# Quantco/tabmat

Measured on AMD Instinct MI355X. Metric: SplitMatrix.sandwich GFLOP/s + effective HBM GB/s, 10M×1k mixed, higher is better.
Workload: dtype f64; 1 GPU; SplitMatrix.sandwich: dense128 + csr512@5% + cats(256,96,32), 10000000 rows/GPU, p=1024, float64 (BASELINE configs[3]); rows_per_gpu=10000000, p=1024, launch=eager, collective=none

## Files before the change

### include/tabmat_hip.h

```cpp
#ifndef TABMAT_HIP_H
#define TABMAT_HIP_H

#include <stddef.h>
#include <stdint.h>

#ifdef __cplusplus
extern "C" {
#endif

#define TM_OK 0
#define TM_EINVAL (-1)
#define TM_ENOMEM (-2)
#define TM_EUNSUPPORTED (-3)

int tm_version(void);
const char *tm_last_error(void);
int tm_device_count(int *count);
int tm_set_device(int device);
int tm_device_info(char *name, int name_len, int *compute_units, int64_t *hbm_bytes);
int tm_malloc(void **ptr, size_t bytes);
int tm_free(void *ptr);
int tm_memcpy_h2d(void *dst, const void *h_src, size_t bytes, void *stream);
int tm_memcpy_d2h(void *h_dst, const void *src, size_t bytes, void *stream);
int tm_memset(void *dst, int value, size_t bytes, void *stream);
// ... 433 lines not shown
                                          int64_t n_sel, int64_t m, const double *d_sel, double *out,
                                          void *stream);
int tm_multi_cat_sparse_sandwich_rows_u8_f32(const void *const *h_codes, const int64_t *h_ncols,
                                             const int32_t *h_drop_first, int n_cats,
                                             const float *cm_data, const uint8_t *cm_col8,
                                             const int32_t *row_ranges, const int32_t *rows,
                                             int64_t n_sel, int64_t m, const float *d_sel, float *out,
                                             void *stream);
int tm_multi_cat_sparse_sandwich_rows_u8_f64(const void *const *h_codes, const int64_t *h_ncols,
                                             const int32_t *h_drop_first, int n_cats,
                                             const double *cm_data, const uint8_t *cm_col8,
                                             const int32_t *row_ranges, const int32_t *rows,
                                             int64_t n_sel, int64_t m, const double *d_sel, double *out,
                                             void *stream);
int tm_multi_cat_sparse_sandwich_ent_f32(const void *const *h_codes, const int64_t *h_ncols,
                                         const int32_t *h_drop_first, int n_cats, int64_t n, const float *d,
                                         const float *vals, const uint16_t *meta, const uint32_t *bstart,
                                         int64_t n_slots, int64_t mk, float *out, void *stream);
int tm_multi_cat_sparse_sandwich_ent_f64(const void *const *h_codes, const int64_t *h_ncols,
                                         const int32_t *h_drop_first, int n_cats, int64_t n, const double *d,
                                         const double *vals, const uint16_t *meta, const uint32_t *bstart,
                                         int64_t n_slots, int64_t mk, double *out, void *stream);
int tm_multi_cat_pack_codes(const void *const *h_codes, const int64_t *h_ncols, const int32_t *h_drop_first, int n_cats,
                            int64_t n, uint32_t *packed, void *stream);
int tm_multi_cat_sparse_sandwich_entp_f32(const void *const *h_codes, const int64_t *h_ncols,
                                          const int32_t *h_drop_first, int n_cats, int64_t n, const float *d,
                                          const float *vals, const uint16_t *meta, const uint32_t *bstart,
                                          int64_t n_slots, int64_t mk, const uint32_t *packed, float *out, void *stream);
int tm_multi_cat_sparse_sandwich_entp_f64(const void *const *h_codes, const int64_t *h_ncols,
                                          const int32_t *h_drop_first, int n_cats, int64_t n, const double *d,
                                          const double *vals, const uint16_t *meta, const uint32_t *bstart,
                                          int64_t n_slots, int64_t mk, const uint32_t *packed, double *out, void *stream);

int tm_multi_cat_sparse_sandwich_slab_f32(const void *const *h_codes, const int64_t *h_ncols,
                                          const int32_t *h_drop_first, int n_cats, int64_t n,
                                          const float *d, const float *vals, const uint32_t *koff,
                                          const uint8_t *ecol, const int64_t *gptr, int64_t m,
                                          float *out, void *stream);
int tm_multi_cat_sparse_sandwich_slab_f64(const void *const *h_codes, const int64_t *h_ncols,
                                          const int32_t *h_drop_first, int n_cats, int64_t n,
                                          const double *d, const double *vals, const uint32_t *koff,
                                          const uint8_t *ecol, const int64_t *gptr, int64_t m,
                                          double *out, void *stream);

int tm_multi_cat_pairs_max_bins(void);
int tm_multi_cat_pairs_max_slots(void);
int tm_multi_cat_pairs_row_words(void);
int tm_multi_cat_pairs_f32(const int64_t *cat_tab, int64_t n, const float *d, const int32_t *rows,
                           int64_t n_rows, const int32_t *bundles, int n_bundles,
                           const int32_t *wg_map, int n_wg, int slots, int64_t bins,
                           const int64_t *desc, int64_t n_pairs, const int64_t *pos, double *tables,
                           double *out, int64_t p, void *stream);
int tm_multi_cat_pairs_f64(const int64_t *cat_tab, int64_t n, const double *d, const int32_t *rows,
                           int64_t n_rows, const int32_t *bundles, int n_bundles,
                           const int32_t *wg_map, int n_wg, int slots, int64_t bins,
                           const int64_t *desc, int64_t n_pairs, const int64_t *pos, double *tables,
                           double *out, int64_t p, void *stream);

int tm_multi_cat_matvec_f32(const int64_t *cat_tab, int n_cats, const int64_t *pos, const float *v,
                            int64_t n, float *out, void *stream);
int tm_multi_cat_matvec_f64(const int64_t *cat_tab, int n_cats, const int64_t *pos, const double *v,
                            int64_t n, double *out, void *stream);

int tm_csr_densify_cols_f32(const float *data, const int32_t *indices, const int64_t *indptr, int64_t n,
                            const int32_t *colmap, float *T, int64_t ld, void *stream);
int tm_csr_densify_cols_f64(const double *data, const int32_t *indices, const int64_t *indptr, int64_t n,
                            const int32_t *colmap, double *T, int64_t ld, void *stream);
int tm_csc_densify_cols_f32(const int32_t *rows, const float *vals, const int64_t *seg, const int32_t *tcol,
                            int64_t n_sel, int64_t max_len, float *T, int64_t ld, void *stream);
int tm_csc_densify_cols_f64(const int32_t *rows, const double *vals, const int64_t *seg, const int32_t *tcol,
                            int64_t n_sel, int64_t max_len, double *T, int64_t ld, void *stream);
int tm_dense_gather_cols_f32(const float *X, int64_t n, int64_t m, int order_f, const int32_t *cols,
                             int64_t n_sel, float *T, int64_t ld, int64_t t0, void *stream);
int tm_dense_gather_cols_f64(const double *X, int64_t n, int64_t m, int order_f, const int32_t *cols,
                             int64_t n_sel, double *T, int64_t ld, int64_t t0, void *stream);

int tm_scatter_block_f32(const float *src, int64_t nr, int64_t nc, const int64_t *ri,
                         const int64_t *ci, double *out, int64_t p, int mirror, int diag,
                         void *stream);
int tm_scatter_block_f64(const double *src, int64_t nr, int64_t nc, const int64_t *ri,
                         const int64_t *ci, double *out, int64_t p, int mirror, int diag,
                         void *stream);

int tm_sparse_sandwich_chunked_rows_f32(const float *cm_data, const int32_t *cm_indices,
                                        const int32_t *row_ranges, int64_t n_sel, int64_t m,
                                        int64_t nnz, const float *d_sel, float *out, void *stream);
int tm_sparse_sandwich_chunked_rows_f64(const double *cm_data, const int32_t *cm_indices,
                                        const int32_t *row_ranges, int64_t n_sel, int64_t m,
                                        int64_t nnz, const double *d_sel, double *out, void *stream);

int tm_sparse_sandwich_chunked_u8_f32(const float *cm_data, const uint8_t *cm_col8, const int32_t *cptr, int64_t n,
                                      int64_t m, int64_t nnz, const float *d, float *out, void *stream);
int tm_sparse_sandwich_chunked_u8_f64(const double *cm_data, const uint8_t *cm_col8, const int32_t *cptr, int64_t n,
                                      int64_t m, int64_t nnz, const double *d, double *out, void *stream);
int tm_sparse_sandwich_chunked_rows_u8_f32(const float *cm_data, const uint8_t *cm_col8, const int32_t *row_ranges,
                                           int64_t n_sel, int64_t m, int64_t nnz, const float *d_sel, float *out,
                                           void *stream);
int tm_sparse_sandwich_chunked_rows_u8_f64(const double *cm_data, const uint8_t *cm_col8, const int32_t *row_ranges,
                                           int64_t n_sel, int64_t m, int64_t nnz, const double *d_sel, double *out,
                                           void *stream);
int tm_sparse_sandwich_direct_f32(const float *csr_data, const int32_t *csr_indices,
                                  const int64_t *csr_indptr, int64_t n, int64_t m, const float *d,
                                  float *out, void *stream);
int tm_sparse_sandwich_direct_f64(const double *csr_data, const int32_t *csr_indices,
                                  const int64_t *csr_indptr, int64_t n, int64_t m, const double *d,
                                  double *out, void *stream);
int tm_csr_dense_sandwich_rows_f32(const float *cm_data, const int32_t *cm_indices,
                                   const int32_t *row_ranges, int64_t n_sel, const int32_t *rows,
                                   const float *d_sel, int64_t n, int64_t m, const float *B, int64_t r,
                                   int order_f, float *out, void *stream);
int tm_csr_dense_sandwich_rows_f64(const double *cm_data, const int32_t *cm_indices,
                                   const int32_t *row_ranges, int64_t n_sel, const int32_t *rows,
                                   const double *d_sel, int64_t n, int64_t m, const double *B, int64_t r,
                                   int order_f, double *out, void *stream);
int tm_csr_dense_sandwich_rows_u8_f32(const float *cm_data, const uint8_t *cm_col8,
                                      const int32_t *row_ranges, int64_t n_sel, const int32_t *rows,
                                      const float *d_sel, int64_t n, int64_t m, const float *B, int64_t r,
                                      int order_f, float *out, void *stream);
int tm_csr_dense_sandwich_rows_u8_f64(const double *cm_data, const uint8_t *cm_col8,
                                      const int32_t *row_ranges, int64_t n_sel, const int32_t *rows,
                                      const double *d_sel, int64_t n, int64_t m, const double *B, int64_t r,
                                      int order_f, double *out, void *stream);

int tm_cat_det_block_rows(void);
int tm_cat_transpose_matvec_det_f32(const int32_t *perm, const int64_t *bstart, int64_t n_blocks,
                                    const int64_t *cat_bptr, int64_t n_cols, const float *v,
                                    float *out, int accumulate, void *stream);
int tm_cat_transpose_matvec_det_f64(const int32_t *perm, const int64_t *bstart, int64_t n_blocks,
                                    const int64_t *cat_bptr, int64_t n_cols, const double *v,
                                    double *out, int accumulate, void *stream);

int tm_cat_dense_sandwich_sorted_f32(const int32_t *perm, const int64_t *bstart, int64_t n_blocks,
                                     const int64_t *cat_bptr, int64_t n_cols, const float *d,
                                     const float *Y, int64_t m, float *out, void *stream);
int tm_cat_dense_sandwich_sorted_f64(const int32_t *perm, const int64_t *bstart, int64_t n_blocks,
                                     const int64_t *cat_bptr, int64_t n_cols, const double *d,
                                     const double *Y, int64_t m, double *out, void *stream);
int tm_csc_dense_sandwich_sorted_f32(const int32_t *rows, const float *vals, const int64_t *bstart,
                                     int64_t n_blocks, const int64_t *col_bptr, int64_t n_cols,
                                     const float *d, const float *Y, int64_t m, float *out,
                                     void *stream);
int tm_csc_dense_sandwich_sorted_f64(const int32_t *rows, const double *vals, const int64_t *bstart,
                                     int64_t n_blocks, const int64_t *col_bptr, int64_t n_cols,
                                     const double *d, const double *Y, int64_t m, double *out,
                                     void *stream);
int tm_cat_sparse_sandwich_sorted_f32(const int32_t *perm, const int64_t *bstart, int64_t n_blocks,
                                      const int64_t *cat_bptr, int64_t n_cols, const float *d,
                                      const float *csr_data, const int32_t *csr_indices,
                                      const int64_t *csr_indptr, int64_t m, float *out, void *stream);
int tm_cat_sparse_sandwich_sorted_f64(const int32_t *perm, const int64_t *bstart, int64_t n_blocks,
                                      const int64_t *cat_bptr, int64_t n_cols, const double *d,
                                      const double *csr_data, const int32_t *csr_indices,
                                      const int64_t *csr_indptr, int64_t m, double *out, void *stream);

int tm_csr_matvec_multi_f32(const float *csr_data, const int32_t *csr_indices,
                            const int64_t *csr_indptr, int64_t n, int64_t m, const float *V,
                            int64_t K, const int32_t *rows, int64_t n_rows, const int32_t *cols,
                            int64_t n_cols, float *out, void *stream);
int tm_csr_rmatvec_multi_f32(const float *csr_data, const int32_t *csr_indices,
                             const int64_t *csr_indptr, int64_t n, int64_t m, const float *V,
                             int64_t K, const int32_t *rows, int64_t n_rows, const int32_t *cols,
                             int64_t n_cols, float *out, void *stream);
int tm_dense_matvec_multi_f32(const float *X, int64_t n, int64_t m, int order_f, const float *V,
                              int64_t K, const int32_t *rows, int64_t n_rows, const int32_t *cols,
                              int64_t n_cols, float *out, void *stream);
int tm_dense_rmatvec_multi_f32(const float *X, int64_t n, int64_t m, int order_f, const float *V,
// ... 31 lines not shown
```

### tabmat_amd/csrc/cat.hip

```cpp
#include <algorithm>

#include "common.hpp"
#include "reduce.hpp"

namespace tmh {

__global__ void fill_i32_kernel(int32_t *p, int64_t n, int32_t v) {
    int64_t i = (int64_t)blockIdx.x * blockDim.x + threadIdx.x;
    if (i < n) p[i] = v;
}

__global__ void scatter_iota_i32_kernel(int32_t *map, const int32_t *cols, int64_t n_cols) {
    int64_t i = (int64_t)blockIdx.x * blockDim.x + threadIdx.x;
    if (i < n_cols) map[cols[i]] = (int32_t)i;
}

int build_col_map(int32_t *map, int64_t m, const int32_t *cols, int64_t n_cols, hipStream_t st) {
    if (m > 0) {
        hipLaunchKernelGGL(fill_i32_kernel, dim3((unsigned)ceil_div(m, 256)), dim3(256), 0, st, map,
                           m, -1);
        TM_LAUNCH_CHECK();
    }
    if (n_cols > 0) {
        hipLaunchKernelGGL(scatter_iota_i32_kernel, dim3((unsigned)ceil_div(n_cols, 256)),
// ... 1199 lines not shown
        }
    }
    __syncthreads();
    F *dst = ws + ((int64_t)blockIdx.y * gridDim.x + blockIdx.x) * stride;
    for (int b = threadIdx.x; b < cs.total * GC; b += blockDim.x)
        dst[b] = (F)tile[(b / GC) * TSTR + (b % GC)];
}

template <typename F, typename IX>
__global__ __launch_bounds__(1024) void multi_cat_sparse_rows_kernel(
    CatSet cs, const F *__restrict__ cm_data, const IX *__restrict__ cm_ind,
    const int32_t *__restrict__ ranges, const int32_t *__restrict__ rows, const F *__restrict__ d_sel,
    int64_t n_sel, int64_t rows_per_block, F *__restrict__ ws, int64_t stride) {
    constexpr int GC = 32;
    extern __shared__ __attribute__((aligned(16))) unsigned char smem_raw[];
    lds_acc_t *tile = reinterpret_cast<lds_acc_t *>(smem_raw);
    constexpr int tstr = GC + 1;
    const int nel = cs.total * tstr;
    for (int b = threadIdx.x; b < nel; b += blockDim.x) tile[b] = 0.0;
    __syncthreads();
    static_assert(SPARSE_CHUNK_COLS == 4 * GC, "the chunk of the chunk-major twin must hold four 32-column groups");
    const int g = blockIdx.y;
    const int ch = g >> 2;
    const int lane = threadIdx.x & 63, wave = threadIdx.x >> 6, nwave = blockDim.x >> 6;
    const int lr = lane >> 3, lt = lane & 7;
    const int64_t t0 = (int64_t)blockIdx.x * rows_per_block;
    const int64_t t1 = min(t0 + rows_per_block, n_sel);
    const int32_t *rg = ranges + (int64_t)ch * n_sel * 2;
    for (int64_t k0 = t0 + wave * 8; k0 < t1; k0 += (int64_t)nwave * 8) {
        const int64_t k = k0 + lr;
        if (k >= t1) continue;
        const F dk = d_sel[k];
        if (dk == F(0)) continue;
        const int e0 = rg[2 * k], e1 = rg[2 * k + 1];
        if (e0 >= e1) continue;
        const int64_t row = rows[k];
        int off[MAX_CATS];
#pragma unroll
        for (int c = 0; c < MAX_CATS; ++c) {
            off[c] = -1;
            if (c < cs.n_cats) {
                const int col = cs.codes[c][row] - cs.drop[c];
                off[c] = col >= 0 ? (cs.off[c] + col) * tstr : -1;
            }
        }
        for (int e = e0 + lt; e < e1; e += 8) {
            const int col = (int)cm_ind[e] - (sizeof(IX) == 1 ? (g & 3) : g) * GC;
            if (col < 0 || col >= GC) continue;
            const lds_acc_t x = (lds_acc_t)(dk * cm_data[e]);
#pragma unroll
            for (int c = 0; c < MAX_CATS; ++c)
                if (off[c] >= 0) atomic_add(&tile[off[c] + col], x);
        }
    }
    __syncthreads();
    F *dst = ws + ((int64_t)blockIdx.y * gridDim.x + blockIdx.x) * stride;
    for (int b = threadIdx.x; b < cs.total * GC; b += blockDim.x)
        dst[b] = (F)tile[(b / GC) * tstr + (b % GC)];
}

static int make_catset(const void *const *h_codes, const int64_t *h_ncols, const int32_t *h_drop,
                       int n_cats, CatSet *cs) {
    if (n_cats < 1 || n_cats > MAX_CATS) {
        set_error("multi-cat call supports 1..%d categoricals, got %d", MAX_CATS, n_cats);
        return TM_EINVAL;
    }
    int off = 0;
    for (int c = 0; c < MAX_CATS; ++c) {
        cs->codes[c] = c < n_cats ? reinterpret_cast<const int32_t *>(h_codes[c]) : nullptr;
        cs->ncol[c] = c < n_cats ? (int)h_ncols[c] : 0;
        cs->drop[c] = c < n_cats ? h_drop[c] : 0;
        cs->off[c] = off;
        off += cs->ncol[c];
    }
    cs->n_cats = n_cats;
    cs->total = off;
    return TM_OK;
}

template <typename F>
static int run_multi_cat_dense(const void *const *h_codes, const int64_t *h_ncols,
                               const int32_t *h_drop, int n_cats, int64_t n, const F *d, const F *M,
                               int64_t m, int order_f, F *out, hipStream_t st,
                               const int32_t *rows = nullptr, int64_t n_rows = 0) {
    CatSet cs;
    int rc = make_catset(h_codes, h_ncols, h_drop, n_cats, &cs);
    if (rc) return rc;
    const int64_t total = (int64_t)cs.total * m;
    if (total == 0) return TM_OK;
    if (rows != nullptr) n = n_rows;
    if (n == 0) {
        TM_HIP(hipMemsetAsync(out, 0, sizeof(F) * (size_t)total, st));
        return TM_OK;
    }
    {
        constexpr int VEC = MCW_VEC;
        constexpr int TJW = 16 * VEC;
        const size_t tile_b = ((sizeof(lds_acc_t) * (size_t)cs.total * TJW + 15) / 16) * 16;
        const size_t lds_w = tile_b + (size_t)16 * MCW_RS * (sizeof(F) + (size_t)n_cats * sizeof(int));
        if (!order_f && n_cats <= 8 && m >= VEC && m % VEC == 0 &&
            (reinterpret_cast<uintptr_t>(M) & 15) == 0 && lds_w <= 150 * 1024 &&
            (int64_t)cs.total * TJW * (int64_t)sizeof(lds_acc_t) < (1ll << 30)) {
            const int64_t n_parts = ceil_div(m, TJW);
            const int64_t stride = (int64_t)cs.total * TJW;
            int64_t nblk = std::max<int64_t>(1, tune("catdense_rounds", 1) * NUM_CU / n_parts);
            nblk = std::min<int64_t>(nblk, std::max<int64_t>(1, ceil_div(n, 4096)));
            const int64_t rpb = ceil_div(ceil_div(n, nblk), MCW_RS) * MCW_RS;
            nblk = ceil_div(n, rpb);
            const size_t tmp_bytes = ((sizeof(F) * (size_t)(n_parts * stride) + 255) / 256) * 256;
            void *wsv = nullptr;
            rc = get_workspace(tmp_bytes + sizeof(F) * (size_t)(n_parts * nblk * stride) + 256, &wsv, st);
            if (rc) return rc;
            F *tmp = reinterpret_cast<F *>(wsv);
            F *ws = reinterpret_cast<F *>(reinterpret_cast<char *>(wsv) + tmp_bytes);
            auto gow = [&](auto kern) -> int {
                TM_HIP(hipFuncSetAttribute(reinterpret_cast<const void *>(kern),
                                           hipFuncAttributeMaxDynamicSharedMemorySize, (int)lds_w));
                prof_begin(st);
                const int nw_dflt = (sizeof(F) == 8 && tile_b > 64 * 1024) ? 8 : 16;
                const int nw = (int)std::min<int64_t>(16, std::max<int64_t>(4, tune("catdense_waves", nw_dflt)));
                hipLaunchKernelGGL(kern, dim3((unsigned)nblk, (unsigned)n_parts), dim3(nw * 64), lds_w, st,
                                   cs, d, M, n, m, rpb, ws, stride, rows, wg_log_ptr());
                prof_end(st);
                TM_LAUNCH_CHECK();
                return TM_OK;
            };
            if (n_cats == 1) rc = gow(&multi_cat_dense_wide_kernel<F, 1>);
            else if (n_cats == 2) rc = gow(&multi_cat_dense_wide_kernel<F, 2>);
            else if (n_cats == 3) rc = gow(&multi_cat_dense_wide_kernel<F, 3>);
            else if (n_cats == 4) rc = gow(&multi_cat_dense_wide_kernel<F, 4>);
            else if (n_cats == 5) rc = gow(&multi_cat_dense_wide_kernel<F, 5>);
            else if (n_cats == 6) rc = gow(&multi_cat_dense_wide_kernel<F, 6>);
            else if (n_cats == 7) rc = gow(&multi_cat_dense_wide_kernel<F, 7>);
            else rc = gow(&multi_cat_dense_wide_kernel<F, 8>);
            if (rc) return rc;
            rc = launch_reduce_partials<F>(ws, stride, (int)nblk, (int)n_parts, tmp, n_parts * stride,
                                           false, st);
            if (rc) return rc;
            hipLaunchKernelGGL((multi_cat_untile_kernel<F>), dim3((unsigned)ceil_div(total, 256)),
                               dim3(256), 0, st, tmp, (int64_t)cs.total, m, TJW, out);
            TM_LAUNCH_CHECK();
            return TM_OK;
        }
    }
    if (rows != nullptr) {
        set_error("multi_cat_dense: the row-list form needs the wide-load path");
        return TM_EUNSUPPORTED;
    }
    int TJ = 64;
    while (TJ > 1 && sizeof(lds_acc_t) * (size_t)cs.total * TJ > HIST_LDS_MAX) TJ >>= 1;
    while (TJ > 1 && TJ / 2 >= m) TJ >>= 1;
    if (sizeof(lds_acc_t) * (size_t)cs.total * TJ > HIST_LDS_MAX) {
        set_error("multi_cat_dense: %d stacked categories exceed the LDS tile", cs.total);
        return TM_EUNSUPPORTED;
    }
    const int64_t n_parts = ceil_div(m, TJ);
    const int64_t stride = (int64_t)cs.total * TJ;
    const size_t lds = sizeof(lds_acc_t) * (size_t)stride;
    int64_t nblk = std::max<int64_t>(1, NUM_CU / n_parts);
    nblk = std::min<int64_t>(nblk, std::max<int64_t>(1, ceil_div(n, 4096)));
    const int64_t rpb = ceil_div(n, nblk);
    nblk = ceil_div(n, rpb);
    const size_t tmp_bytes = ((sizeof(F) * (size_t)(n_parts * stride) + 255) / 256) * 256;
    void *wsv = nullptr;
    rc = get_workspace(tmp_bytes + sizeof(F) * (size_t)(n_parts * nblk * stride) + 256, &wsv, st);
    if (rc) return rc;
    F *tmp = reinterpret_cast<F *>(wsv);
    F *ws = reinterpret_cast<F *>(reinterpret_cast<char *>(wsv) + tmp_bytes);
    auto go = [&](auto kern) -> int {
        if (lds > 48 * 1024)
            TM_HIP(hipFuncSetAttribute(reinterpret_cast<const void *>(kern),
                                       hipFuncAttributeMaxDynamicSharedMemorySize, (int)lds));
        prof_begin(st);
        hipLaunchKernelGGL(kern, dim3((unsigned)nblk, (unsigned)n_parts), dim3(1024), lds, st, cs, d,
                           M, n, m, rpb, ws, stride);
        prof_end(st);
        TM_LAUNCH_CHECK();
        return TM_OK;
    };
#define TM_MCD_CASE(V)                                                                       \
    case V:                                                                                  \
        if (order_f) rc = go(&multi_cat_dense_f_kernel<F, V>);                               \
        else if (n_cats == 1) rc = go(&multi_cat_dense_c_kernel<F, V, 1>);                   \
        else if (n_cats == 2) rc = go(&multi_cat_dense_c_kernel<F, V, 2>);                   \
        else if (n_cats == 3) rc = go(&multi_cat_dense_c_kernel<F, V, 3>);                   \
        else if (n_cats == 4) rc = go(&multi_cat_dense_c_kernel<F, V, 4>);                   \
        else rc = go(&multi_cat_dense_c_kernel<F, V, 0>);                                    \
        break;
    switch (TJ) {
        TM_MCD_CASE(64)
        TM_MCD_CASE(32)
        TM_MCD_CASE(16)
        TM_MCD_CASE(8)
        TM_MCD_CASE(4)
        TM_MCD_CASE(2)
        TM_MCD_CASE(1)
        default:
            rc = TM_EINVAL;
    }
#undef TM_MCD_CASE
    if (rc) return rc;
    rc = launch_reduce_partials<F>(ws, stride, (int)nblk, (int)n_parts, tmp, n_parts * stride, false,
                                   st);
    if (rc) return rc;
    hipLaunchKernelGGL((multi_cat_untile_kernel<F>), dim3((unsigned)ceil_div(total, 256)),
                       dim3(256), 0, st, tmp, (int64_t)cs.total, m, TJ, out);
    TM_LAUNCH_CHECK();
    return TM_OK;
}

template <typename F, typename IX>
static int run_multi_cat_sparse_rows(const void *const *h_codes, const int64_t *h_ncols,
                                     const int32_t *h_drop, int n_cats, const F *cm_data,
                                     const IX *cm_ind, const int32_t *ranges, const int32_t *rows,
                                     int64_t n_sel, int64_t m, const F *d_sel, F *out, hipStream_t st);

template <typename F>
static int run_multi_cat_sparse(const void *const *h_codes, const int64_t *h_ncols,
                                const int32_t *h_drop, int n_cats, int64_t n, const F *d,
                                const F *vals, const unsigned *koff, const unsigned char *ecol,
                                const int64_t *gptr, int64_t m, int slab_rows, int group_cols,
                                F *out, hipStream_t st) {
    CatSet cs;
    int rc = make_catset(h_codes, h_ncols, h_drop, n_cats, &cs);
    if (rc) return rc;
    const int64_t total = (int64_t)cs.total * m;
    if (total == 0) return TM_OK;
    if (n == 0) {
        TM_HIP(hipMemsetAsync(out, 0, sizeof(F) * (size_t)total, st));
        return TM_OK;
    }
    const int64_t stride = (int64_t)cs.total * group_cols;
    const size_t tile_bytes = ((sizeof(lds_acc_t) * (size_t)cs.total * (group_cols + 1) + 15) / 16) * 16;
    if (tile_bytes > HIST_LDS_MAX) {
        set_error("multi_cat_sparse: %d stacked categories exceed the LDS tile", cs.total);
        return TM_EUNSUPPORTED;
    }
    const int nw = (int)std::min<int64_t>(16, std::max<int64_t>(4, tune("catsparse_waves", 16)));
    const size_t stage_bytes = (size_t)nw * slab_rows * (sizeof(F) + sizeof(int32_t) * (size_t)n_cats);
    const bool stage = tile_bytes + stage_bytes <= 150 * 1024;
    const size_t lds = tile_bytes + (stage ? stage_bytes : 0);
    const int n_groups = (int)ceil_div(m, group_cols);
    const int64_t n_slabs = ceil_div(n, slab_rows);
    int64_t nblk = std::max<int64_t>(1, tune("catsparse_rounds", 1) * NUM_CU / n_groups);
    nblk = std::min<int64_t>(nblk, n_slabs);
    const int64_t spb = ceil_div(n_slabs, nblk);
    nblk = ceil_div(n_slabs, spb);
    const size_t tmp_bytes = ((sizeof(F) * (size_t)(n_groups * stride) + 255) / 256) * 256;
    void *wsv = nullptr;
    rc = get_workspace(tmp_bytes + sizeof(F) * (size_t)((int64_t)n_groups * nblk * stride) + 256,
                       &wsv, st);
    if (rc) return rc;
    F *tmp = reinterpret_cast<F *>(wsv);
    F *ws = reinterpret_cast<F *>(reinterpret_cast<char *>(wsv) + tmp_bytes);
    if (stage && n_cats <= 8 && slab_rows == 128) {
        auto kpf = n_cats == 1   ? &multi_cat_sparse_pf_kernel<F, 1>
                   : n_cats == 2 ? &multi_cat_sparse_pf_kernel<F, 2>
                   : n_cats == 3 ? &multi_cat_sparse_pf_kernel<F, 3>
                   : n_cats == 4 ? &multi_cat_sparse_pf_kernel<F, 4>
                   : n_cats == 5 ? &multi_cat_sparse_pf_kernel<F, 5>
                   : n_cats == 6 ? &multi_cat_sparse_pf_kernel<F, 6>
                   : n_cats == 7 ? &multi_cat_sparse_pf_kernel<F, 7>
                                 : &multi_cat_sparse_pf_kernel<F, 8>;
        if (lds > 48 * 1024)
            TM_HIP(hipFuncSetAttribute(reinterpret_cast<const void *>(kpf),
                                       hipFuncAttributeMaxDynamicSharedMemorySize, (int)lds));
        prof_begin(st);
        hipLaunchKernelGGL(kpf, dim3((unsigned)nblk, (unsigned)n_groups), dim3(nw * 64), lds, st, cs, d,
                           vals, koff, ecol, gptr, n_groups, n_slabs, spb, group_cols, n, ws, stride,
                           wg_log_ptr());
        prof_end(st);
        TM_LAUNCH_CHECK();
    } else {
        auto kern = stage ? &multi_cat_sparse_kernel<F, true> : &multi_cat_sparse_kernel<F, false>;
        if (lds > 48 * 1024)
            TM_HIP(hipFuncSetAttribute(reinterpret_cast<const void *>(kern),
                                       hipFuncAttributeMaxDynamicSharedMemorySize, (int)lds));
        prof_begin(st);
        hipLaunchKernelGGL(kern, dim3((unsigned)nblk, (unsigned)n_groups), dim3(nw * 64), lds, st, cs,
                           d, vals, koff, ecol, gptr, n_groups, n_slabs, spb, slab_rows, group_cols,
                           n, ws, stride);
        prof_end(st);
        TM_LAUNCH_CHECK();
    }
    rc = launch_reduce_partials<F>(ws, stride, (int)nblk, n_groups, tmp,
                                   (int64_t)n_groups * stride, false, st);
    if (rc) return rc;
    hipLaunchKernelGGL((multi_cat_untile_kernel<F>), dim3((unsigned)ceil_div(total, 256)),
                       dim3(256), 0, st, tmp, (int64_t)cs.total, m, group_cols, out);
    TM_LAUNCH_CHECK();
    return TM_OK;
}

__global__ __launch_bounds__(256) void multi_cat_pack_codes_kernel(CatSet cs, int64_t n, unsigned *__restrict__ out) {
    for (int64_t r = (int64_t)blockIdx.x * blockDim.x + threadIdx.x; r < n; r += (int64_t)gridDim.x * blockDim.x) {
        unsigned pk = 0u;
#pragma unroll
        for (int c = 0; c < 3; ++c) {
            unsigned f = 1023u;
            if (c < cs.n_cats) {
                const int col = cs.codes[c][r] - cs.drop[c];
                if (col >= 0 && col < cs.ncol[c]) f = (unsigned)(cs.off[c] + col);
            }
            pk |= f << (10 * c);
        }
        out[r] = pk;
    }
}

template <typename F>
static int run_multi_cat_sparse_ent(const void *const *h_codes, const int64_t *h_ncols, const int32_t *h_drop,
                                    int n_cats, int64_t n, const F *d, const F *vals, const unsigned short *meta,
                                    const unsigned *bstart, int64_t mk, F *out, hipStream_t st,
                                    const unsigned *packed = nullptr, int64_t n_slots = 0) {
    CatSet cs;
    int rc = make_catset(h_codes, h_ncols, h_drop, n_cats, &cs);
    if (rc) return rc;
    const int64_t total = (int64_t)cs.total * mk;
    if (total == 0) return TM_OK;
    if (n == 0) {
        TM_HIP(hipMemsetAsync(out, 0, sizeof(F) * (size_t)total, st));
        return TM_OK;
    }
    TM_REQUIRE(mk % 16 == 0 && n_cats >= 1 && n_cats <= 8, "kernel columns in groups of 16, 1 .. 8 categoricals");
    TM_REQUIRE(n < (1ll << 28), "at most 2^28 - 1 rows per block");
    constexpr int GC = 32;
    const int64_t stride = (int64_t)cs.total * GC;
    const size_t lds = ((sizeof(lds_acc_t) * (size_t)cs.total * (GC + 1) + 15) / 16) * 16;
    if (lds > HIST_LDS_MAX) {
        set_error("multi_cat_sparse_ent: %d stacked categories exceed the LDS tile", cs.total);
        return TM_EUNSUPPORTED;
    }
    const int nw = (int)std::min<int64_t>(16, std::max<int64_t>(4, tune("catsparse_waves", 16)));
    const int n_groups = (int)(mk / 16);
    const int n_pairs = (n_groups + 1) / 2;
    const int64_t n_slabs = ceil_div(n, 64);
    int64_t nblk = std::max<int64_t>(1, tune("catsparse_rounds", 1) * NUM_CU / n_pairs);
    nblk = std::min<int64_t>(nblk, n_slabs);
    const int64_t spb = ceil_div(n_slabs, nblk);
    nblk = ceil_div(n_slabs, spb);
    const size_t tmp_bytes = ((sizeof(F) * (size_t)(n_pairs * stride) + 255) / 256) * 256;
    void *wsv = nullptr;
    rc = get_workspace(tmp_bytes + sizeof(F) * (size_t)((int64_t)n_pairs * nblk * stride) + 256, &wsv, st);
    if (rc) return rc;
    F *tmp = reinterpret_cast<F *>(wsv);
    F *ws = reinterpret_cast<F *>(reinterpret_cast<char *>(wsv) + tmp_bytes);
    auto kern = n_cats == 1   ? &multi_cat_sparse_ent_kernel<F, 1>
                : n_cats == 2 ? &multi_cat_sparse_ent_kernel<F, 2>
                : n_cats == 3 ? &multi_cat_sparse_ent_kernel<F, 3>
                : n_cats == 4 ? &multi_cat_sparse_ent_kernel<F, 4>
                : n_cats == 5 ? &multi_cat_sparse_ent_kernel<F, 5>
                : n_cats == 6 ? &multi_cat_sparse_ent_kernel<F, 6>
                : n_cats == 7 ? &multi_cat_sparse_ent_kernel<F, 7>
                              : &multi_cat_sparse_ent_kernel<F, 8>;
    TM_REQUIRE(packed == nullptr || (n_cats <= 3 && cs.total < 1023), "packed codes: at most 3 categoricals, 1022 levels");
    const int ncw = packed != nullptr ? 1 : n_cats;
    const size_t lds_staged = lds + (size_t)nw * 64 * (sizeof(F) + 4 * (size_t)ncw);
    const double fill = (double)n_slots / ((double)std::max(n_groups, 1) * (double)n_slabs);
    if (tune("catsparse_staged", 1) != 0 && lds_staged <= 156 * 1024 &&
        fill >= (double)tune("catsparse_staged_fill", 44)) {
        using KS = void (*)(CatSet, const F *, const F *, const unsigned short *, const unsigned *, int, int64_t, int64_t,
                            int64_t, F *, int64_t, const unsigned *, int);
        KS ks = nullptr;
        if (packed != nullptr) {
            ks = n_cats == 1 ? &multi_cat_sparse_ent_staged_kernel<F, 1, true>
                 : n_cats == 2 ? &multi_cat_sparse_ent_staged_kernel<F, 2, true>
                               : &multi_cat_sparse_ent_staged_kernel<F, 3, true>;
        } else {
            ks = n_cats == 1   ? &multi_cat_sparse_ent_staged_kernel<F, 1, false>
                 : n_cats == 2 ? &multi_cat_sparse_ent_staged_kernel<F, 2, false>
                 : n_cats == 3 ? &multi_cat_sparse_ent_staged_kernel<F, 3, false>
                 : n_cats == 4 ? &multi_cat_sparse_ent_staged_kernel<F, 4, false>
                 : n_cats == 5 ? &multi_cat_sparse_ent_staged_kernel<F, 5, false>
                 : n_cats == 6 ? &multi_cat_sparse_ent_staged_kernel<F, 6, false>
                 : n_cats == 7 ? &multi_cat_sparse_ent_staged_kernel<F, 7, false>
                               : &multi_cat_sparse_ent_staged_kernel<F, 8, false>;
        }
        if (lds_staged > 48 * 1024)
            TM_HIP(hipFuncSetAttribute(reinterpret_cast<const void *>(ks),
                                       hipFuncAttributeMaxDynamicSharedMemorySize, (int)lds_staged));
        prof_begin(st);
        hipLaunchKernelGGL(ks, dim3((unsigned)nblk, (unsigned)n_pairs), dim3(nw * 64), lds_staged, st, cs, d, vals,
                           meta, bstart, n_groups, n, n_slabs, spb, ws, stride, packed, (int)lds);
        prof_end(st);
        TM_LAUNCH_CHECK();
    } else {
        if (lds > 48 * 1024)
            TM_HIP(hipFuncSetAttribute(reinterpret_cast<const void *>(kern),
                                       hipFuncAttributeMaxDynamicSharedMemorySize, (int)lds));
        prof_begin(st);
        hipLaunchKernelGGL(kern, dim3((unsigned)nblk, (unsigned)n_pairs), dim3(nw * 64), lds, st, cs, d, vals, meta,
                           bstart, n_groups, n, n_slabs, spb, ws, stride, packed);
        prof_end(st);
        TM_LAUNCH_CHECK();
    }
    rc = launch_reduce_partials<F>(ws, stride, (int)nblk, n_pairs, tmp, (int64_t)n_pairs * stride, false, st);
    if (rc) return rc;
    hipLaunchKernelGGL((multi_cat_untile_kernel<F>), dim3((unsigned)ceil_div(total, 256)), dim3(256), 0, st, tmp,
                       (int64_t)cs.total, mk, GC, out);
    TM_LAUNCH_CHECK();
    return TM_OK;
}

}

using namespace tmh;

#define TM_CHECK_COMMON(nn) \
    TM_REQUIRE((nn) >= 0, "negative size")

extern "C" {

int tm_cat_transpose_matvec_f32(const int32_t *codes, int64_t n, int64_t n_cols, int drop_first,
                                const float *v, const int32_t *rows, int64_t n_rows,
                                const int32_t *cols, int64_t n_cols_sel, float *out, void *stream) {
    TM_CHECK_COMMON(n);
    return run_cat_tmv<float>(codes, n, n_cols, drop_first, v, rows, n_rows, cols, n_cols_sel, out,
                              as_stream(stream));
}
int tm_cat_transpose_matvec_f64(const int32_t *codes, int64_t n, int64_t n_cols, int drop_first,
                                const double *v, const int32_t *rows, int64_t n_rows,
                                const int32_t *cols, int64_t n_cols_sel, double *out,
                                void *stream) {
    TM_CHECK_COMMON(n);
    return run_cat_tmv<double>(codes, n, n_cols, drop_first, v, rows, n_rows, cols, n_cols_sel,
                               out, as_stream(stream));
}

int tm_cat_matvec_f32(const int32_t *codes, int64_t n, int64_t n_cols, int drop_first,
                      const float *v, const int32_t *cols, int64_t n_cols_sel, float *out,
                      void *stream) {
    TM_CHECK_COMMON(n);
    return run_cat_matvec<float>(codes, n, n_cols, drop_first, v, cols, n_cols_sel, out,
                                 as_stream(stream));
}
int tm_cat_matvec_f64(const int32_t *codes, int64_t n, int64_t n_cols, int drop_first,
                      const double *v, const int32_t *cols, int64_t n_cols_sel, double *out,
                      void *stream) {
    TM_CHECK_COMMON(n);
    return run_cat_matvec<double>(codes, n, n_cols, drop_first, v, cols, n_cols_sel, out,
                                  as_stream(stream));
}

int tm_cat_matvec_assign_f32(const int32_t *codes, int64_t n, int64_t n_cols, int drop_first,
                             const float *v, const int32_t *cols, int64_t n_cols_sel, float *out,
                             void *stream) {
    TM_CHECK_COMMON(n);
    return run_cat_matvec<float>(codes, n, n_cols, drop_first, v, cols, n_cols_sel, out,
                                 as_stream(stream), true);
}
int tm_cat_matvec_assign_f64(const int32_t *codes, int64_t n, int64_t n_cols, int drop_first,
                             const double *v, const int32_t *cols, int64_t n_cols_sel, double *out,
                             void *stream) {
    TM_CHECK_COMMON(n);
    return run_cat_matvec<double>(codes, n, n_cols, drop_first, v, cols, n_cols_sel, out,
                                  as_stream(stream), true);
}

int tm_cat_cat_sandwich_f32(const int32_t *i_codes, const int32_t *j_codes, int64_t n,
                            const float *d, const int32_t *rows, int64_t n_rows, int64_t i_ncol,
                            int64_t j_ncol, int i_drop_first, int j_drop_first, float *out,
                            void *stream) {
    TM_CHECK_COMMON(n);
    return run_hist<float, true>(i_codes, j_codes, d, rows, rows ? n_rows : n, i_drop_first,
                                 j_drop_first, i_ncol, j_ncol, nullptr, out, false,
                                 as_stream(stream));
}
int tm_cat_cat_sandwich_f64(const int32_t *i_codes, const int32_t *j_codes, int64_t n,
                            const double *d, const int32_t *rows, int64_t n_rows, int64_t i_ncol,
                            int64_t j_ncol, int i_drop_first, int j_drop_first, double *out,
                            void *stream) {
    TM_CHECK_COMMON(n);
    return run_hist<double, true>(i_codes, j_codes, d, rows, rows ? n_rows : n, i_drop_first,
                                  j_drop_first, i_ncol, j_ncol, nullptr, out, false,
                                  as_stream(stream));
}

int tm_cat_cat_sandwich_atomic_f32(const int32_t *i_codes, const int32_t *j_codes, int64_t n,
                                   const float *d, const int32_t *rows, int64_t n_rows, int64_t i_ncol,
                                   int64_t j_ncol, int i_drop_first, int j_drop_first, float *out,
                                   void *stream) {
    TM_CHECK_COMMON(n);
    return run_hist<float, true>(i_codes, j_codes, d, rows, rows ? n_rows : n, i_drop_first,
                                 j_drop_first, i_ncol, j_ncol, nullptr, out, false,
                                 as_stream(stream), 12);
}
int tm_cat_cat_sandwich_atomic_f64(const int32_t *i_codes, const int32_t *j_codes, int64_t n,
                                   const double *d, const int32_t *rows, int64_t n_rows, int64_t i_ncol,
                                   int64_t j_ncol, int i_drop_first, int j_drop_first, double *out,
                                   void *stream) {
    TM_CHECK_COMMON(n);
    return run_hist<double, true>(i_codes, j_codes, d, rows, rows ? n_rows : n, i_drop_first,
                                  j_drop_first, i_ncol, j_ncol, nullptr, out, false,
                                  as_stream(stream), 12);
}

int tm_cat_cat_sandwich_sorted_f32(const int32_t *ci_sorted, const int32_t *cj_sorted, const int32_t *perm,
                                   const int64_t *lptr, int64_t n_sorted, const float *d, int64_t i_ncol,
                                   int64_t j_ncol, float *out, void *stream) {
    TM_CHECK_COMMON(n_sorted);
    return run_hist_sorted<float>(ci_sorted, cj_sorted, perm, lptr, n_sorted, d, i_ncol, j_ncol, out,
                                  as_stream(stream));
}
int tm_cat_cat_sandwich_sorted_f64(const int32_t *ci_sorted, const int32_t *cj_sorted, const int32_t *perm,
                                   const int64_t *lptr, int64_t n_sorted, const double *d, int64_t i_ncol,
                                   int64_t j_ncol, double *out, void *stream) {
    TM_CHECK_COMMON(n_sorted);
    return run_hist_sorted<double>(ci_sorted, cj_sorted, perm, lptr, n_sorted, d, i_ncol, j_ncol, out,
                                   as_stream(stream));
}

int tm_cat_dense_sandwich_f32(const int32_t *codes, int64_t n, int64_t i_ncol, int drop_first,
                              const float *d, const int32_t *rows, int64_t n_rows, const float *M,
                              int64_t M_ncol, int order_f, const int32_t *j_cols, int64_t n_j,
                              float *out, void *stream) {
    TM_CHECK_COMMON(n);
    return run_cat_dense<float>(codes, n, i_ncol, drop_first, d, rows, n_rows, M, M_ncol, order_f,
                                j_cols, j_cols ? n_j : M_ncol, out, as_stream(stream));
}
int tm_cat_dense_sandwich_f64(const int32_t *codes, int64_t n, int64_t i_ncol, int drop_first,
                              const double *d, const int32_t *rows, int64_t n_rows,
                              const double *M, int64_t M_ncol, int order_f, const int32_t *j_cols,
                              int64_t n_j, double *out, void *stream) {
    TM_CHECK_COMMON(n);
    return run_cat_dense<double>(codes, n, i_ncol, drop_first, d, rows, n_rows, M, M_ncol, order_f,
                                 j_cols, j_cols ? n_j : M_ncol, out, as_stream(stream));
}

int tm_cat_sparse_sandwich_f32(const int32_t *codes, int64_t n, int64_t i_ncol, int drop_first,
                               const float *csr_data, const int32_t *csr_indices,
                               const int64_t *csr_indptr, int64_t s_ncol, const float *d,
                               const int32_t *rows, int64_t n_rows, const int32_t *cols,
                               int64_t n_cols, float *out, void *stream) {
    TM_CHECK_COMMON(n);
    return run_cat_sparse<float>(codes, n, i_ncol, drop_first, csr_data, csr_indices, csr_indptr,
                                 s_ncol, d, rows, n_rows, cols, n_cols, out, as_stream(stream));
}
int tm_cat_sparse_sandwich_f64(const int32_t *codes, int64_t n, int64_t i_ncol, int drop_first,
                               const double *csr_data, const int32_t *csr_indices,
                               const int64_t *csr_indptr, int64_t s_ncol, const double *d,
                               const int32_t *rows, int64_t n_rows, const int32_t *cols,
                               int64_t n_cols, double *out, void *stream) {
    TM_CHECK_COMMON(n);
    return run_cat_sparse<double>(codes, n, i_ncol, drop_first, csr_data, csr_indices, csr_indptr,
                                  s_ncol, d, rows, n_rows, cols, n_cols, out, as_stream(stream));
}

int tm_multi_cat_dense_sandwich_f32(const void *const *h_codes, const int64_t *h_ncols,
                                    const int32_t *h_drop_first, int n_cats, int64_t n,
                                    const float *d, const float *M, int64_t M_ncol, int order_f,
                                    float *out, void *stream) {
    return run_multi_cat_dense<float>(h_codes, h_ncols, h_drop_first, n_cats, n, d, M, M_ncol,
                                      order_f, out, as_stream(stream));
}
int tm_multi_cat_dense_sandwich_f64(const void *const *h_codes, const int64_t *h_ncols,
                                    const int32_t *h_drop_first, int n_cats, int64_t n,
                                    const double *d, const double *M, int64_t M_ncol, int order_f,
                                    double *out, void *stream) {
    return run_multi_cat_dense<double>(h_codes, h_ncols, h_drop_first, n_cats, n, d, M, M_ncol,
                                       order_f, out, as_stream(stream));
}
int tm_multi_cat_dense_sandwich_rows_f32(const void *const *h_codes, const int64_t *h_ncols,
                                         const int32_t *h_drop_first, int n_cats, int64_t n,
                                         const float *d, const float *M, int64_t M_ncol,
                                         const int32_t *rows, int64_t n_rows, float *out,
                                         void *stream) {
    return run_multi_cat_dense<float>(h_codes, h_ncols, h_drop_first, n_cats, n, d, M, M_ncol, 0, out,
                                      as_stream(stream), rows, n_rows);
}
int tm_multi_cat_dense_sandwich_rows_f64(const void *const *h_codes, const int64_t *h_ncols,
                                         const int32_t *h_drop_first, int n_cats, int64_t n,
                                         const double *d, const double *M, int64_t M_ncol,
                                         const int32_t *rows, int64_t n_rows, double *out,
                                         void *stream) {
    return run_multi_cat_dense<double>(h_codes, h_ncols, h_drop_first, n_cats, n, d, M, M_ncol, 0, out,
                                       as_stream(stream), rows, n_rows);
}
int tm_multi_cat_sparse_sandwich_ent_f32(const void *const *h_codes, const int64_t *h_ncols,
                                         const int32_t *h_drop_first, int n_cats, int64_t n, const float *d,
                                         const float *vals, const uint16_t *meta, const uint32_t *bstart,
                                         int64_t n_slots, int64_t mk, float *out, void *stream) {
    return run_multi_cat_sparse_ent<float>(h_codes, h_ncols, h_drop_first, n_cats, n, d, vals, meta, bstart, mk,
                                           out, as_stream(stream), nullptr, n_slots);
}
int tm_multi_cat_sparse_sandwich_ent_f64(const void *const *h_codes, const int64_t *h_ncols,
                                         const int32_t *h_drop_first, int n_cats, int64_t n, const double *d,
                                         const double *vals, const uint16_t *meta, const uint32_t *bstart,
                                         int64_t n_slots, int64_t mk, double *out, void *stream) {
    return run_multi_cat_sparse_ent<double>(h_codes, h_ncols, h_drop_first, n_cats, n, d, vals, meta, bstart, mk,
                                            out, as_stream(stream), nullptr, n_slots);
}
int tm_multi_cat_pack_codes(const void *const *h_codes, const int64_t *h_ncols, const int32_t *h_drop_first, int n_cats,
                            int64_t n, uint32_t *packed, void *stream) {
    CatSet cs;
    int rc = make_catset(h_codes, h_ncols, h_drop_first, n_cats, &cs);
    if (rc) return rc;
    TM_REQUIRE(n_cats <= 3 && cs.total < 1023, "packed codes: at most 3 categoricals, 1022 stacked levels");
    if (n == 0) return TM_OK;
    hipLaunchKernelGGL(multi_cat_pack_codes_kernel, dim3((unsigned)std::min<int64_t>(4 * NUM_CU, ceil_div(n, 256))),
                       dim3(256), 0, as_stream(stream), cs, n, packed);
    TM_LAUNCH_CHECK();
    return TM_OK;
}
int tm_multi_cat_sparse_sandwich_entp_f32(const void *const *h_codes, const int64_t *h_ncols,
                                          const int32_t *h_drop_first, int n_cats, int64_t n, const float *d,
                                          const float *vals, const uint16_t *meta, const uint32_t *bstart,
                                          int64_t n_slots, int64_t mk, const uint32_t *packed, float *out, void *stream) {
    return run_multi_cat_sparse_ent<float>(h_codes, h_ncols, h_drop_first, n_cats, n, d, vals, meta, bstart, mk, out,
                                           as_stream(stream), packed, n_slots);
}
int tm_multi_cat_sparse_sandwich_entp_f64(const void *const *h_codes, const int64_t *h_ncols,
                                          const int32_t *h_drop_first, int n_cats, int64_t n, const double *d,
                                          const double *vals, const uint16_t *meta, const uint32_t *bstart,
                                          int64_t n_slots, int64_t mk, const uint32_t *packed, double *out, void *stream) {
    return run_multi_cat_sparse_ent<double>(h_codes, h_ncols, h_drop_first, n_cats, n, d, vals, meta, bstart, mk,
                                            out, as_stream(stream), packed, n_slots);
}
int tm_multi_cat_sparse_sandwich_slab_f32(const void *const *h_codes, const int64_t *h_ncols,
                                          const int32_t *h_drop_first, int n_cats, int64_t n,
                                          const float *d, const float *vals, const uint32_t *koff,
                                          const uint8_t *ecol, const int64_t *gptr, int64_t m,
                                          float *out, void *stream) {
    return run_multi_cat_sparse<float>(h_codes, h_ncols, h_drop_first, n_cats, n, d, vals, koff,
                                       ecol, gptr, m, tm_slab_rows(), tm_slab_group_cols(), out,
                                       as_stream(stream));
}
int tm_multi_cat_sparse_sandwich_slab_f64(const void *const *h_codes, const int64_t *h_ncols,
                                          const int32_t *h_drop_first, int n_cats, int64_t n,
                                          const double *d, const double *vals, const uint32_t *koff,
                                          const uint8_t *ecol, const int64_t *gptr, int64_t m,
                                          double *out, void *stream) {
    return run_multi_cat_sparse<double>(h_codes, h_ncols, h_drop_first, n_cats, n, d, vals, koff,
                                        ecol, gptr, m, tm_slab_rows(), tm_slab_group_cols(), out,
                                        as_stream(stream));
}

}

namespace tmh {
template <typename F, typename IX>
static int run_multi_cat_sparse_rows(const void *const *h_codes, const int64_t *h_ncols,
                                     const int32_t *h_drop, int n_cats, const F *cm_data,
                                     const IX *cm_ind, const int32_t *ranges, const int32_t *rows,
                                     int64_t n_sel, int64_t m, const F *d_sel, F *out, hipStream_t st) {
    CatSet cs;
    int rc = make_catset(h_codes, h_ncols, h_drop, n_cats, &cs);
    if (rc) return rc;
    const int64_t total = (int64_t)cs.total * m;
    if (total == 0) return TM_OK;
    if (n_sel == 0) {
        TM_HIP(hipMemsetAsync(out, 0, sizeof(F) * (size_t)total, st));
        return TM_OK;
    }
    constexpr int GC = 32;
    const size_t lds = ((sizeof(lds_acc_t) * (size_t)cs.total * (GC + 1) + 15) / 16) * 16;
    if (lds > HIST_LDS_MAX) {
        set_error("multi_cat_sparse_rows: %d stacked categories exceed the LDS tile", cs.total);
        return TM_EUNSUPPORTED;
    }
    const int n_groups = (int)ceil_div(m, GC);
    const int64_t stride = (int64_t)cs.total * GC;
    int64_t nblk = std::max<int64_t>(1, tune("catsparse_rounds", 1) * NUM_CU / n_groups);
    nblk = std::min<int64_t>(nblk, std::max<int64_t>(1, ceil_div(n_sel, 2048)));
    const int64_t rpb = ceil_div(n_sel, nblk);
    nblk = ceil_div(n_sel, rpb);
    const size_t tmp_bytes = ((sizeof(F) * (size_t)(n_groups * stride) + 255) / 256) * 256;
    void *wsv = nullptr;
    rc = get_workspace(tmp_bytes + sizeof(F) * (size_t)((int64_t)n_groups * nblk * stride) + 256, &wsv, st);
    if (rc) return rc;
    F *tmp = reinterpret_cast<F *>(wsv);
    F *ws = reinterpret_cast<F *>(reinterpret_cast<char *>(wsv) + tmp_bytes);
    auto kern = &multi_cat_sparse_rows_kernel<F, IX>;
    if (lds > 48 * 1024)
        TM_HIP(hipFuncSetAttribute(reinterpret_cast<const void *>(kern),
                                   hipFuncAttributeMaxDynamicSharedMemorySize, (int)lds));
    prof_begin(st);
    hipLaunchKernelGGL(kern, dim3((unsigned)nblk, (unsigned)n_groups), dim3(1024), lds, st, cs, cm_data,
                       cm_ind, ranges, rows, d_sel, n_sel, rpb, ws, stride);
    prof_end(st);
    TM_LAUNCH_CHECK();
    rc = launch_reduce_partials<F>(ws, stride, (int)nblk, n_groups, tmp, (int64_t)n_groups * stride, false, st);
    if (rc) return rc;
    hipLaunchKernelGGL((multi_cat_untile_kernel<F>), dim3((unsigned)ceil_div(total, 256)), dim3(256), 0,
                       st, tmp, (int64_t)cs.total, m, GC, out);
    TM_LAUNCH_CHECK();
    return TM_OK;
}
}

extern "C" {
int tm_multi_cat_sparse_sandwich_rows_f32(const void *const *h_codes, const int64_t *h_ncols,
                                          const int32_t *h_drop_first, int n_cats,
                                          const float *cm_data, const int32_t *cm_indices,
                                          const int32_t *row_ranges, const int32_t *rows,
                                          int64_t n_sel, int64_t m, const float *d_sel, float *out,
                                          void *stream) {
    return tmh::run_multi_cat_sparse_rows<float, int32_t>(h_codes, h_ncols, h_drop_first, n_cats, cm_data,
                                                 cm_indices, row_ranges, rows, n_sel, m, d_sel, out,
                                                 tmh::as_stream(stream));
// ... 33 lines not shown
```

### tabmat_amd/csrc/reduce.hpp

```cpp
#pragma once
#include "common.hpp"

namespace tmh {

template <typename F, bool ACCUMULATE, int NW>
__global__ __launch_bounds__(NW * 64) void reduce_partials_kernel(const F *__restrict__ ws,
                                                                  int64_t stride, int nb,
                                                                  F *__restrict__ out,
                                                                  int64_t out_elems) {
    __shared__ double red[NW][64];
    const int lane = threadIdx.x & 63;
    const int wave = threadIdx.x >> 6;
    const int64_t e = (int64_t)blockIdx.x * 64 + lane;
    const int part = blockIdx.y;
    double acc = 0.0;
    if (e < stride) {
        const F *p = ws + ((int64_t)part * nb) * stride + e;
        for (int b = wave; b < nb; b += NW) acc += (double)p[(int64_t)b * stride];
    }
    red[wave][lane] = acc;
    __syncthreads();
    if (wave == 0 && e < stride) {
        const int64_t o = (int64_t)part * stride + e;
        if (o < out_elems) {
            double s = 0.0;
#pragma unroll
            for (int w = 0; w < NW; w += 4)
                s += (red[w][lane] + red[w + 1][lane]) + (red[w + 2][lane] + red[w + 3][lane]);
            if (ACCUMULATE)
                out[o] += (F)s;
            else
                out[o] = (F)s;
        }
    }
}

template <typename F>
inline int launch_reduce_partials(const F *ws, int64_t stride, int nb, int n_parts, F *out,
                                  int64_t out_elems, bool accumulate, hipStream_t st) {
    dim3 grid((unsigned)ceil_div(stride, 64), (unsigned)n_parts);
    const bool small = (int64_t)grid.x * grid.y < 1024 && nb > 16;
    if (small) {
        if (accumulate)
            hipLaunchKernelGGL((reduce_partials_kernel<F, true, 16>), grid, dim3(1024), 0, st, ws,
                               stride, nb, out, out_elems);
        else
            hipLaunchKernelGGL((reduce_partials_kernel<F, false, 16>), grid, dim3(1024), 0, st, ws,
                               stride, nb, out, out_elems);
    } else if (accumulate) {
        hipLaunchKernelGGL((reduce_partials_kernel<F, true, 4>), grid, dim3(256), 0, st, ws, stride,
                           nb, out, out_elems);
    } else {
        hipLaunchKernelGGL((reduce_partials_kernel<F, false, 4>), grid, dim3(256), 0, st, ws, stride,
                           nb, out, out_elems);
    }
    TM_LAUNCH_CHECK();
    return TM_OK;
}

__global__ void fill_i32_kernel(int32_t *p, int64_t n, int32_t v);
__global__ void scatter_iota_i32_kernel(int32_t *map, const int32_t *cols, int64_t n_cols);

int build_col_map(int32_t *map, int64_t m, const int32_t *cols, int64_t n_cols, hipStream_t st);

}
```

### tabmat_amd/csrc/sparse_blocks.hip

```cpp
#include <algorithm>

#include "common.hpp"
#include "reduce.hpp"

namespace tmh {

constexpr int KB_WAVES = 16;
constexpr int KB_TS = 128;

template <typename F>
__global__ void blocks_assemble_kernel(const F *__restrict__ tiles, int n_out, F *__restrict__ out) {
    const int j = blockIdx.x * blockDim.x + threadIdx.x;
    const int i = blockIdx.y;
    if (i >= n_out || j >= n_out) return;
    const int hi = max(i, j), lo = min(i, j);
    const int I = hi / KB_TS, J = lo / KB_TS;
    const int part = I * (I + 1) / 2 + J;
    out[(int64_t)i * n_out + j] = tiles[(int64_t)part * KB_TS * KB_TS + (hi % KB_TS) * KB_TS + (lo % KB_TS)];
}

constexpr int KB_FLAG_REP_A = 1 << 16;
constexpr int KB_FLAG_REP_B = 1 << 17;

template <typename F, bool U8, bool D12 = false>
// ... 96 lines not shown
                const unsigned iA = min((unsigned)(sd.q.x - baseA) + min((unsigned)e.ta, (unsigned)max(e.nA - 1, 0)), spanA1);
                const unsigned iB = min((unsigned)(sd.q.y - baseB) + min((unsigned)e.tb, (unsigned)max(e.nB - 1, 0)), spanB1);
#ifdef KB_ABL_WRAP
                const unsigned iAw = iA & (unsigned)(KB_ABL_WRAP), iBw = iB & (unsigned)(KB_ABL_WRAP);
                e.ca = ldi(indA, min(iAw, spanA1));
                e.va = ldf(dataA, min(iAw, spanA1));
                e.cb = ldi(indB, min(iBw, spanB1));
                e.vb = ldf(dataB, min(iBw, spanB1));
                return e;
#endif
                e.ca = U8 ? (int)ind8A[iA] : ldi(indA, iA);
                e.va = ldf(dataA, iA);
                e.cb = U8 ? (int)ind8B[iB] : ldi(indB, iB);
                e.vb = ldf(dataB, iB);
                return e;
            };
            auto process = [&](const Grp &cur) {
                __builtin_amdgcn_s_setprio(1);
                const int colA = cur.ta < cur.nA ? cur.ca - i0c : -1;
                const int colB = cur.tb < cur.nB ? cur.cb - j0c : -1;
                const int la = (colA < 0 ? -8 : colA << SH) | offmask;
                const int ba = (int)(((unsigned)colA << (7 + SH)) | ((colA & 15) << (3 + SH)));
                const int kb = colB < 0 ? BIGKEY : colB << SH;
                const F av = cur.va * cur.d, vb = cur.vb;
                add_pair(kb, la, ba, av * vb);
                add_pair(dpp_xor_i32<1>(kb), la, ba, av * dpp_xor<1>(vb));
                add_pair(dpp_xor_i32<2>(kb), la, ba, av * dpp_xor<2>(vb));
                add_pair(dpp_xor_i32<3>(kb), la, ba, av * dpp_xor<3>(vb));
#ifndef KB_ABL_HALFSTEPS
                if constexpr (FULL) {
                    const int kb4 = dpp_xor_i32<4>(kb);
                    const F vb4 = dpp_xor<4>(vb);
                    add_pair(kb4, la, ba, av * vb4);
                    add_pair(dpp_xor_i32<1>(kb4), la, ba, av * dpp_xor<1>(vb4));
                    add_pair(dpp_xor_i32<2>(kb4), la, ba, av * dpp_xor<2>(vb4));
                    add_pair(dpp_xor_i32<3>(kb4), la, ba, av * dpp_xor<3>(vb4));
                }
#endif
                __builtin_amdgcn_s_setprio(0);
            };
            const int gstep = nw * 8;
            const int gw = (wave - w0) * 8;
            Grp ea[2], eb[2];
            Dsc ps[2];
            ea[0] = load_entries(load_desc(gw));
            ea[1] = load_entries(load_desc(gw + gstep));
            ps[0] = load_desc(gw + 2 * gstep);
            ps[1] = load_desc(gw + 3 * gstep);
            for (int g = gw; g < nseg; g += 4 * gstep) {
                eb[0] = load_entries(ps[0]);
                eb[1] = load_entries(ps[1]);
                ps[0] = load_desc(g + 4 * gstep);
                ps[1] = load_desc(g + 5 * gstep);
                process(ea[0]);
                if (g + gstep < nseg) process(ea[1]);
                if (g + 2 * gstep >= nseg) break;
                ea[0] = load_entries(ps[0]);
                ea[1] = load_entries(ps[1]);
                ps[0] = load_desc(g + 6 * gstep);
                ps[1] = load_desc(g + 7 * gstep);
                process(eb[0]);
                if (g + 3 * gstep < nseg) process(eb[1]);
            }
        };
        auto run_tile = [&](auto diag_c) {
            if (wave < wfull) run_list(diag_c, std::true_type{}, b0, bfull, 0, wfull);
            else run_list(diag_c, std::false_type{}, bfull, b1, wfull, (int)(blockDim.x >> 6) - wfull);
        };
        if (I == J) run_tile(std::true_type{});
        else run_tile(std::false_type{});
    }
    __syncthreads();
    if (threadIdx.x == 0) wg_log_end(wglog, t_begin, WG_K2);
    F *dst = ws + ((int64_t)part * max_nb + slot) * (TS * TS);
    for (int b = threadIdx.x; b < TS * TS; b += blockDim.x) {
        const int r = b / TS, c = b % TS;
        dst[b] = (F)tile[r * TS + (c ^ ((r & 15) << 3))];
    }
}

template <typename F, bool U8 = false, bool D12 = false>
static int run_sparse_sandwich_blocks(const F *data, const int32_t *ind, const int32_t *cptr, int64_t n,
                                      int64_t m, int64_t nnz, const int32_t *blocks, const int32_t *wg_tab,
                                      int n_wg, int max_nb, const F *d, F *out, hipStream_t st) {
    if (m == 0) return TM_OK;
    if (n == 0 || nnz == 0 || n_wg == 0) {
        TM_HIP(hipMemsetAsync(out, 0, sizeof(F) * (size_t)(m * m), st));
        return TM_OK;
    }
    constexpr int TS = KB_TS;
    const int nchunk = (int)ceil_div(m, TS);
    const int n_parts = nchunk * (nchunk + 1) / 2;
    TM_REQUIRE(nnz < (1ll << 31) && n < (1ll << 29), "sparse block too large for the block-list sandwich");
    TM_REQUIRE(!D12 || n < (1ll << 24), "12-byte block descriptors hold 24 bits of row");
    TM_REQUIRE(max_nb >= 1 && n_wg >= 1, "empty workgroup table");
    const size_t lds = sizeof(lds_acc_t) * (size_t)(TS * TS);
    const size_t tmp_bytes = (sizeof(F) * (size_t)n_parts * TS * TS + 255) / 256 * 256;
    const size_t ws_bytes = sizeof(F) * (size_t)n_parts * (size_t)max_nb * TS * TS;
    void *wsv = nullptr;
    int rc = get_workspace(tmp_bytes + ws_bytes + 256, &wsv, st);
    if (rc) return rc;
    F *tmp = reinterpret_cast<F *>(wsv);
    F *ws = reinterpret_cast<F *>(reinterpret_cast<char *>(wsv) + tmp_bytes);
    TM_HIP(hipMemsetAsync(ws, 0, ws_bytes, st));
    auto kern = &sparse_sandwich_blocks_kernel<F, U8, D12>;
    TM_HIP(hipFuncSetAttribute(reinterpret_cast<const void *>(kern),
                               hipFuncAttributeMaxDynamicSharedMemorySize, (int)lds));
    prof_begin(st);
    const int kb_waves = (int)std::min<int64_t>(KB_WAVES, std::max<int64_t>(2, tune("k2b_waves", KB_WAVES)));
    hipLaunchKernelGGL(kern, dim3((unsigned)n_wg), dim3(kb_waves * 64), lds, st, data, ind, cptr, n, nnz - 1,
                       blocks, reinterpret_cast<const int4 *>(wg_tab), d,
                       max_nb, ws, wg_log_ptr());
    prof_end(st);
    TM_LAUNCH_CHECK();
    rc = launch_reduce_partials<F>(ws, (int64_t)TS * TS, max_nb, n_parts, tmp, (int64_t)n_parts * TS * TS,
                                   false, st);
    if (rc) return rc;
    hipLaunchKernelGGL((blocks_assemble_kernel<F>), dim3((unsigned)ceil_div(m, 64), (unsigned)m), dim3(64),
                       0, st, tmp, (int)m, out);
    TM_LAUNCH_CHECK();
    return TM_OK;
}

}

extern "C" {

int tm_sparse_sandwich_blocks_f32(const float *cm_data, const int32_t *cm_indices, const int32_t *cptr,
                                  int64_t n, int64_t m, int64_t nnz, const int32_t *blocks,
                                  const int32_t *wg_tab, int n_wg, int max_nb, const float *d, float *out,
                                  void *stream) {
    return tmh::run_sparse_sandwich_blocks<float>(cm_data, cm_indices, cptr, n, m, nnz, blocks, wg_tab, n_wg,
                                                  max_nb, d, out, tmh::as_stream(stream));
}
int tm_sparse_sandwich_blocks_f64(const double *cm_data, const int32_t *cm_indices, const int32_t *cptr,
                                  int64_t n, int64_t m, int64_t nnz, const int32_t *blocks,
                                  const int32_t *wg_tab, int n_wg, int max_nb, const double *d, double *out,
                                  void *stream) {
    return tmh::run_sparse_sandwich_blocks<double>(cm_data, cm_indices, cptr, n, m, nnz, blocks, wg_tab, n_wg,
                                                   max_nb, d, out, tmh::as_stream(stream));
}

int tm_sparse_sandwich_blocks_u8_f32(const float *cm_data, const uint8_t *cm_col8, const int32_t *cptr,
                                     int64_t n, int64_t m, int64_t nnz, const int32_t *blocks,
                                     const int32_t *wg_tab, int n_wg, int max_nb, const float *d, float *out,
                                     void *stream) {
    return tmh::run_sparse_sandwich_blocks<float, true>(cm_data, reinterpret_cast<const int32_t *>(cm_col8), cptr, n, m,
                                                        nnz, blocks, wg_tab, n_wg, max_nb, d, out,
                                                        tmh::as_stream(stream));
}
int tm_sparse_sandwich_blocks_u8_f64(const double *cm_data, const uint8_t *cm_col8, const int32_t *cptr,
                                     int64_t n, int64_t m, int64_t nnz, const int32_t *blocks,
                                     const int32_t *wg_tab, int n_wg, int max_nb, const double *d, double *out,
                                     void *stream) {
    return tmh::run_sparse_sandwich_blocks<double, true>(cm_data, reinterpret_cast<const int32_t *>(cm_col8), cptr, n, m,
                                                         nnz, blocks, wg_tab, n_wg, max_nb, d, out,
                                                         tmh::as_stream(stream));
}

int tm_sparse_sandwich_blocks_p12_f32(const float *cm_data, const uint8_t *cm_col8, const int32_t *cptr,
                                      int64_t n, int64_t m, int64_t nnz, const int32_t *blocks12,
                                      const int32_t *wg_tab, int n_wg, int max_nb, const float *d, float *out,
                                      void *stream) {
    return tmh::run_sparse_sandwich_blocks<float, true, true>(cm_data, reinterpret_cast<const int32_t *>(cm_col8), cptr,
                                                              n, m, nnz, blocks12, wg_tab, n_wg, max_nb, d, out,
                                                              tmh::as_stream(stream));
}
int tm_sparse_sandwich_blocks_p12_f64(const double *cm_data, const uint8_t *cm_col8, const int32_t *cptr,
                                      int64_t n, int64_t m, int64_t nnz, const int32_t *blocks12,
                                      const int32_t *wg_tab, int n_wg, int max_nb, const double *d, double *out,
                                      void *stream) {
    return tmh::run_sparse_sandwich_blocks<double, true, true>(cm_data, reinterpret_cast<const int32_t *>(cm_col8), cptr,
                                                               n, m, nnz, blocks12, wg_tab, n_wg, max_nb, d, out,
                                                               tmh::as_stream(stream));
}

}
```

### tabmat_amd/csrc/sparse_ent.hip

```cpp
#include "common.hpp"
#include "reduce.hpp"

namespace tmh {

constexpr int EN_R = 64;
constexpr int EN_C = 16;
constexpr int EN_NW = 16;
constexpr int EN_THREADS = EN_NW * 64;
constexpr int EN_W = 128;
constexpr int EN_B = 16;
constexpr int EN_SB = 64;

template <typename F>
struct EnLds {
    static constexpr int ROWB = EN_W * (int)sizeof(F);
    static constexpr int SLABB = EN_R * ROWB;
    static constexpr int SCR_OFF = ROWB + 2 * SLABB;
    static constexpr int CS_OFF = SCR_OFF + EN_NW * EN_SB * 16;
    static constexpr int TOTAL = CS_OFF + EN_NW * EN_C * (int)sizeof(double);
};

constexpr int EN_CVGPR = 24;
#define EN_LD "40"

// ... 254 lines not shown
        if (q != 3) enext = scratch[(q + 1) * EN_B + l16];
        EN_TICK(pt_a)
        const int slab = __builtin_amdgcn_readlane((int)e[3], 1);
        while (w < slab) end_slab();
        if (ncopied == 0 && w + 1 < ns) {
            issue_pieces((w & 1) ^ 1, 0, NV);

            ncopied = NV;
            psince += NV;
            lsince = 0;
        }
        EN_TICK(pt_p)
        F a;
        if constexpr (sizeof(F) == 8) a = __hiloint2double((int)e[1], (int)e[0]);
        else a = __uint_as_float(e[0]);
#if defined(EN_ABL_NOBATCH)
        asm volatile("" ::"v"(a), "v"(e[2]), "v"(e[3]));
#else
        const unsigned live = (unsigned)__builtin_amdgcn_ballot_w64(a != F(0)) & 0xffffu;
        const int nq = live ? ((31 - __builtin_clz(live)) >> 2) + 1 : 0;
        unsigned p0 = (unsigned)__builtin_amdgcn_readlane((int)e[3], 0);
        unsigned p1 = (unsigned)__builtin_amdgcn_readlane((int)e[3], 4);
        unsigned p2 = (unsigned)__builtin_amdgcn_readlane((int)e[3], 8);
        unsigned p3 = (unsigned)__builtin_amdgcn_readlane((int)e[3], 12);
        if (nq == 4) en_batch_asm<16, F>(p0, p1, p2, p3, a, e[2], lane_off);
        else if (nq == 3) en_batch_asm<12, F>(p0, p1, p2, p3, a, e[2], lane_off);
        else if (nq == 2) en_batch_asm<8, F>(p0, p1, p2, p3, a, e[2], lane_off);
        else if (nq == 1) en_batch_asm<4, F>(p0, p1, p2, p3, a, e[2], lane_off);
#endif
        EN_TICK(pt_x)
#if defined(EN_PROF)
        ++pt_n;
#endif
    }
    while (w < ns) end_slab();
    wait_loads(std::integral_constant<int, 0>{});
#if defined(EN_PROF)
    if (prof != nullptr && lane == 0) {
        long long *o = prof + (((int64_t)blockIdx.z * gridDim.y + blockIdx.y) * gridDim.x + blockIdx.x) * (EN_NW * 8) + wave * 8;
        o[0] = pt_a; o[1] = pt_p; o[2] = pt_x; o[3] = pt_b; o[4] = pt_bar; o[5] = pt_n; o[6] = clock64() - pt_start; o[7] = ns;
    }
#endif

    if (active) {
        F *dst = ws + (((int64_t)blockIdx.y * gridDim.x + blockIdx.x) * n_groups + group) * (EN_C * EN_W);
        static_for<EN_C>([&](auto jc) {
            constexpr int j = decltype(jc)::value;
            if constexpr (sizeof(F) == 8) {
                const u4 o = u4{en_read_acc<4 * j>(), en_read_acc<4 * j + 1>(), en_read_acc<4 * j + 2>(),
                                en_read_acc<4 * j + 3>()};
                *reinterpret_cast<u4 *>(dst + j * EN_W + 2 * lane) = o;
            } else {
                typedef unsigned u2 __attribute__((ext_vector_type(2)));
                const u2 o = u2{en_read_acc<2 * j>(), en_read_acc<2 * j + 1>()};
                *reinterpret_cast<u2 *>(dst + j * EN_W + 2 * lane) = o;
            }
        });
        if constexpr (CSUM) {
            if (blockIdx.y == 0 && lane < EN_C)
                ws_csum[(int64_t)blockIdx.x * (n_groups * EN_C) + group * EN_C + lane] = (F)cs_lds[lane];
        }
    }
}

template <typename F>
__global__ void en_untile_kernel(const F *__restrict__ tmp, int64_t m, int64_t nB, F *__restrict__ out) {
    const int64_t e = (int64_t)blockIdx.x * blockDim.x + threadIdx.x;
    if (e >= m * nB) return;
    const int64_t i = e / nB, j = e % nB;
    out[e] = tmp[((j / EN_W) * m + i) * EN_W + (j % EN_W)];
}

template <typename F>
__global__ void en_csum_kernel(const F *__restrict__ part, int nblk, int64_t m, F *__restrict__ csum) {
    const int64_t c = (int64_t)blockIdx.x * blockDim.x + threadIdx.x;
    if (c >= m) return;
    double a = 0.0;
    for (int b = 0; b < nblk; ++b) a += (double)part[(int64_t)b * m + c];
    csum[c] = (F)a;
}

template <typename F>
static int run_csr_dense_ent(const F *vals, const uint16_t *meta, const uint32_t *bstart, int64_t n, int64_t m,
                             const F *B, int64_t r, const F *d, F *out, F *colsum, hipStream_t st) {
    const int64_t nB = r;
    const int64_t total = m * nB;
    if (total == 0) return TM_OK;
    constexpr int VEC = 16 / (int)sizeof(F);
    if ((reinterpret_cast<uintptr_t>(B) & 15) != 0 || r % VEC != 0 || nB < VEC) {
        set_error("tm_csr_dense_sandwich_ent: B must be C-ordered with 16-byte aligned rows");
        return TM_EUNSUPPORTED;
    }
    if (m % EN_C != 0) {
        set_error("tm_csr_dense_sandwich_ent: m must be a multiple of tm_ent_group_cols()");
        return TM_EINVAL;
    }
    if (n >= (1ll << 28)) {
        set_error("tm_csr_dense_sandwich_ent: at most 2^28 - 1 rows per block (work in row parts)");
        return TM_EUNSUPPORTED;
    }
    const int64_t n_slabs = ceil_div(n, EN_R);
    const int n_groups = (int)(m / EN_C);
    const int n_parts = (int)ceil_div(nB, EN_W);
    const int nz = (int)ceil_div(n_groups, EN_NW);
    const bool want_csum = colsum != nullptr;
    if (n_slabs == 0) {
        TM_HIP(hipMemsetAsync(out, 0, sizeof(F) * (size_t)total, st));
        if (want_csum) TM_HIP(hipMemsetAsync(colsum, 0, sizeof(F) * (size_t)m, st));
        return TM_OK;
    }
    int64_t nblk = std::max<int64_t>(1, tune("ent_rounds", 1) * NUM_CU / ((int64_t)n_parts * nz));
    nblk = std::min<int64_t>(nblk, n_slabs);
    const int64_t spb = ceil_div(n_slabs, nblk);
    nblk = ceil_div(n_slabs, spb);
    const int64_t stride = m * EN_W;
    const size_t tmp_bytes = (sizeof(F) * (size_t)(n_parts * stride) + 255) / 256 * 256;
    const size_t part_bytes = (sizeof(F) * (size_t)((int64_t)n_parts * nblk * stride) + 255) / 256 * 256;
    const size_t csum_bytes = ((want_csum ? sizeof(F) * (size_t)(nblk * m) : 0) + 255) / 256 * 256 + 256;
    void *wsv = nullptr;
    int rc = get_workspace(tmp_bytes + part_bytes + csum_bytes + 256, &wsv, st);
    if (rc) return rc;
    F *tmp = reinterpret_cast<F *>(wsv);
    F *ws = reinterpret_cast<F *>(reinterpret_cast<char *>(wsv) + tmp_bytes);
    F *ws_csum = reinterpret_cast<F *>(reinterpret_cast<char *>(wsv) + tmp_bytes + part_bytes);
    const size_t lds = (size_t)EnLds<F>::TOTAL;
    auto kern = want_csum ? &csr_dense_ent_kernel<F, true> : &csr_dense_ent_kernel<F, false>;
    TM_HIP(hipFuncSetAttribute(reinterpret_cast<const void *>(kern),
                               hipFuncAttributeMaxDynamicSharedMemorySize, (int)lds));
    prof_begin(st);
    hipLaunchKernelGGL(kern, dim3((unsigned)nblk, (unsigned)n_parts, (unsigned)nz), dim3(EN_THREADS), lds, st,
                       vals, meta, bstart, n_groups, n_slabs, spb, B, n, r, (int)nB, d, ws, ws_csum,
                       reinterpret_cast<long long *>((uintptr_t)tune("ent_prof", 0)));
    prof_end(st);
    TM_LAUNCH_CHECK();
    rc = launch_reduce_partials<F>(ws, stride, (int)nblk, n_parts, tmp, n_parts * stride, false, st);
    if (rc) return rc;
    hipLaunchKernelGGL((en_untile_kernel<F>), dim3((unsigned)ceil_div(total, 256)), dim3(256), 0, st, tmp, m,
                       nB, out);
    TM_LAUNCH_CHECK();
    if (want_csum) {
        hipLaunchKernelGGL((en_csum_kernel<F>), dim3((unsigned)ceil_div(m, 256)), dim3(256), 0, st, ws_csum,
                           (int)nblk, m, colsum);
        TM_LAUNCH_CHECK();
    }
    return TM_OK;
}

}

extern "C" {
int tm_ent_rows(void) { return tmh::EN_R; }
int tm_ent_group_cols(void) { return tmh::EN_C; }
int tm_ent_batch_slots(void) { return tmh::EN_B; }

int tm_csr_dense_sandwich_ent_f32(const float *vals, const uint16_t *meta, const uint32_t *bstart, int64_t n,
                                  int64_t m, const float *B, int64_t r, const float *d, float *out,
                                  float *colsum, void *stream) {
    return tmh::run_csr_dense_ent<float>(vals, meta, bstart, n, m, B, r, d, out, colsum, tmh::as_stream(stream));
}
int tm_csr_dense_sandwich_ent_f64(const double *vals, const uint16_t *meta, const uint32_t *bstart, int64_t n,
                                  int64_t m, const double *B, int64_t r, const double *d, double *out,
                                  double *colsum, void *stream) {
    return tmh::run_csr_dense_ent<double>(vals, meta, bstart, n, m, B, r, d, out, colsum, tmh::as_stream(stream));
}
}
```

### tabmat_amd/csrc/syrk_i8.hip

```cpp
#include <algorithm>
#include <cmath>

#include "common.hpp"

#if defined(I8_NO_SB)
#define I8_SB
#else
#define I8_SB __builtin_amdgcn_sched_barrier(0)
#endif
#if defined(I8_TRACE)
#define I8_STAMP(k)                                                                                     \
    do {                                                                                                \
        if (blockIdx.x == 0 && lane == 0 && trace_it >= 8 && trace_it < 12)                             \
            trace_buf[((trace_it - 8) * 4 + wave) * 8 + (k)] = __builtin_readcyclecounter();            \
    } while (0)
#else
#define I8_STAMP(k)
#endif
namespace tmh {

constexpr int I8_W = 128;
constexpr int I8_T = 36;
constexpr int I8_ND = 5;
constexpr int I8_WLO = 2;
// ... 647 lines not shown
        if (xtv) TM_HIP(hipMemsetAsync(xtv, 0, sizeof(double) * (size_t)m, st));
        return TM_OK;
    }
    if (colsum) TM_HIP(hipMemsetAsync(colsum, 0, sizeof(double) * (size_t)m, st));
    if (xtv) TM_HIP(hipMemsetAsync(xtv, 0, sizeof(double) * (size_t)m, st));
    const int64_t n_items64 = ceil_div(n, I8_ITEM_ROWS);
    TM_REQUIRE(n_items64 < (1ll << 31), "too many rows");
    const int n_items = (int)n_items64;
    const int grid = (int)std::max<int64_t>(1, std::min<int64_t>(n_items, tune("i8_grid", NUM_CU)));
    const size_t part_bytes = sizeof(double) * (size_t)grid * I8_T * 256;
    const size_t own_bytes = (4096 + part_bytes + 255) / 256 * 256;
    void *wsv = nullptr;
    int rc = get_workspace(own_bytes + syrk_co_ws_bytes(), &wsv, st);
    if (rc) return rc;
    char *wb = reinterpret_cast<char *>(wsv);
    I8Info *info = reinterpret_cast<I8Info *>(wb);
    unsigned *counter = reinterpret_cast<unsigned *>(wb + 256);
    double *sigma = reinterpret_cast<double *>(wb + 512);
    double *rscale = reinterpret_cast<double *>(wb + 512 + 1024);
    double *part = reinterpret_cast<double *>(wb + 4096);
    TM_HIP(hipMemsetAsync(wb, 0, 4096 + part_bytes, st));
    const int sgrid = (int)std::min<int64_t>(4 * NUM_CU, ceil_div(n, 1024));
    hipLaunchKernelGGL(i8_screen_kernel, dim3((unsigned)sgrid), dim3(256), 0, st, d, n, info);
    hipLaunchKernelGGL(i8_scale_kernel, dim3(1), dim3(I8_W), 0, st, colmax, (int)m, n, info, sigma, rscale, history);
    TM_LAUNCH_CHECK();
    prof_begin(st);
    auto go = [&](auto kern) {
        hipLaunchKernelGGL(kern, dim3((unsigned)grid), dim3(I8_THREADS), 0, st, X, ldx, n, m, d, sigma, info, n_items,
                           counter, part, colsum, center, v, xtv);
    };
    if (v) {
        if (center) go(syrk_i8_kernel<false, true, true>);
        else go(syrk_i8_kernel<false, false, true>);
    } else if (center) {
        if (colsum) go(syrk_i8_kernel<true, true>);
        else go(syrk_i8_kernel<false, true>);
    } else {
        if (colsum) go(syrk_i8_kernel<true, false>);
        else go(syrk_i8_kernel<false, false>);
    }
    prof_end(st);
    TM_LAUNCH_CHECK();
    hipLaunchKernelGGL(syrk_i8_finish_kernel, dim3(I8_T, 4), dim3(64, 16), 0, st, part, grid, (int)m, rscale, info,
                       out, ldo);
    hipLaunchKernelGGL(i8_envelope_kernel, dim3(1), dim3(I8_W), 0, st, out, ldo, colmax, (int)m, n, info, history);
    TM_LAUNCH_CHECK();
    prof_hold(true);
    rc = run_syrk_co_flagged(X, ldx, n, m, d, out, ldo, colsum, &info->flag, wb + own_bytes, st, center, v, xtv);
    prof_hold(false);
    if (rc == TM_OK && history != nullptr) {
        hipLaunchKernelGGL(i8_record_diag_kernel, dim3(1), dim3(I8_W), 0, st, out, ldo, (int)m, history);
        TM_LAUNCH_CHECK();
    }
    return rc;
}

int run_syrk_i8(const double *X, int64_t n, int64_t m, const double *d, const double *colmax, double *out,
                double *colsum, int *history, hipStream_t st, const double *center = nullptr,
                const double *v = nullptr, double *xtv = nullptr) {
    return run_syrk_i8_panel(X, m, n, m, d, colmax, out, m, colsum, history, st, center, v, xtv);
}

}

extern "C" {

int tm_dense_sandwich_i8_history_words(void) { return 4 + 2 * tmh::I8_W; }

int tm_dense_sandwich_i8_f64(const double *X, int64_t n, int64_t m, const double *d, const double *colmax,
                             double *out, void *stream) {
    return tmh::run_syrk_i8(X, n, m, d, colmax, out, nullptr, nullptr, tmh::as_stream(stream));
}

int tm_dense_sandwich_i8_xtd_f64(const double *X, int64_t n, int64_t m, const double *d, const double *colmax,
                                 double *out, double *colsum, void *stream) {
    return tmh::run_syrk_i8(X, n, m, d, colmax, out, colsum, nullptr, tmh::as_stream(stream));
}

int tm_dense_sandwich_i8_hist_f64(const double *X, int64_t n, int64_t m, const double *d, const double *colmax,
                                  double *out, double *colsum, int32_t *history, void *stream) {
    return tmh::run_syrk_i8(X, n, m, d, colmax, out, colsum, history, tmh::as_stream(stream));
}

int tm_dense_sandwich_i8_centered_f64(const double *X, int64_t n, int64_t m, const double *d, const double *colmax,
                                      const double *center, double *out, double *colsum, int32_t *history,
                                      void *stream) {
    return tmh::run_syrk_i8(X, n, m, d, colmax, out, colsum, history, tmh::as_stream(stream), center);
}

int tm_dense_sandwich_i8_xtv_f64(const double *X, int64_t n, int64_t m, const double *d, const double *v,
                                 const double *colmax, double *out, double *xtv, int32_t *history, void *stream) {
    TM_REQUIRE(v != nullptr && xtv != nullptr, "v and xtv are required");
    return tmh::run_syrk_i8(X, n, m, d, colmax, out, nullptr, history, tmh::as_stream(stream), nullptr, v, xtv);
}

int tm_dense_sandwich_i8_centered_xtv_f64(const double *X, int64_t n, int64_t m, const double *d, const double *v,
                                          const double *colmax, const double *center, double *out, double *xtv,
                                          int32_t *history, void *stream) {
    TM_REQUIRE(v != nullptr && xtv != nullptr, "v and xtv are required");
    return tmh::run_syrk_i8(X, n, m, d, colmax, out, nullptr, history, tmh::as_stream(stream), center, v, xtv);
}

}
```

### tabmat_amd/dense_matrix.py

```python
from __future__ import annotations

import os
import warnings

import numpy as np
import torch

from . import _device as D
from .ext import dense as xd
from .ext._types import DenseDev
from .matrix_base import MatrixBase
from .util import (
    check_indexer,
    check_matvec_dimensions,
    check_matvec_out_shape,
    check_sandwich_compatible,
    check_transpose_matvec_out_shape,
    normalize_index,
    np_dtype_of,
    device_row_index,
    selects_all_columns,
)


# ... 131 lines not shown
    def astype(self, dtype, order="K", casting="unsafe", copy=True):
        return type(self)(self.toarray().astype(dtype, order, casting, copy),
                          column_names=self._colnames, term_names=self._terms)

    def getcol(self, i):
        return type(self)(self.toarray()[:, [i]], column_names=[self._colnames[i]],
                          term_names=[self._terms[i]])

    def __getitem__(self, key):
        row, col = check_indexer(key)
        if self._devblk is not None and selects_all_columns(col, self.shape[1]):
            kind, *arg = device_row_index(row, self.shape[0])
            t = self._devblk.as_2d()
            sub = t[arg[0]:arg[1]] if kind == "slice" else t[D.idx_dev(arg[0], torch.int64)]
            return type(self)(sub, column_names=self._colnames, term_names=self._terms)
        names = np.array(self._colnames, dtype=object)[col].ravel().tolist()
        terms = np.array(self._terms, dtype=object)[col].ravel().tolist()
        return type(self)(self.toarray()[row, col], column_names=names, term_names=terms)

    def __matmul__(self, other):
        return self.matvec(other)

    def __str__(self):
        return "{}x{} DenseMatrix:\n\n".format(*self.shape) + np.array_str(self.toarray())

    def __repr__(self):
        return f"DenseMatrix({np.array2string(self.toarray(), separator=', ')})"

    def multiply(self, other):
        other = np.asanyarray(other)
        arr = self.toarray() * (other[:, None] if other.ndim == 1 else other)
        return type(self)(arr, column_names=self._colnames, term_names=self._terms)

    def _i8_colmax(self, center=None):
        hit = getattr(self, "_i8_ok", None)
        if hit is None:
            hit = False
            blk = self._dev_c()
            if (not blk.order_f and blk.buf.dtype == torch.float64 and 64 < blk.m <= I8_MAX_COLS
                    and (blk.m % 2 == 0 or blk.m <= 128) and blk.n >= I8_MIN_ROWS
                    and blk.buf.data_ptr() % 16 == 0):
                x = blk.as_2d()
                hi, lo = x.amax(dim=0), x.amin(dim=0)
                if bool((torch.isfinite(hi) & torch.isfinite(lo)).all().item()):
                    hit = (hi, lo, torch.maximum(hi, -lo).contiguous())
            self._i8_ok = hit
        if hit is False:
            return None
        if center is None:
            return hit[2]
        return torch.maximum(hit[0] - center, center - hit[1]).contiguous()

    def _i8_history(self, key=None):
        hs = self.__dict__.setdefault("_i8_hist", {})
        h = hs.get(key)
        if h is None:
            from ._lib import lib

            h = hs[key] = torch.zeros(int(lib().tm_dense_sandwich_i8_history_words()), dtype=torch.int32,
                                      device=self._dev_c().buf.device)
        return h

    def _center_dev(self, center):
        if center is None:
            return None
        tdt = D.torch_dtype(self.dtype)
        c = D.to_dev(center, tdt) if not isinstance(center, torch.Tensor) else center.to(tdt)
        return c.contiguous()

    def _sandwich_dev(self, d, rows, cols, center=None):
        if (SYRK_I8 and cols is None and d.dtype == torch.float64
                and (rows is None or D.nlen(rows) >= I8_MASKED_ROWS_SHARE * self.shape[0])):
            cmax = self._i8_colmax(center)
            if cmax is not None:
                key = None if center is None else "centered"
                if rows is not None:
                    d = D.masked_d(d, rows)
                    key = "masked" if center is None else "masked-centered"
                if self.shape[1] > 128:
                    return xd.dense_sandwich_i8_wide(self._dev_c(), d, cmax, center=center)
                return xd.dense_sandwich_i8(self._dev_c(), d, cmax, history=self._i8_history(key), center=center)
        return xd.dense_sandwich(self._dev_c(), d, rows, cols, center=center)

    def _sandwich_xtd_dev(self, d, center=None):
        blk = self._dev_c()
        if SYRK_I8 and d.dtype == torch.float64 and blk.m <= 128:
            cmax = self._i8_colmax(center)
            if cmax is not None:
                return xd.dense_sandwich_i8(blk, d, cmax, want_colsum=True,
                                            history=self._i8_history(None if center is None else "centered"),
                                            center=center)
        if xd.co_supported(blk, d):
            return xd.dense_sandwich_co(blk, d, want_colsum=True, center=center)
        return None

    def _sandwich_xtv_dev(self, d, v, rows=None, center=None):
        from . import categorical_matrix as _cm

        if _cm.DETERMINISTIC or d.dtype != torch.float64 or v.dtype != torch.float64 or v.ndim != 1:
            return None
        n = self.shape[0]
        if rows is not None and not (SYRK_I8 and D.nlen(rows) >= I8_MASKED_ROWS_SHARE * n):
            return None
        blk = self._dev_c()
        res = None
        if SYRK_I8:
            cmax = self._i8_colmax(center)
            if cmax is not None:
                key = None if center is None else "centered"
                if rows is not None:
                    d, v = D.masked_d(d, rows), D.masked_d(v, rows)
                    key = "masked" if center is None else "masked-centered"
                if self.shape[1] > 128:
                    out, _, xtv = xd.dense_sandwich_xtv(blk, d, v.contiguous(), "i8_wide", cmax, center=center)
                else:
                    out, _, xtv = xd.dense_sandwich_xtv(blk, d, v.contiguous(), "i8", cmax,
                                                        history=self._i8_history(key), center=center)
                res = (out, xtv)
        if res is None and rows is None and xd.co_supported(blk, d):
            out, _, xtv = xd.dense_sandwich_xtv(blk, d, v.contiguous(), "co", center=center)
            res = (out, xtv)
        if res is not None and center is not None:
            res = (res[0], res[1] + center.to(torch.float64) * v.sum(dtype=torch.float64))
        return res

    def sandwich_and_transpose_matvec(self, d, v, rows=None, cols=None):
        from .matrix_base import _check_1d

        _check_1d(v)
        d_dev_side, v_dev_side = D.is_dev(d), D.is_dev(v)
        if not d_dev_side:
            d = np.asarray(d)
        if not v_dev_side:
            v = np.asarray(v)
        check_sandwich_compatible(self, d)
        check_matvec_dimensions(self, v, transpose=True)
        n, m = self.shape
        rows_n = normalize_index(rows, n)
        cols_n = normalize_index(cols, m)
        both = None
        if (cols_n is None or (len(cols_n) == m and np.array_equal(cols_n, np.arange(m)))) \
                and (rows_n is None or len(rows_n) < n) and self.dtype == np.float64:
            d_dev = D.to_dev(d)
            if d_dev.dtype == torch.float64:
                both = self._sandwich_xtv_dev(d_dev, D.to_dev(v, torch.float64), D.idx_dev(rows_n))
        if both is None:
            return self.sandwich(d, rows, cols), self.transpose_matvec(v, rows, cols)
        H, g = both
        if not v_dev_side:
            g = D.to_host(g)
            if np.issubdtype(v.dtype, np.floating) and v.dtype != self.dtype:
                g = g.astype(np.result_type(v.dtype, self.dtype))
        return (H if d_dev_side else D.to_host(H)), g

    def _smv_block(self):
        blk = self._dev_c()
        return blk if xd.sandwich_matvec_supported(blk) else None

    def _smv_dev(self, dm, u_full, shift=None, centers=None):
        blk = self._smv_block()
        if blk is None:
            return None
        c, shift = _centre_and_shift(centers, 0, u_full, shift)
        g, w = xd.dense_sandwich_matvec(blk, u_full.contiguous(), dm, center=c, shift=shift, want_w=True)
        return g, w, (None if c is None else (None, c))

# ... 141 lines not shown
```

### tabmat_amd/ext/dense.py

```python
from __future__ import annotations

from .. import _device as D
from .._lib import call
from ._types import DenseDev


def dense_sandwich(X: DenseDev, d, rows, cols, center=None):
    out_m = X.m if cols is None else D.nlen(cols)
    in_n = X.n if rows is None else D.nlen(rows)
    if in_n == 0 or out_m == 0:
        return D.zeros((out_m, out_m), X.dtype)
    out = D.out_buf((out_m, out_m), X.dtype)
    D.same_float("dense_sandwich", X.buf, d)
    if center is not None:
        D.same_float("dense_sandwich", X.buf, center)
        assert center.numel() == X.m and center.is_contiguous()
        call(f"tm_dense_sandwich_centered_{D.fsuf(X.buf)}", D.p(X.buf), X.n, X.m, X.order_f, D.p(d), D.p(rows),
             D.nlen(rows), D.p(cols), D.nlen(cols), D.p(center), D.p(out), D.stream_ptr())
        return out
    call(f"tm_dense_sandwich_{D.fsuf(X.buf)}", D.p(X.buf), X.n, X.m, X.order_f, D.p(d), D.p(rows),
         D.nlen(rows), D.p(cols), D.nlen(cols), D.p(out), D.stream_ptr())
    return out


# ... 33 lines not shown
    D.same_float("dense_matvec_multi", X.buf, V)
    Vc = V.contiguous()
    fn = "tm_dense_rmatvec_multi_" if transpose else "tm_dense_matvec_multi_"
    call(fn + D.fsuf(X.buf), D.p(X.buf), X.n, X.m, X.order_f, D.p(Vc), K, D.p(rows), D.nlen(rows),
         D.p(cols), D.nlen(cols), D.p(out), D.stream_ptr())
    return out


def transpose_square_dot_weights(X: DenseDev, weights, shift):
    out = D.zeros((X.m,), X.dtype)
    if X.n == 0 or X.m == 0:
        return out
    D.same_float("transpose_square_dot_weights", X.buf, weights, shift)
    call(f"tm_dense_col_sq_dev_{D.fsuf(X.buf)}", D.p(X.buf), X.n, X.m, X.order_f, D.p(weights),
         D.p(shift), D.p(out), D.stream_ptr())
    return out


def dense_gather_cols(X: DenseDev, cols, T, t0: int):
    D.same_float("dense_gather_cols", X.buf, T)
    call(f"tm_dense_gather_cols_{D.fsuf(T)}", D.p(X.buf), X.n, X.m, int(X.order_f), D.p(cols),
         D.nlen(cols), D.p(T), T.shape[1], int(t0), D.stream_ptr())


def dense_sandwich_co(X: DenseDev, d, want_colsum=False, center=None):
    import torch

    out = D.out_buf((X.m, X.m), torch.float64)
    cs = D.out_buf((X.m,), torch.float64) if want_colsum else None
    D.same_float("dense_sandwich_co", X.buf, d, out)
    if center is not None:
        D.same_float("dense_sandwich_co", X.buf, center)
        assert center.numel() == X.m and center.is_contiguous()
        call("tm_dense_sandwich_co_centered_f64", D.p(X.buf), X.n, X.m, D.p(d), D.p(center), D.p(out), D.p(cs),
             D.stream_ptr())
        return (out, cs) if want_colsum else out
    call("tm_dense_sandwich_co_f64", D.p(X.buf), X.n, X.m, D.p(d), D.p(out), D.p(cs), D.stream_ptr())
    return (out, cs) if want_colsum else out


def co_supported(X: DenseDev, d, any_width=False) -> bool:
    import torch

    return (not X.order_f and X.buf.dtype == torch.float64 and d.dtype == torch.float64
            and X.m <= 128 and X.m > 0 and X.n > 0 and X.buf.data_ptr() % 16 == 0
            and (any_width or X.m > 64))


def dense_sandwich_bf16x3(X: DenseDev, d):
    import torch

    assert not X.order_f and X.buf.dtype == torch.float32 and X.m % 4 == 0 and X.m <= 256
    out = D.out_buf((X.m, X.m), torch.float32)
    D.same_float("dense_sandwich_bf16x3", X.buf, d)
    call("tm_dense_sandwich_bf16x3_f32", D.p(X.buf), X.n, X.m, D.p(d), D.p(out), D.stream_ptr())
    return out


def dense_sandwich_i8(X: DenseDev, d, colmax, want_colsum=False, history=None, center=None):
    import torch
    from .._lib import lib

    out = D.out_buf((X.m, X.m), torch.float64)
    D.same_float("dense_sandwich_i8", X.buf, d, colmax)
    cs = D.out_buf((X.m,), torch.float64) if want_colsum else None
    if history is not None and history.numel() < int(lib().tm_dense_sandwich_i8_history_words()):
        raise ValueError("history needs tm_dense_sandwich_i8_history_words() int32 words")
    if center is not None:
        D.same_float("dense_sandwich_i8", X.buf, center)
        assert center.numel() == X.m and center.is_contiguous()
        call("tm_dense_sandwich_i8_centered_f64", D.p(X.buf), X.n, X.m, D.p(d), D.p(colmax), D.p(center),
             D.p(out), D.p(cs), D.p(history), D.stream_ptr())
        return (out, cs) if want_colsum else out
    if history is not None:
        call("tm_dense_sandwich_i8_hist_f64", D.p(X.buf), X.n, X.m, D.p(d), D.p(colmax), D.p(out), D.p(cs),
             D.p(history), D.stream_ptr())
        return (out, cs) if want_colsum else out
    if want_colsum:
        call("tm_dense_sandwich_i8_xtd_f64", D.p(X.buf), X.n, X.m, D.p(d), D.p(colmax), D.p(out), D.p(cs),
             D.stream_ptr())
        return out, cs
    call("tm_dense_sandwich_i8_f64", D.p(X.buf), X.n, X.m, D.p(d), D.p(colmax), D.p(out), D.stream_ptr())
    return out


def dense_sandwich_i8_wide(X: DenseDev, d, colmax, center=None):
    import torch

    out = D.out_buf((X.m, X.m), torch.float64)
    D.same_float("dense_sandwich_i8_wide", X.buf, d, colmax)
    if center is not None:
        D.same_float("dense_sandwich_i8_wide", X.buf, center)
        assert center.numel() == X.m and center.is_contiguous()
        call("tm_dense_sandwich_i8_wide_centered_f64", D.p(X.buf), X.n, X.m, D.p(d), D.p(colmax), D.p(center),
             D.p(out), D.stream_ptr())
        return out
    call("tm_dense_sandwich_i8_wide_f64", D.p(X.buf), X.n, X.m, D.p(d), D.p(colmax), D.p(out), D.stream_ptr())
    return out


def dense_sandwich_xtv(X: DenseDev, d, v, kind, colmax=None, history=None, center=None, want_colsum=False):
    import torch
    from .._lib import lib

    out = D.out_buf((X.m, X.m), torch.float64)
    xtv = D.out_buf((X.m,), torch.float64)
    cs = D.out_buf((X.m,), torch.float64) if want_colsum else None
    D.same_float("dense_sandwich_xtv", X.buf, d, v, out)
    assert v.numel() == X.n and v.is_contiguous() and d.numel() == X.n
    if center is not None:
        D.same_float("dense_sandwich_xtv", X.buf, center)
        assert center.numel() == X.m and center.is_contiguous()
    if kind == "co":
        if center is not None:
            call("tm_dense_sandwich_co_centered_xtv_f64", D.p(X.buf), X.n, X.m, D.p(d), D.p(v), D.p(center),
                 D.p(out), D.p(cs), D.p(xtv), D.stream_ptr())
        else:
            call("tm_dense_sandwich_co_xtv_f64", D.p(X.buf), X.n, X.m, D.p(d), D.p(v), D.p(out), D.p(cs), D.p(xtv),
                 D.stream_ptr())
        return out, cs, xtv
    assert not want_colsum, "the int8 kernels give X' d or X' v, not both"
    D.same_float("dense_sandwich_xtv", X.buf, colmax)
    if kind == "i8_wide":
        call("tm_dense_sandwich_i8_wide_xtv_f64", D.p(X.buf), X.n, X.m, D.p(d), D.p(v), D.p(colmax), D.p(center),
             D.p(out), D.p(xtv), D.stream_ptr())
        return out, None, xtv
    assert kind == "i8"
    if history is not None and history.numel() < int(lib().tm_dense_sandwich_i8_history_words()):
        raise ValueError("history needs tm_dense_sandwich_i8_history_words() int32 words")
    if center is not None:
        call("tm_dense_sandwich_i8_centered_xtv_f64", D.p(X.buf), X.n, X.m, D.p(d), D.p(v), D.p(colmax),
             D.p(center), D.p(out), D.p(xtv), D.p(history), D.stream_ptr())
    else:
        call("tm_dense_sandwich_i8_xtv_f64", D.p(X.buf), X.n, X.m, D.p(d), D.p(v), D.p(colmax), D.p(out), D.p(xtv),
             D.p(history), D.stream_ptr())
    return out, None, xtv


SANDWICH_MATVEC_MAX_BYTES = 64 * 8 * 16
SANDWICH_MATVEC_MAX_UNALIGNED = 64 * 8


def sandwich_matvec_supported(X: DenseDev) -> bool:
    if X.order_f or X.m == 0:
        return False
    es = X.buf.element_size()
    aligned = (X.m * es) % 16 == 0 and X.buf.data_ptr() % 16 == 0
    return X.m * es <= SANDWICH_MATVEC_MAX_BYTES if aligned else X.m <= SANDWICH_MATVEC_MAX_UNALIGNED


def dense_sandwich_matvec(X: DenseDev, u, dm, t_add=None, center=None, shift=None, want_w=False):
    g = D.out_buf((X.m,), X.dtype)
    w = D.out_buf((X.n,), X.dtype) if want_w else None
    D.same_float("dense_sandwich_matvec", X.buf, u, dm, t_add, center, shift)
    assert sandwich_matvec_supported(X)
    assert u.numel() == X.m and dm.numel() == X.n and u.is_contiguous() and dm.is_contiguous()
    assert t_add is None or (t_add.numel() == X.n and t_add.is_contiguous())
    assert center is None or (center.numel() == X.m and center.is_contiguous())
    assert shift is None or shift.numel() == 1
    call(f"tm_dense_sandwich_matvec_{D.fsuf(X.buf)}", D.p(X.buf), X.n, X.m, D.p(u), D.p(dm), D.p(t_add),
         D.p(center), D.p(shift), D.p(g), D.p(w), D.stream_ptr())
    return g, w


def dense_sandwich_diag(X: DenseDev, dm, center=None):
    out = D.out_buf((X.m,), X.dtype)
# ... 98 lines not shown
```

### tabmat_amd/ext/sparse.py

```python
from __future__ import annotations

import os


from .. import _device as D
from .._lib import call
from ._types import CsrDev, DenseDev, SlabCsc, SlabEll, SlabEnt, SlabLg


def _csr_args(A: CsrDev):
    return (D.p(A.data), D.p(A.indices), D.p(A.indptr), A.n, A.m)


def sparse_sandwich(A: CsrDev, d, rows, cols):
    m = A.m if cols is None else D.nlen(cols)
    out = D.zeros((m, m), A.dtype)
    if m == 0 or (rows is not None and D.nlen(rows) == 0):
        return out
    D.same_float("sparse_sandwich", A.data, d)
    call(f"tm_sparse_sandwich_{D.fsuf(A.data)}", *_csr_args(A), D.p(d), D.p(rows), D.nlen(rows),
         D.p(cols), D.nlen(cols), D.p(out), D.stream_ptr())
    return out


# ... 55 lines not shown

def csr_matvec_multi(X: CsrDev, V, rows, cols, transpose):
    K = int(V.shape[1])
    n_cols = X.m if cols is None else D.nlen(cols)
    n_rows = X.n if rows is None else D.nlen(rows)
    out = D.zeros((n_cols if transpose else n_rows, K), X.dtype)
    if K == 0 or n_rows == 0 or n_cols == 0:
        return out
    D.same_float("csr_matvec_multi", X.data, V)
    Vc = V.contiguous()
    fn = "tm_csr_rmatvec_multi_" if transpose else "tm_csr_matvec_multi_"
    call(fn + D.fsuf(X.data), *_csr_args(X), D.p(Vc), K, D.p(rows), D.nlen(rows), D.p(cols),
         D.nlen(cols), D.p(out), D.stream_ptr())
    return out


def csr_dense_sandwich_slab(A: SlabCsc, B: DenseDev, d):
    assert B.n == A.n
    out = D.zeros((A.m, B.m), A.vals.dtype)
    if A.m == 0 or B.m == 0 or A.n == 0:
        return out
    D.same_float("csr_dense_sandwich_slab", A.vals, B.buf, d)
    call(f"tm_csr_dense_sandwich_slab_{D.fsuf(A.vals)}", D.p(A.vals), D.p(A.koff), D.p(A.cnt),
         D.p(A.gptr), A.n, A.m, D.p(B.buf), B.m, B.order_f, D.p(d), D.p(out), D.stream_ptr())
    return out


def ell_supported(B: DenseDev) -> bool:
    vec = 16 // B.buf.element_size()
    return (not B.order_f) and B.m % vec == 0 and B.m >= vec and B.buf.data_ptr() % 16 == 0


def csr_dense_sandwich_ell(A: SlabEll, B: DenseDev, d):
    assert B.n == A.n and ell_supported(B)
    if A.m == 0 or B.m == 0 or A.n == 0:
        return D.zeros((A.m, B.m), A.vals.dtype)
    out = D.zeros((A.mk, B.m), A.vals.dtype)
    D.same_float("csr_dense_sandwich_ell", A.vals, B.buf, d)
    fn = "tm_csr_dense_sandwich_ellw_" if A.wide else "tm_csr_dense_sandwich_ell_"
    call(fn + D.fsuf(A.vals), D.p(A.vals), D.p(A.koff), D.p(A.gptr),
         A.n, A.mk, D.p(B.buf), B.m, D.p(d), D.p(out), D.stream_ptr())
    return out[A.inv]


def csr_dense_sandwich_lg(A: SlabLg, B: DenseDev, d, unc=None, want_colsum=False):
    assert B.n == A.n and ell_supported(B)
    dt = A.dtype
    if A.m == 0 or B.m == 0 or A.n == 0:
        z = D.zeros((A.m, B.m), dt)
        return (z, D.zeros((A.m,), dt)) if want_colsum else z
    out = D.out_buf((A.mk, B.m), dt)
    u = int(A.unc if unc is None else unc)
    cs = D.out_buf((A.mk,), dt) if want_colsum else None
    if A.cvals is not None:
        D.same_float("csr_dense_sandwich_lg", A.cvals, B.buf, d)
        call("tm_csr_dense_sandwich_lgc_" + D.fsuf(A.cvals), D.p(A.cvals), D.p(A.cmap), D.p(A.crec),
             D.p(A.xkoff), A.n, A.mk, D.p(B.buf), B.m, D.p(d), u, D.p(out), D.p(cs), D.stream_ptr())
    elif want_colsum:
        D.same_float("csr_dense_sandwich_lg", A.vals, B.buf, d)
        call("tm_csr_dense_sandwich_lg_xtd_" + D.fsuf(A.vals), D.p(A.vals), D.p(A.koff), D.p(A.xptr),
             D.p(A.xvals), D.p(A.xkoff), A.n, A.mk, D.p(B.buf), B.m, D.p(d), u, D.p(out), D.p(cs),
             D.stream_ptr())
    else:
        D.same_float("csr_dense_sandwich_lg", A.vals, B.buf, d)
        call("tm_csr_dense_sandwich_lg_" + D.fsuf(A.vals), D.p(A.vals), D.p(A.koff), D.p(A.xptr),
             D.p(A.xvals), D.p(A.xkoff), A.n, A.mk, D.p(B.buf), B.m, D.p(d), u, D.p(out), D.stream_ptr())
    return (out[A.inv], cs[A.inv]) if want_colsum else out[A.inv]


def csr_dense_sandwich_ent(A: SlabEnt, B: DenseDev, d, want_colsum=False):
    assert B.n == A.n and ell_supported(B)
    dt = A.dtype
    if A.m == 0 or B.m == 0 or A.n == 0:
        z = D.zeros((A.m, B.m), dt)
        return (z, D.zeros((A.m,), dt)) if want_colsum else z
    out = D.out_buf((A.mk, B.m), dt)
    cs = D.out_buf((A.mk,), dt) if want_colsum else None
    D.same_float("csr_dense_sandwich_ent", A.vals, B.buf, d)
    call("tm_csr_dense_sandwich_ent_" + D.fsuf(A.vals), D.p(A.vals), D.p(A.meta), D.p(A.bstart), A.n, A.mk,
         D.p(B.buf), B.m, D.p(d), D.p(out), D.p(cs), D.stream_ptr())
    return (out[A.inv], cs[A.inv]) if want_colsum else out[A.inv]


def _row_table(A: CsrDev, rows, d, as_set: bool):
    import weakref

    import torch

    cm_data, cm_c8, cptr = A.chunk_major()
    cached = getattr(A, "_row_table", None)
    stamp = (rows.data_ptr(), rows._version, int(rows.numel()))
    if cached is not None and cached[0]() is rows and cached[4] == stamp:
        _, r64, dup, tabs, _ = cached
    else:
        r64 = torch.sort(rows.to(torch.int64)).values
        dup = bool((r64[1:] == r64[:-1]).any().item()) if r64.numel() > 1 else False
        tabs = {}
        A._row_table = (weakref.ref(rows), r64, dup, tabs, stamp)
    key = bool(as_set and dup)
    if key not in tabs:
        rr = torch.unique_consecutive(r64) if key else r64
        tabs[key] = (rr, torch.stack([cptr[:, rr], cptr[:, rr + 1]], dim=2).contiguous())
    rr, ranges = tabs[key]
    return cm_data, cm_c8, ranges, rr.to(torch.int32).contiguous(), d[rr].contiguous()


def sparse_sandwich_rows(A: CsrDev, d, rows):
    out = D.zeros((A.m, A.m), A.dtype)
    if A.m == 0 or D.nlen(rows) == 0 or A.data.numel() == 0:
        return out
    D.same_float("sparse_sandwich_rows", A.data, d)
    cm_data, cm_c8, ranges, r32, d_sel = _row_table(A, rows, d, True)
    cols = cm_c8 if K2B_U8 else A.chunk_cols32()
    call(f"tm_sparse_sandwich_chunked_rows_{'u8_' if K2B_U8 else ''}{D.fsuf(A.data)}", D.p(cm_data),
         D.p(cols), D.p(ranges),
         int(r32.numel()), A.m, int(cm_data.numel()), D.p(d_sel), D.p(out), D.stream_ptr())
    return out


def csr_dense_sandwich_rows(A: CsrDev, B: DenseDev, d, rows):
    out = D.zeros((A.m, B.m), A.dtype)
    if A.m == 0 or B.m == 0 or D.nlen(rows) == 0 or A.data.numel() == 0:
        return out
    D.same_float("csr_dense_sandwich_rows", A.data, B.buf, d)
    cm_data, cm_c8, ranges, r32, d_sel = _row_table(A, rows, d, False)
    call(f"tm_csr_dense_sandwich_rows_u8_{D.fsuf(A.data)}", D.p(cm_data), D.p(cm_c8), D.p(ranges),
         int(r32.numel()), D.p(r32), D.p(d_sel), A.n, A.m, D.p(B.buf), B.m, B.order_f, D.p(out),
         D.stream_ptr())
    return out


def sparse_sandwich_chunked(A: CsrDev, d):
    if A.m == 0 or A.n == 0:
        return D.zeros((A.m, A.m), A.dtype)
    out = D.out_buf((A.m, A.m), A.dtype)
    D.same_float("sparse_sandwich_chunked", A.data, d)
    cm_data, cm_c8, cptr = A.chunk_major()
    cols = cm_c8 if K2B_U8 else A.chunk_cols32()
    call(f"tm_sparse_sandwich_chunked_{'u8_' if K2B_U8 else ''}{D.fsuf(A.data)}", D.p(cm_data),
         D.p(cols), D.p(cptr),
         A.n, A.m, int(cm_data.numel()), D.p(d), D.p(out), D.stream_ptr())
    return out


K2_BLOCKS = True


def blocks_sandwich_pays(A: CsrDev) -> bool:
    import torch

    if not K2_BLOCKS or A.n == 0 or A.m == 0 or A.n >= 2**29:
        return False
    nnz = int(A.data.numel())
    nch = -(-A.m // 128)
    if not (0 < nnz < 2**31) or nnz / (A.n * nch) <= 4.5 or nch > 32:
        return False
    est = 16 * 2 * A.n * nch * (nch + 1) // 2
    return est * 3 < torch.cuda.mem_get_info(A.data.device)[0] or bool(getattr(A, "_pb", None))


K2B_U8 = os.environ.get("TABMAT_AMD_K2B_U8", "1") == "1"


def sparse_sandwich_blocks(A: CsrDev, d):
    if A.m == 0 or A.n == 0:
        return D.zeros((A.m, A.m), A.dtype)
    out = D.out_buf((A.m, A.m), A.dtype)
    D.same_float("sparse_sandwich_blocks", A.data, d)
    cm_data, cm_c8, cptr = A.chunk_major()
    blocks, wg_tab, max_nb = A.pair_blocks(d12=None if K2B_U8 else False)
    if int(blocks.shape[1]) == 3:
        call(f"tm_sparse_sandwich_blocks_p12_{D.fsuf(A.data)}", D.p(cm_data), D.p(cm_c8), D.p(cptr), A.n, A.m,
             int(cm_data.numel()), D.p(blocks), D.p(wg_tab), int(wg_tab.shape[0]), int(max_nb), D.p(d),
             D.p(out), D.stream_ptr())
        return out
    if K2B_U8:
        call(f"tm_sparse_sandwich_blocks_u8_{D.fsuf(A.data)}", D.p(cm_data), D.p(cm_c8), D.p(cptr), A.n, A.m,
             int(cm_data.numel()), D.p(blocks), D.p(wg_tab), int(wg_tab.shape[0]), int(max_nb), D.p(d),
             D.p(out), D.stream_ptr())
        return out
    cm_ind = A.chunk_cols32()
    call(f"tm_sparse_sandwich_blocks_{D.fsuf(A.data)}", D.p(cm_data), D.p(cm_ind), D.p(cptr), A.n, A.m,
         int(cm_data.numel()), D.p(blocks), D.p(wg_tab), int(wg_tab.shape[0]), int(max_nb), D.p(d),
         D.p(out), D.stream_ptr())
    return out


def sparse_sandwich_pairs(A: CsrDev, d):
    if A.m == 0 or A.n == 0:
        return D.zeros((A.m, A.m), A.dtype)
    out = D.out_buf((A.m, A.m), A.dtype)
    D.same_float("sparse_sandwich_pairs", A.data, d)
    _, _, cptr = A.chunk_major()
    if K2_PAIRS_PACKED and A.n < 2**25:
        rec = A.chunk_records_packed()
        call(f"tm_sparse_sandwich_pairs_pk_{D.fsuf(A.data)}", D.p(rec), D.p(cptr), A.n, A.m, int(A.data.numel()), D.p(d),
             D.p(out), D.stream_ptr())
        return out
    rec = A.chunk_records()
    call(f"tm_sparse_sandwich_pairs_{D.fsuf(A.data)}", D.p(rec), D.p(cptr), A.n, A.m, int(rec.shape[0]), D.p(d),
         D.p(out), D.stream_ptr())
    return out


def csc_dense_sandwich_sorted(A: CsrDev, B: DenseDev, d):
    if A.m == 0 or B.m == 0:
        return D.zeros((A.m, B.m), A.dtype)
    rows, vals, bstart, n_blocks, col_bptr = A.csc_blocks()
    out = D.out_buf((A.m, B.m), A.dtype)
    D.same_float("csc_dense_sandwich_sorted", vals, B.buf, d)
    call(f"tm_csc_dense_sandwich_sorted_{D.fsuf(vals)}", D.p(rows), D.p(vals), D.p(bstart),
         int(n_blocks), D.p(col_bptr), A.m, D.p(d), D.p(B.buf), B.m, D.p(out), D.stream_ptr())
    return out


def sparse_sandwich_direct(A: CsrDev, d):
    if A.m == 0 or A.n == 0:
        return D.zeros((A.m, A.m), A.dtype)
    out = D.out_buf((A.m, A.m), A.dtype)
    D.same_float("sparse_sandwich_direct", A.data, d)
    call(f"tm_sparse_sandwich_direct_{D.fsuf(A.data)}", D.p(A.data), D.p(A.indices), D.p(A.indptr),
         A.n, A.m, D.p(d), D.p(out), D.stream_ptr())
    return out


def direct_sandwich_pays(A: CsrDev) -> bool:
    nnz, n, m = int(A.data.numel()), A.n, A.m
    if n == 0 or nnz == 0 or m <= 1024:
        return False
    nch = (m + 127) // 128
    per_row = nnz / n
    pairs = n * per_row * (per_row + 1.0) / 2.0 * 1.3
    if nch > 32:
        return pairs / 15e9 < n * (nch * (nch + 1) / 2) * 0.3e-9
    if per_row / nch > 0.6:
        return False
    return pairs / 15e9 < n * (nch * (nch + 1) / 2) * 15e-12


K2_PAIRS = "auto"
K2_PAIRS_PACKED = os.environ.get("TABMAT_AMD_K2_PAIRS_PACKED", "1") == "1"
K2_PAIRS_MAX_M = 16384
K2_PAIRS_MAX_NNZ = 2**31 - 4 * 16 * 64


def pairs_sandwich_pays(A: CsrDev) -> bool:
    if K2_PAIRS != "auto":
        return K2_PAIRS == "1" and A.m <= K2_PAIRS_MAX_M and 0 < int(A.data.numel()) < K2_PAIRS_MAX_NNZ
    nnz, n, m = int(A.data.numel()), A.n, A.m
    if n == 0 or nnz == 0 or m <= 512 or m > K2_PAIRS_MAX_M or nnz >= K2_PAIRS_MAX_NNZ:
        return False
    nch = (m + 127) // 128
    parts = nch * (nch + 1) / 2
    per_row = nnz / n
    k = per_row / nch
    pairs = n * per_row * (per_row + 2.0) / 2.0
    pk = 0.75 if (K2_PAIRS_PACKED and n < 2**25) else 1.0
    t_pairs = (nnz * (nch + 1) / 2.0 * 2.3e-12 * pk * min(6.0, max(1.0, (1.6 / k) ** 0.8)) + pairs * 2.7e-12 * pk
               + min(parts, 768) * 0.8e-6 + max(0.0, parts - 768) * 0.1e-6)
    t_direct = pairs / 21e9
    if nch > 32:
        t_tiled = n * parts * 0.3e-9
    else:
        t_tiled = pairs * 1.15e-12 if k > 4.5 else n * parts * 17e-12 + pairs * 0.8e-12
    return t_pairs < 0.9 * min(t_direct, t_tiled)


def transpose_square_dot_weights(A: CsrDev, weights):
# ... 51 lines not shown
```

### tabmat_amd/ext/split.py

```python
from __future__ import annotations

import ctypes as C

import numpy as np

from .. import _device as D
from .._lib import call
from ._types import CsrDev, DenseDev, SlabCsc


def sandwich_cat_dense(i_indices, i_ncol, d, mat_j: DenseDev, rows, j_cols, drop_first=False):
    n_j = mat_j.m if j_cols is None else D.nlen(j_cols)
    res = D.zeros((i_ncol, n_j), mat_j.dtype)
    n_rows = i_indices.numel() if rows is None else D.nlen(rows)
    if d.numel() == 0 or n_rows == 0 or n_j == 0 or i_ncol == 0:
        return res
    D.same_float("sandwich_cat_dense", mat_j.buf, d)
    call(f"tm_cat_dense_sandwich_{D.fsuf(mat_j.buf)}", D.p(i_indices), i_indices.numel(), i_ncol,
         int(drop_first), D.p(d), D.p(rows), D.nlen(rows), D.p(mat_j.buf), mat_j.m, mat_j.order_f,
         D.p(j_cols), D.nlen(j_cols), D.p(res), D.stream_ptr())
    return res


def sandwich_cat_cat(i_indices, j_indices, i_ncol, j_ncol, d, rows, i_drop_first=False,
# ... 262 lines not shown
        order = np.argsort(b, kind="stable").astype(np.int32)
        ends = np.cumsum(np.bincount(b, minlength=n_blocks))
        starts = np.concatenate([[0], ends[:-1]])
        return ([order[s:e] for s, e in zip(starts, ends)],
                [loc[order[s:e]] for s, e in zip(starts, ends)], len(cols))
    next_idx = [0] * n_blocks
    sub_idx = [[] for _ in range(n_blocks)]
    sub_cols = [[] for _ in range(n_blocks)]
    for i, c in enumerate(cols.tolist()):
        for j in range(n_blocks):
            ind = self.indices[j]
            k = next_idx[j]
            while k < len(ind) and ind[k] < c:
                k += 1
            next_idx[j] = k
            if k < len(ind) and ind[k] == c:
                sub_idx[j].append(i)
                sub_cols[j].append(k)
                next_idx[j] = k + 1
                break
    return (
        [np.array(s, dtype=np.int32) for s in sub_idx],
        [np.array(s, dtype=np.int32) for s in sub_cols],
        len(cols),
    )


def is_sorted(a) -> bool:
    a = np.asarray(a)
    return bool(np.all(a[1:] >= a[:-1]))


MAX_FUSED_CATS = 16


def _cat_args(cats):
    n = len(cats)
    codes = (C.c_void_p * n)(*[c[0].data_ptr() for c in cats])
    ncols = (C.c_int64 * n)(*[int(c[1]) for c in cats])
    drop = (C.c_int32 * n)(*[int(bool(c[2])) for c in cats])
    return codes, ncols, drop, n


def multi_cat_dense_wide_ok(cats, mat_j: DenseDev) -> bool:
    fb = mat_j.buf.element_size()
    vec = 2
    total = sum(int(c[1]) for c in cats)
    tile = (total * 16 * vec * 8 + 15) // 16 * 16
    lds = tile + 16 * 32 * (fb + 4 * len(cats))
    return (not mat_j.order_f and 1 <= len(cats) <= 8 and mat_j.m >= vec and mat_j.m % vec == 0
            and mat_j.buf.data_ptr() % 16 == 0 and lds <= 150 * 1024)


def multi_cat_dense_tile_ok(cats, mat_j: DenseDev) -> bool:
    total = sum(int(c[1]) for c in cats)
    m = mat_j.m
    if total == 0 or m == 0 or not 1 <= len(cats) <= 16:
        return False
    tj = 64
    while tj > 1 and 8 * total * tj > 128 * 1024:
        tj >>= 1
    while tj > 1 and tj // 2 >= m:
        tj >>= 1
    return 8 * total * tj <= 128 * 1024 and (m + tj - 1) // tj <= 2


def multi_cat_dense_sandwich(cats, d, mat_j: DenseDev, rows=None):
    total = sum(int(c[1]) for c in cats)
    if total == 0 or mat_j.m == 0 or mat_j.n == 0 or (rows is not None and D.nlen(rows) == 0):
        return D.zeros((total, mat_j.m), mat_j.dtype)
    res = D.out_buf((total, mat_j.m), mat_j.dtype)
    codes, ncols, drop, n = _cat_args(cats)
    if rows is not None:
        D.same_float("multi_cat_dense_sandwich", mat_j.buf, d)
        call(f"tm_multi_cat_dense_sandwich_rows_{D.fsuf(mat_j.buf)}", codes, ncols, drop, n, mat_j.n,
             D.p(d), D.p(mat_j.buf), mat_j.m, D.p(rows), D.nlen(rows), D.p(res), D.stream_ptr())
        return res
    D.same_float("multi_cat_dense_sandwich", mat_j.buf, d)
    call(f"tm_multi_cat_dense_sandwich_{D.fsuf(mat_j.buf)}", codes, ncols, drop, n, mat_j.n,
         D.p(d), D.p(mat_j.buf), mat_j.m, mat_j.order_f, D.p(res), D.stream_ptr())
    return res


def multi_cat_sparse_sandwich(cats, d, S: SlabCsc):
    total = sum(int(c[1]) for c in cats)
    if total == 0 or S.m == 0 or S.n == 0:
        return D.zeros((total, S.m), S.vals.dtype)
    res = D.out_buf((total, S.m), S.vals.dtype)
    codes, ncols, drop, n = _cat_args(cats)
    D.same_float("multi_cat_sparse_sandwich", S.vals, d)
    call(f"tm_multi_cat_sparse_sandwich_slab_{D.fsuf(S.vals)}", codes, ncols, drop, n, S.n, D.p(d),
         D.p(S.vals), D.p(S.koff), D.p(S.ecol), D.p(S.gptr), S.m, D.p(res), D.stream_ptr())
    return res


PACKED_CODES = True


def pack_codes(cats):
    import torch

    total = sum(int(c[1]) for c in cats)
    if not PACKED_CODES or len(cats) > 3 or total >= 1023 or len(cats) == 0:
        return None
    codes, ncols, drop, n = _cat_args(cats)
    nrow = int(cats[0][0].numel())
    out = torch.empty((nrow,), dtype=torch.int32, device=cats[0][0].device)
    call("tm_multi_cat_pack_codes", codes, ncols, drop, n, nrow, D.p(out), D.stream_ptr())
    return out


def multi_cat_sparse_sandwich_ent(cats, d, E, packed=None):
    total = sum(int(c[1]) for c in cats)
    if total == 0 or E.m == 0 or E.n == 0:
        return D.zeros((total, E.m), E.vals.dtype)
    res = D.out_buf((total, E.mk), E.vals.dtype)
    codes, ncols, drop, n = _cat_args(cats)
    D.same_float("multi_cat_sparse_sandwich_ent", E.vals, d)
    if packed is not None:
        call(f"tm_multi_cat_sparse_sandwich_entp_{D.fsuf(E.vals)}", codes, ncols, drop, n, E.n, D.p(d),
             D.p(E.vals), D.p(E.meta), D.p(E.bstart), E.n_slots(), E.mk, D.p(packed), D.p(res), D.stream_ptr())
        return res[:, E.inv]
    call(f"tm_multi_cat_sparse_sandwich_ent_{D.fsuf(E.vals)}", codes, ncols, drop, n, E.n, D.p(d),
         D.p(E.vals), D.p(E.meta), D.p(E.bstart), E.n_slots(), E.mk, D.p(res), D.stream_ptr())
    return res[:, E.inv]


def multi_cat_sparse_sandwich_rows(cats, d, A, rows):
    from . import sparse as xs

    total = sum(int(c[1]) for c in cats)
    if total == 0 or A.m == 0 or D.nlen(rows) == 0 or A.data.numel() == 0:
        return D.zeros((total, A.m), A.data.dtype)
    res = D.out_buf((total, A.m), A.data.dtype)
    codes, ncols, drop, n = _cat_args(cats)
    D.same_float("multi_cat_sparse_sandwich_rows", A.data, d)
    cm_data, cm_c8, ranges, r32, d_sel = xs._row_table(A, rows, d, False)
    call(f"tm_multi_cat_sparse_sandwich_rows_u8_{D.fsuf(A.data)}", codes, ncols, drop, n, D.p(cm_data),
         D.p(cm_c8), D.p(ranges), D.p(r32), int(r32.numel()), A.m, D.p(d_sel), D.p(res), D.stream_ptr())
    return res
```

### tabmat_amd/sparse_matrix.py

```python
from __future__ import annotations

import os

import numpy as np
import torch
from scipy import sparse as sps

from . import _device as D
from .ext import sparse as xs
from .ext._types import CsrDev, SlabCsc, SlabEll, SlabEnt, SlabLg
from .matrix_base import MatrixBase
from .util import (
    check_indexer,
    check_matvec_dimensions,
    check_matvec_out_shape,
    check_sandwich_compatible,
    check_transpose_matvec_out_shape,
    normalize_index,
    device_row_index,
    selects_all_columns,
)


ELL_MAX_PAD = 8.0
# ... 228 lines not shown
            for a, b, part in parts:
                r = None
                if rows is not None:
                    r64 = rows.to(torch.int64)
                    sel = r64[(r64 >= a) & (r64 < b)]
                    if sel.numel() == 0:
                        continue
                    r = (sel - a).to(torch.int32)
                res = part._sandwich_dev(d[a:b], r, cols)
                out = res if out is None else out + res
            if out is None:
                k = self.shape[1] if cols is None else D.nlen(cols)
                out = D.zeros((k, k), d.dtype)
            return out
        A = self._dev()
        from . import categorical_matrix as _cm

        if _cm.DETERMINISTIC and A.data.numel() > 0 and self.shape[0] > 0:
            res = self._sandwich_deterministic(d, rows, cols)
            if res is not None:
                return res
            import warnings

            warnings.warn("TABMAT_AMD_DETERMINISTIC=1: this sparse block has no entry twin, its self sandwich "
                          "falls back to the LDS-atomic kernels and is NOT bit-reproducible from run to run",
                          RuntimeWarning, stacklevel=3)
        if getattr(self, "_direct_pays", None) is None:
            self._direct_pays = xs.direct_sandwich_pays(A)
        w = D.nlen(cols) if cols is not None else 0
        if (0 < w <= NARROW_COLS and 2 * w < self.shape[1] and self.shape[0] > 0 and A.data.numel() > 0
                and self._narrow_pays(w)
                and self.shape[0] * w * A.data.element_size() * 4 < torch.cuda.mem_get_info()[0]):
            from .ext import dense as xd
            from .ext._types import DenseDev

            rws, vls, bstart, _, col_bptr = A.csc_blocks()
            mx = getattr(self, "_max_col_len", None)
            if mx is None:
                ends = bstart[col_bptr]
                mx = self._max_col_len = int((ends[1:] - ends[:-1]).max().item())
            cd = cols.to(torch.int64)
            seg = torch.stack([bstart[col_bptr[cd]], bstart[col_bptr[cd + 1]]], dim=1).contiguous()
            T = torch.zeros((self.shape[0], w), dtype=A.data.dtype, device=A.data.device)
            xs.csc_densify_cols(rws, vls, seg, torch.arange(w, dtype=torch.int32, device=A.data.device),
                                mx, T)
            return xd.dense_sandwich(DenseDev(T, self.shape[0], w, 0), d, rows, None)
        pp = getattr(self, "_pairs_pay", None)
        if pp is None:
            pp = self._pairs_pay = xs.pairs_sandwich_pays(A)
        if pp and (rows is None or D.nlen(rows) > 0.3 * self.shape[0]):
            d = D.masked_d(d, rows, as_set=True)
            res = xs.sparse_sandwich_pairs(A, d)
            if cols is not None:
                c64 = cols.to(torch.int64)
                res = res[c64][:, c64].contiguous()
            return res
        pays = getattr(self, "_direct_pays", None)
        if pays is None:
            pays = self._direct_pays = xs.direct_sandwich_pays(A)
        if pays:
            d = D.masked_d(d, rows, as_set=True)
            res = xs.sparse_sandwich_direct(A, d)
            if cols is not None:
                c64 = cols.to(torch.int64)
                res = res[c64][:, c64].contiguous()
            return res
        if A.data.numel() > 0 and A.data.numel() < 2**31 and self.shape[1] <= 128 * 32:
            if rows is not None and 0 < D.nlen(rows) <= ROW_LIST_FRACTION * self.shape[0]:
                res = xs.sparse_sandwich_rows(A, d, rows)
                if cols is not None:
                    c64 = cols.to(torch.int64)
                    res = res[c64][:, c64].contiguous()
                return res
            d = D.masked_d(d, rows, as_set=True)
            bl = getattr(self, "_blocks_pay", None)
            if bl is None:
                bl = self._blocks_pay = xs.blocks_sandwich_pays(A)
            res = xs.sparse_sandwich_blocks(A, d) if bl else xs.sparse_sandwich_chunked(A, d)
            if cols is not None:
                c64 = cols.to(torch.int64)
                res = res[c64][:, c64].contiguous()
            return res
        return xs.sparse_sandwich(A, d, rows, cols)

    def _ent_det(self):
        ent = self._ent()
        if ent is None:
            hit = getattr(self, "_entblk_det", None)
            if hit is None:
                twin = SlabEnt.from_csr(self._dev(), max_pad=None)
                hit = self._entblk_det = twin if twin is not None else False
            ent = hit or None
        return ent

    def _sandwich_deterministic(self, d, rows, cols=None):
        from .ext._types import DenseDev

        ent = self._ent_det()
        if ent is None:
            return None
        n, m = self.shape
        A = self._dev()
        d = D.masked_d(d, rows, as_set=True)
        inv = None
        if cols is None:
            sel = torch.arange(m, dtype=torch.int64, device=d.device)
        else:
            sel, inv = torch.unique(cols.to(torch.int64), return_inverse=True)
            if int(sel.numel()) == int(inv.numel()) and bool((sel == cols.to(torch.int64)).all()):
                inv = None
        k = int(sel.numel())
        out = torch.empty((m, k), dtype=d.dtype, device=d.device)
        W = 128
        for c0 in range(0, k, W):
            w = min(W, k - c0)
            w_pad = (w + 3) // 4 * 4
            colmap = torch.full((m,), -1, dtype=torch.int32, device=d.device)
            colmap[sel[c0:c0 + w]] = torch.arange(w, dtype=torch.int32, device=d.device)
            T = torch.zeros((n, w_pad), dtype=A.data.dtype, device=d.device)
            xs.csr_densify_cols(A, colmap, T)
            res = xs.csr_dense_sandwich_ent(ent, DenseDev(T, n, w_pad, 0), d)
            out[:, c0:c0 + w] = res[:, :w]
            del T
        out = out if cols is None else out[sel]
        low = torch.tril(out)
        full = low + torch.tril(out, -1).T
        if inv is not None:
            full = full.index_select(0, inv).index_select(1, inv)
        return full

    def _sdiag_dev(self, d, rows, want_s1=False):
        parts = self._row_parts()
        if parts is not None:
            s1 = D.zeros((self.shape[1],), d.dtype) if want_s1 else None
            s2 = D.zeros((self.shape[1],), d.dtype)
            for a, b, part in parts:
                r = None
                if rows is not None:
                    r64 = rows.to(torch.int64)
                    sel = r64[(r64 >= a) & (r64 < b)]
                    if sel.numel() == 0:
                        continue
                    r = (sel - a).to(torch.int32)
                p1, p2 = part._sdiag_dev(d[a:b], r, want_s1)
                s2 += p2
                if want_s1:
                    s1 += p1
            return s1, s2
        A = self._dev()
        if rows is not None and A.data.numel() > 0 and not self._values_finite():
            r64 = rows.to(torch.int64)
            return xs.csr_sandwich_diag(A.take_rows("index", r64), d[r64].contiguous(), want_s1)
        return xs.csr_sandwich_diag(A, D.masked_d(d, rows).contiguous(), want_s1)

    def sandwich_diag(self, d, rows=None, cols=None):
        from .matrix_base import _sd_args

        a = _sd_args(self, d, rows, cols)
        if a.trivial is not None:
            return a.finish(a.trivial)
        tdt = D.torch_dtype(self.dtype)
        _, g = self._sdiag_dev(D.to_dev(a.d, tdt), D.idx_dev(a.rows))
        if a.cols is not None:
            g = g[D.idx_dev(a.cols, torch.int64)]
        return a.finish(g)

# ... 136 lines not shown
```

### tabmat_amd/split_matrix.py

```python
from __future__ import annotations

import os
import warnings
from collections.abc import Sequence
from typing import Optional, Union

import numpy as np
import torch
from scipy import sparse as sps

from . import _device as D
from .categorical_matrix import CategoricalMatrix
from .dense_matrix import DenseMatrix, _centre_and_shift
from .ext import split as xsplit
from .ext.dense import dense_glm_loss_grad as xd_glm
from .ext.dense import dense_sandwich_matvec as xd_smv
from .matrix_base import MatrixBase
from .sparse_matrix import SparseMatrix
from .standardized_mat import StandardizedMatrix
from .util import (
    check_matvec_dimensions,
    check_matvec_out_shape,
    check_sandwich_compatible,
    check_transpose_matvec_out_shape,
    collapse_identity,
    normalize_index,
    set_up_rows_or_cols,
)


ROW_LIST_FRACTION_CATSPARSE = 0.04
DIAG_FROM_PAIRS = True
CAT_PAIRS_FUSED = os.environ.get("TABMAT_AMD_CAT_PAIRS", "1") != "0"
FULL_THEN_SELECT = float(os.environ.get("TABMAT_AMD_FULL_THEN_SELECT", "0.5"))
FULL_RESULT_MAX_BYTES = 256 << 20
FULL_UNSELECTED_SHARE = 0.2
FULL_THEN_SELECT_MV = 0.0
NARROW_COLS = int(os.environ.get("TABMAT_AMD_NARROW_COLS", "128"))
from . import categorical_matrix as _cm
from . import sparse_matrix as _spm


class _Centering:
    NARROW_GROUP = 1 << 20

    def __init__(self, vec):
        self.vec = dict(vec)
        self.cs_centered = set()
        self.groups = None

    def get(self, b):
        return self.vec.get(b)


class _Xtv:

    def __init__(self, v):
        self.v = v
        self.out = {}


def as_tabmat(a):
    if isinstance(a, (MatrixBase, StandardizedMatrix)):
        return a
    if sps.issparse(a):
        return SparseMatrix(a.tocsc(copy=False))
    if isinstance(a, np.ndarray):
        return DenseMatrix(a)
    raise ValueError(f"Cannot convert type {type(a)} to Matrix.")


def hstack(tup: Sequence) -> MatrixBase:
    mats = [as_tabmat(a) for a in tup]
    if not mats:
        raise ValueError("Need at least one array to concatenate.")
    if all(isinstance(m, SparseMatrix) for m in mats):
        return SparseMatrix(sps.hstack([m.array_csc for m in mats]))
    if all(isinstance(m, DenseMatrix) for m in mats):
        return DenseMatrix(np.hstack([m.toarray() for m in mats]))
    return SplitMatrix(mats)


def _merge_same_kind(matrices, indices):
    for kind in (DenseMatrix, SparseMatrix):
        which = [i for i, m in enumerate(matrices) if isinstance(m, kind)]
        if len(which) <= 1:
            continue
        gidx = np.concatenate([indices[i] for i in which])
        order = np.argsort(gidx)
        names = np.concatenate([np.array(matrices[i]._colnames, dtype=object) for i in which])
        terms = np.concatenate([np.array(matrices[i]._terms, dtype=object) for i in which])
        if kind is DenseMatrix:
            merged = DenseMatrix(np.hstack([matrices[i].toarray() for i in which])[:, order])
        else:
            merged = SparseMatrix(sps.hstack([matrices[i].array_csc for i in which]).tocsc()[:, order])
        merged._colnames = names[order].tolist()
        merged._terms = terms[order].tolist()
        matrices[which[0]] = merged
        indices[which[0]] = gidx[order]
        drop = set(which[1:])
        matrices = [m for i, m in enumerate(matrices) if i not in drop]
        indices = [x for i, x in enumerate(indices) if i not in drop]
    return matrices, indices


def _block_sdiag(mb, d, rows, center=None, want_s1=False):
    d = d.to(D.torch_dtype(mb.dtype))
    if isinstance(mb, DenseMatrix):
        return mb._sdiag_dev(d, rows, None if center is None else center.to(d.dtype).contiguous()), None
    if isinstance(mb, SparseMatrix):
        s1, s2 = mb._sdiag_dev(d, rows, want_s1)
        return s2, s1
    if isinstance(mb, CategoricalMatrix):
        h = mb._sandwich_diag_dev(d, rows, None)
        return h, (h if want_s1 else None)
    r = None if rows is None else D.to_host(rows)
    s2 = D.to_dev(mb.sandwich_diag(d, r))
    return s2, (D.to_dev(mb.transpose_matvec(d, r)) if want_s1 else None)


class SplitMatrix(MatrixBase):
# ... 218 lines not shown
        cmask = None if center is None else torch.zeros((n_cols,), dtype=torch.bool, device=xtd.device)
        for i, (mi, pd, sd) in enumerate(zip(self.matrices, pos_d, sub_d)):
            if sd is not None and D.nlen(sd) == 0:
                continue
            cs = colsum[i]
            if cs is None:
                if isinstance(mi, CategoricalMatrix):
                    full = D.zeros((mi.shape[1],), d.dtype)
                    mi._transpose_matvec_dev(d, rows, sd, full)
                    cs = full if sd is None else full[sd.to(torch.int64)]
                else:
                    cs = mi._matvec_dev(d, rows, sd, None, True)
            elif center is not None and i in center.cs_centered:
                cmask[pd] = True
            xtd[pd] = cs.to(torch.float64)
        if center is not None:
            return out, xtd, cmask, center.groups
        return out, xtd

    FUSED_LEVELS = 496
    FUSED_CATS = 8

    def _cat_groups(self, cat_ids):
        groups, cur, tot = [], [], 0
        for i in cat_ids:
            k = self.matrices[i].shape[1]
            if k > self.FUSED_LEVELS:
                continue
            if cur and (len(cur) == self.FUSED_CATS or tot + k > self.FUSED_LEVELS):
                groups.append(cur)
                cur, tot = [], 0
            cur.append(i)
            tot += k
        if cur:
            groups.append(cur)
        return groups

    def _cat_pairs_plan(self):
        plan = self.__dict__.get("_cp_plan", False)
        if plan is False:
            plan = None
            ids = [i for i, m in enumerate(self.matrices)
                   if isinstance(m, CategoricalMatrix) and m.shape[1] > 0]
            if len(ids) >= 1:
                pos = self._full_dev_indices()
                plan = xsplit.CatPairsPlan([(i, self.matrices[i].shape[1]) for i in ids],
                                           [pos[i] for i in ids])
            self.__dict__["_cp_plan"] = plan
        return plan

    def _cat_hist_plan(self):
        plan = self.__dict__.get("_ch_plan", False)
        if plan is False:
            plan = None
            ids = [i for i, m in enumerate(self.matrices)
                   if isinstance(m, CategoricalMatrix) and m.shape[1] > 0 and m.shape[0] > 0]
            if len(ids) >= 2:
                pos = self._full_dev_indices()
                plan = xsplit.CatPairsPlan([(i, self.matrices[i].shape[1]) for i in ids],
                                           [pos[i] for i in ids], diag_only=True)
            self.__dict__["_ch_plan"] = plan
        return plan

    def _fused_cats(self, mw, cats, cat_ids, d_eff, rows, total, budget, d_rows=None):
        if isinstance(mw, DenseMatrix) and xsplit.multi_cat_dense_wide_ok(cats, mw._dev_c()):
            if rows is not None and D.nlen(rows) <= 0.5 * self.shape[0]:
                return xsplit.multi_cat_dense_sandwich(cats, d_rows, mw._dev_c(), rows)
            return xsplit.multi_cat_dense_sandwich(cats, d_eff, mw._dev_c())
        if isinstance(mw, DenseMatrix) and xsplit.multi_cat_dense_tile_ok(cats, mw._dev_c()):
            return xsplit.multi_cat_dense_sandwich(cats, d_eff, mw._dev_c())
        if isinstance(mw, DenseMatrix):
            if xsplit.cat_dense_sorted_ok(mw._dev_c()):
                return None
            from .ext import sparse as xs

            oh, inv = self._onehot_slab(cat_ids)
            return xs.csr_dense_sandwich_slab(oh, mw._dev_c(), d_eff)[inv]
        if (isinstance(mw, SparseMatrix) and total * 33 <= budget and rows is not None
                and 0 < D.nlen(rows) <= ROW_LIST_FRACTION_CATSPARSE * self.shape[0]
                and 0 < mw._dev().data.numel() < 2**31):
            return xsplit.multi_cat_sparse_sandwich_rows(cats, d_rows, mw._dev(), rows)
        if (isinstance(mw, SparseMatrix) and total * 33 <= budget
                and mw._dev().data.numel() > 0 and (rows is None or mw._values_finite())):
            ent = None
            if len(cats) <= 8 and (getattr(mw, "_entblk", None) or any(
                    isinstance(mo, DenseMatrix) and mo.shape[1] > 64 and mo.dtype == mw.dtype
                    for mo in self.matrices)):
                ent = mw._ent()
            if ent is not None:
                pk_cache = self.__dict__.setdefault("_packed_codes", {})
                key = tuple(cat_ids)
                if key not in pk_cache:
                    pk_cache[key] = xsplit.pack_codes(cats)
                return xsplit.multi_cat_sparse_sandwich_ent(cats, d_eff, ent, pk_cache[key])
            return xsplit.multi_cat_sparse_sandwich(cats, d_eff, mw._slab())
        return None

    def _parts(self):
        parts = self.__dict__.get("_row_parts", False)
        if parts is False:
            parts = None
            big = [m for m in self.matrices
                   if isinstance(m, SparseMatrix) and m._dev().data.numel() >= _spm.PART_NNZ]
            if big:
                n = self.shape[0]
                lead = max(big, key=lambda m: m._dev().data.numel())
                ptr = lead._dev().indptr
                nnz = int(ptr[-1].item())
                k = -(-nnz // max(1, int(0.8 * _spm.PART_NNZ)))
                while True:
                    targets = torch.arange(1, k, device=ptr.device, dtype=torch.int64) * nnz // k
                    cuts = [0] + torch.searchsorted(ptr, targets).clamp_(0, n).tolist() + [n]
                    cuts = sorted(set(int(c) for c in cuts))
                    ok = all(int((m._dev().indptr[cuts[1:]] - m._dev().indptr[cuts[:-1]]).max().item())
                             < _spm.PART_NNZ for m in big)
                    if ok or k >= n:
                        break
                    k += 1
                parts = [(a, b, self[a:b]) for a, b in zip(cuts[:-1], cuts[1:]) if b > a]
            self.__dict__["_row_parts"] = parts
        return parts

    def _sandwich_parts(self, parts, d, rows, cols_host, colsum, center=None):
        out = None
        for a, b, part in parts:
            r = None
            if rows is not None:
                r64 = rows.to(torch.int64)
                sel = r64[(r64 >= a) & (r64 < b)]
                if sel.numel() == 0:
                    continue
                r = (sel - a).to(torch.int32)
            cs = [None] * len(self.matrices) if colsum is not None else None
            sub_cen = None if center is None else _Centering(center.vec)
            res = part._sandwich_dev(d[a:b], r, cols_host, None, cs, center=sub_cen)
            if sub_cen is not None:
                center.groups = sub_cen.groups
            if sub_cen is not None and colsum is not None:
                dsum = (d[a:b] if r is None else d[a:b][r.to(torch.int64)]).sum(dtype=torch.float64)
                _, sub_p, _ = self._sandwich_plan(cols_host)
                for i in sub_cen.cs_centered:
                    if cs[i] is not None and sub_cen.get(i) is not None:
                        cv = sub_cen.get(i).to(torch.float64)
                        if sub_p[i] is not None:
                            cv = cv[sub_p[i].to(torch.int64)]
                        cs[i] = cs[i].to(torch.float64) + cv * dsum
            out = res if out is None else out + res
            if colsum is not None:
                for i, c in enumerate(cs):
                    if c is None:
                        colsum[i] = False
                    elif colsum[i] is not False:
                        colsum[i] = c if colsum[i] is None else colsum[i] + c
        if colsum is not None:
            for i, c in enumerate(colsum):
                if c is False:
                    colsum[i] = None
        if out is None:
            _, _, n_cols = self._sandwich_plan(cols_host)
            out = D.zeros((n_cols, n_cols), torch.float64)
        return out

    def _full_product_pays(self, sub_h) -> bool:
        p = self.shape[1]
        if p * p * 8 > FULL_RESULT_MAX_BYTES:
            return False
        n = max(self.shape[0], 1)
        tot = unsel = 0.0
        for b, mb in enumerate(self.matrices):
            if isinstance(mb, DenseMatrix):
                wb = float(mb.shape[1])
            elif isinstance(mb, SparseMatrix):
                nnz = mb._devblk.data.numel() if mb._devblk is not None else mb._host().nnz
                wb = max(1.0, float(nnz) / n)
            else:
                wb = 1.0 + mb.shape[1] / 256.0
            tot += wb
            if len(sub_h[b]) == 0:
                unsel += wb
# ... 24 lines not shown
                and any(len(sub_h[b]) < mats[b].shape[1] for b in noncat)
                and self.shape[0] * (w + 1) * itemsize * 4 < torch.cuda.mem_get_info()[0]):
            w_pad = w + (w & 1)
            t0, parts = 0, []
            sel = np.zeros(n_cols, dtype=np.int64)
            for b in noncat:
                s = len(sub_h[b])
                if s == 0:
                    continue
                sc = np.asarray(sub_h[b], dtype=np.int32)
                if isinstance(mats[b], SparseMatrix):
                    rws, vls, bstart, _, col_bptr = mats[b]._dev().csc_blocks()
                    cd = D.idx_dev(sc, torch.int64)
                    seg = torch.stack([bstart[col_bptr[cd]], bstart[col_bptr[cd + 1]]], dim=1).contiguous()
                    mx = int((seg[:, 1] - seg[:, 0]).max().item()) if s else 0
                    tcol = D.to_dev(t0 + np.arange(s, dtype=np.int32))
                    parts.append((b, t0, s, (rws, vls, seg, tcol, mx)))
                else:
                    parts.append((b, t0, s, D.to_dev(sc)))
                sel[np.asarray(pos_h[b], dtype=np.int64)] = t0 + np.arange(s)
                t0 += s
            off, cat_off, cat_sub = w_pad, {}, {}
            for i in cat:
                cat_off[i] = off
                if len(sub_h[i]):
                    sel[np.asarray(pos_h[i], dtype=np.int64)] = off + np.asarray(sub_h[i], dtype=np.int64)
                    cat_sub[i] = D.idx_dev(sub_h[i], torch.int64)
                off += mats[i].shape[1]
            indices = [np.arange(w_pad)] + [cat_off[i] + np.arange(mats[i].shape[1]) for i in cat]
            nar = dict(w=w, w_pad=w_pad, parts=parts, cat=cat, cat_sub=cat_sub, indices=indices,
                       sel=D.to_dev(sel), tmp=None, n_cols=n_cols)
        elif noncat and w > NARROW_COLS and FULL_THEN_SELECT <= 1.0 and self._full_product_pays(sub_h):
            nar = "wide"
        self.__dict__["_narrow_cache"] = (key, nar)
        return nar

    def _sandwich_narrow(self, nar, d, rows, colsum, center=None):
        from .ext import dense as xd
        from .ext import sparse as xs
        from .ext._types import DenseDev

        n = self.shape[0]
        T = torch.zeros((n, nar["w_pad"]), dtype=d.dtype, device=d.device)
        for b, t0, s, idx in nar["parts"]:
            mb = self.matrices[b]
            if isinstance(mb, SparseMatrix):
                xs.csc_densify_cols(*idx, T)
            else:
                xd.dense_gather_cols(mb._dev(), idx, T, t0)
        tmp = nar["tmp"]
        if tmp is None:
            tmp = nar["tmp"] = SplitMatrix([DenseMatrix(T)] + [self.matrices[i] for i in nar["cat"]],
                                           nar["indices"])
        dm = tmp.matrices[0]
        dm._devblk = DenseDev(T, n, nar["w_pad"], 0)
        sub_cen = None
        if center is not None:
            tc = torch.zeros((nar["w_pad"],), dtype=d.dtype, device=d.device)
            for b, t0, s, idx in nar["parts"]:
                if center.get(b) is not None:
                    tc[t0:t0 + s] = center.get(b)[idx.to(torch.int64)]
            sub_cen = _Centering({0: tc})
        try:
            cs_tmp = [None] * len(tmp.matrices) if colsum is not None else None
            full = tmp._sandwich_dev(d, rows, None, None, cs_tmp, center=sub_cen)
        finally:
            dm._devblk = None
        if colsum is not None:
            if cs_tmp[0] is not None:
                for b, t0, s, _ in nar["parts"]:
                    colsum[b] = cs_tmp[0][t0:t0 + s]
                    if sub_cen is not None and 0 in sub_cen.cs_centered:
                        center.cs_centered.add(b)
            for k, i in enumerate(nar["cat"]):
                if cs_tmp[1 + k] is not None and i in nar["cat_sub"]:
                    colsum[i] = cs_tmp[1 + k][nar["cat_sub"][i]]
        if center is not None:
            g = torch.full_like(nar["sel"], -1, dtype=torch.int32)
            g[nar["sel"] < nar["w_pad"]] = _Centering.NARROW_GROUP
            center.groups = g
        sel = nar["sel"]
        return full.index_select(0, sel).index_select(1, sel)

    def _sandwich_dev(self, d, rows, cols_host, plan=None, colsum=None, center=None, xtv=None):
        if cols_host is not None and len(cols_host) >= FULL_THEN_SELECT * self.shape[1] \
                and len(cols_host) > 0 and self._full_product_pays_cols(cols_host):
            pos_d, sub_d, n_cols = plan if plan is not None else self._sandwich_plan(cols_host)
            cs_full = [None] * len(self.matrices) if colsum is not None else None
            full = self._sandwich_dev(d, rows, None, None, cs_full, center=center, xtv=xtv)
            if colsum is not None:
                for i, c in enumerate(cs_full):
                    if c is not None:
                        colsum[i] = c if sub_d[i] is None else c[sub_d[i].to(torch.int64)]
            cd = self._cols_dev64(cols_host)
            return full.index_select(0, cd).index_select(1, cd)
        parts = self._parts()
        if parts is not None:
            return self._sandwich_parts(parts, d, rows, cols_host, colsum, center)
        if cols_host is not None and plan is None and NARROW_COLS > 0:
            nar = self._narrow_plan(cols_host)
            if nar == "wide":
                cs_full = [None] * len(self.matrices) if colsum is not None else None
                full = self._sandwich_dev(d, rows, None, None, cs_full, center=center, xtv=xtv)
                if colsum is not None:
                    _, sub_sel, _ = self._sandwich_plan(cols_host)
                    for i, c in enumerate(cs_full):
                        if c is not None:
                            colsum[i] = c if sub_sel[i] is None else c[sub_sel[i].to(torch.int64)]
                cd = self._cols_dev64(cols_host)
                return full.index_select(0, cd).index_select(1, cd)
            if nar is not None and d.dtype == D.torch_dtype(self.dtype):
                return self._sandwich_narrow(nar, d, rows, colsum, center)
        pos_d, sub_d, n_cols = plan if plan is not None else self._sandwich_plan(cols_host)
        out = D.zeros((n_cols, n_cols), torch.float64)
        mats = self.matrices
        empty = [sd is not None and D.nlen(sd) == 0 for sd in sub_d]
        done = set()
        return self._sandwich_terms(d, rows, cols_host, colsum, out, pos_d, sub_d, empty, done, center,
                                    xtv if cols_host is None else None)

    def _sandwich_terms(self, d, rows, cols_host, colsum, out, pos_d, sub_d, empty, done, center=None, xtv=None):
        from .ext import dense as xd

        mats = self.matrices
        cat_ids = [i for i, m in enumerate(mats) if isinstance(m, CategoricalMatrix) and not empty[i]
                   and m.shape[1] > 0]
        budget = (128 * 1024) // 8
        groups = self._cat_groups(cat_ids)
        if groups:
            d_eff = D.masked_d(d, rows)
        for grp in groups:
            cats = [(mats[i]._dev(), mats[i].shape[1], mats[i].drop_first) for i in grp]
            total = sum(c[1] for c in cats)
            offs = np.concatenate([[0], np.cumsum([c[1] for c in cats])])
            for w, mw in enumerate(mats):
                if empty[w] or mw.dtype != self.dtype or d.dtype != D.torch_dtype(self.dtype):
                    continue
                stacked = self._fused_cats(mw, cats, grp, d_eff, rows, total, budget, d)
                if stacked is None:
                    continue
                whole = cols_host is None and len(grp) > 1
                if whole:
                    cache = self.__dict__.setdefault("_group_pos", {})
                    gpos = cache.get(tuple(grp))
                    if gpos is None:
                        gpos = cache[tuple(grp)] = torch.cat([pos_d[i] for i in grp])
                    xsplit.scatter_block(stacked.contiguous(), gpos, pos_d[w], out, mirror=True)
                for ci, i in enumerate(grp):
                    res = stacked[int(offs[ci]):int(offs[ci + 1])]
                    if (colsum is not None and colsum[w] is None and not mats[i].drop_first
                            and not mats[i]._has_missings):
                        cs = res.sum(dim=0)
                        colsum[w] = cs if sub_d[w] is None else cs[sub_d[w].to(torch.int64)]
                    if not whole:
                        res = CategoricalMatrix._restrict(res, sub_d[i], sub_d[w])
                        xsplit.scatter_block(res.contiguous(), pos_d[i], pos_d[w], out, mirror=True)
                    done.add((min(i, w), max(i, w)))
        big = [i for i in cat_ids if mats[i].shape[1] > self.FUSED_LEVELS]
        if len(big) >= 2 and len(big) <= 16 and d.dtype == D.torch_dtype(self.dtype):
            cats = [(mats[i]._dev(), mats[i].shape[1], mats[i].drop_first) for i in big]
            offs = np.concatenate([[0], np.cumsum([c[1] for c in cats])])
            d_big = None
            for w, mw in enumerate(mats):
                if (empty[w] or not isinstance(mw, DenseMatrix) or mw.dtype != self.dtype
                        or not xsplit.multi_cat_dense_tile_ok(cats, mw._dev_c())):
                    continue
                if d_big is None:
                    d_big = D.masked_d(d, rows)
                stacked = xsplit.multi_cat_dense_sandwich(cats, d_big, mw._dev_c())
                for ci, i in enumerate(big):
                    res = stacked[int(offs[ci]):int(offs[ci + 1])]
                    if (colsum is not None and colsum[w] is None and not mats[i].drop_first
                            and not mats[i]._has_missings):
                        cs = res.sum(dim=0)
                        colsum[w] = cs if sub_d[w] is None else cs[sub_d[w].to(torch.int64)]
                    res = CategoricalMatrix._restrict(res, sub_d[i], sub_d[w])
                    xsplit.scatter_block(res.contiguous(), pos_d[i], pos_d[w], out, mirror=True)
                    done.add((min(i, w), max(i, w)))
        cat_diag = {}
        diag_scattered = set()
        det = _cm.DETERMINISTIC
        plan = self._cat_pairs_plan() if CAT_PAIRS_FUSED and not det else None
        if (plan is not None and plan.n_pairs > 0
                and d.dtype in (torch.float32, torch.float64)
                and d.dtype == D.torch_dtype(self.dtype)):
            cl = [(mats[i]._dev(), mats[i].shape[1], mats[i].drop_first) for i in plan.cat_ids]
            pos_sel = None if cols_host is None else self._pairs_pos_sel(plan, cols_host)
            tables = xsplit.multi_cat_pairs(plan, cl, d, rows, out, pos=pos_sel)
            for i, j, toff, li, lj, stride in plan.pairs:
                if i == j:
                    if not empty[i]:
                        full = tables[toff:toff + (li - 1) * stride + 1:stride]
                        if sub_d[i] is not None and colsum is not None:
                            full = full[sub_d[i].to(torch.int64)]
                        cat_diag[i] = full.to(d.dtype)
                        diag_scattered.add(i)
                else:
                    done.add((i, j))
        complete = [isinstance(m, CategoricalMatrix) and not m.drop_first and not m._has_missings
                    and sub_d[k] is None and not empty[k] for k, m in enumerate(mats)]
        for i, mi in enumerate(mats):
            if empty[i] or not isinstance(mi, CategoricalMatrix):
                continue
            for j in range(i + 1, len(mats)):
                if empty[j] or not isinstance(mats[j], CategoricalMatrix) or (i, j) in done:
                    continue
                res = mi._cross_sandwich_dev(mats[j], d, rows, sub_d[i], sub_d[j])
                xsplit.scatter_block(res.contiguous(), pos_d[i], pos_d[j], out, mirror=True)
                done.add((i, j))
                if DIAG_FROM_PAIRS and not det and complete[j] and i not in cat_diag:
                    cat_diag[i] = res.sum(dim=1)
                if DIAG_FROM_PAIRS and not det and complete[i] and j not in cat_diag:
                    cat_diag[j] = res.sum(dim=0)
        for i, mi in enumerate(mats):
            if empty[i]:
                continue
            if isinstance(mi, CategoricalMatrix):
                diag = cat_diag[i] if i in cat_diag else mi._sandwich_diag_dev(d, rows, sub_d[i])
                if colsum is not None:
                    colsum[i] = diag
                if i not in diag_scattered:
                    xsplit.scatter_block(diag, pos_d[i], pos_d[i], out, diag=True)
            elif (xtv is not None and colsum is None and center is None and isinstance(mi, DenseMatrix)
                  and sub_d[i] is None and (both := mi._sandwich_xtv_dev(d, xtv.v, rows)) is not None):
                res, xtv.out[i] = both
                xsplit.scatter_block(res, pos_d[i], pos_d[i], out)
            elif (colsum is not None and colsum[i] is None and isinstance(mi, DenseMatrix)
                  and rows is None and sub_d[i] is None
                  and (both := mi._sandwich_xtd_dev(d, cen_i := (center.get(i) if center else None))) is not None):
                res, colsum[i] = both
                if cen_i is not None:
                    center.cs_centered.add(i)
                xsplit.scatter_block(res, pos_d[i], pos_d[i], out)
            elif isinstance(mi, DenseMatrix) and center is not None and center.get(i) is not None:
                res = mi._sandwich_dev(d, rows, sub_d[i], center=center.get(i))
                xsplit.scatter_block(res, pos_d[i], pos_d[i], out)
            else:
                res = mi._sandwich_dev(d, rows, sub_d[i])
                xsplit.scatter_block(res, pos_d[i], pos_d[i], out)
        for i, mi in enumerate(mats):
            if empty[i]:
                continue
            for j in range(i + 1, len(mats)):
                if empty[j] or (i, j) in done:
                    continue
                si, di = (i, j) if isinstance(mi, SparseMatrix) else (j, i)
                if (colsum is not None and colsum[si] is None and isinstance(mats[si], SparseMatrix)
                        and isinstance(mats[di], DenseMatrix)):
                    box = []
                    res = mats[si]._cross_sandwich_dev(mats[di], d, rows, sub_d[si], sub_d[di],
                                                       colsum_box=box)
                    if box:
                        colsum[si] = box[0]
                    if si != i:
                        res = res.T
                else:
                    res = mi._cross_sandwich_dev(mats[j], d, rows, sub_d[i], sub_d[j])
                xsplit.scatter_block(res.contiguous(), pos_d[i], pos_d[j], out, mirror=True)
        return out

    def sandwich_graph(self, d, rows=None, cols=None):
        from .graph import CapturedProduct

        check_sandwich_compatible(self, d)
        rows_d = D.idx_dev(normalize_index(rows, self.shape[0]))
        cols_n = collapse_identity(normalize_index(cols, self.shape[1]), self.shape[1])
        plan = self._sandwich_plan(cols_n)
        return CapturedProduct(lambda dd: self._sandwich_dev(dd, rows_d, cols_n, plan), d)

    def sandwich(self, d, rows=None, cols=None):
        on_dev = D.is_dev(d)
        if not on_dev:
            d = np.asarray(d)
        check_sandwich_compatible(self, d)
        rows_n = normalize_index(rows, self.shape[0])
        cols_n = collapse_identity(normalize_index(cols, self.shape[1]), self.shape[1])
        out = self._sandwich_dev(D.to_dev(d), D.idx_dev(rows_n), cols_n)
        return out if on_dev else D.to_host(out)

    def sandwich_and_transpose_matvec(self, d, v, rows=None, cols=None):
        from .matrix_base import _check_1d

        _check_1d(v)
        d_dev_side, v_dev_side = D.is_dev(d), D.is_dev(v)
        if not d_dev_side:
            d = np.asarray(d)
        if not v_dev_side:
            v = np.asarray(v)
        check_sandwich_compatible(self, d)
        check_matvec_dimensions(self, v, transpose=True)
        rows_n = normalize_index(rows, self.shape[0])
        cols_n = collapse_identity(normalize_index(cols, self.shape[1]), self.shape[1])
        tdt = D.torch_dtype(self.dtype)
        v_dev = D.to_dev(v, tdt)
        acc = None
        if (tdt == torch.float64 and not _cm.DETERMINISTIC
                and (rows_n is None or len(rows_n) < self.shape[0])):
            acc = _Xtv(v_dev)
        H = self._sandwich_dev(D.to_dev(d), D.idx_dev(rows_n), cols_n, xtv=acc)
        g, _ = self._transpose_matvec_dev(v_dev, rows_n, cols_n, done=None if acc is None else acc.out)
        if not v_dev_side:
            g = D.to_host(g)
            if np.issubdtype(v.dtype, np.floating):
                g = g.astype(np.result_type(self.dtype, v.dtype), copy=False)
        return (H if d_dev_side else D.to_host(H)), g

    def sandwich_matvec(self, d, u, rows=None, cols=None):
        from .matrix_base import _smv_args, _smv_compose

        a = _smv_args(self, d, u, rows, cols, h_dtype=np.float64)
        if a.trivial is not None:
            return a.finish(a.trivial)
        tdt = D.torch_dtype(self.dtype)
        res = None
        if (rows is None and cols is None) or self._blocks_finite():
            res = self._smv_dev(a.d_masked(tdt), a.u_full(tdt))
        if res is None:
            return a.finish(_smv_compose(self, a))
        g = res[0]
        if a.cols is not None:
            g = g[self._cols_dev64(a.cols)]
        return a.finish(g)

    def _sdiag_dev(self, d, rows, cols_host=None, centers=None, want_s1=False):
        p = self.shape[1]
        parts = self._parts()
        if parts is not None:
            s2 = D.zeros((p,), torch.float64)
            s1 = D.zeros((p,), torch.float64) if want_s1 else None
            for a, b, part in parts:
                r = None
                if rows is not None:
                    r64 = rows.to(torch.int64)
                    sel = r64[(r64 >= a) & (r64 < b)]
                    if sel.numel() == 0:
                        continue
                    r = (sel - a).to(torch.int32)
                p2, p1 = part._sdiag_dev(d[a:b], r, cols_host, centers, want_s1)
                s2 += p2
                if want_s1:
                    s1 += p1
            return s2, s1
        mask = None
        if cols_host is not None:
            mask = np.zeros(p, dtype=bool)
            mask[np.asarray(cols_host, dtype=np.int64)] = True
        s2 = D.zeros((p,), torch.float64)
        s1 = D.zeros((p,), torch.float64) if want_s1 else None
        idx_d = self._full_dev_indices()
        for b, (mb, idx) in enumerate(zip(self.matrices, self.indices)):
            if mb.shape[0] == 0 or (mask is not None and not mask[idx].any()):
                continue
            r2, r1 = _block_sdiag(mb, d, rows, None if centers is None else centers.get(b), want_s1)
            s2[idx_d[b]] = r2.to(torch.float64)
            if want_s1 and r1 is not None:
                s1[idx_d[b]] = r1.to(torch.float64)
        return s2, s1

    def sandwich_diag(self, d, rows=None, cols=None):
        from .matrix_base import _sd_args
# ... 217 lines not shown
```

Baseline: 1030 GB/s.

## Finish SplitMatrix sandwich blocks directly into the output matrix

Adds "_into" variants of the dense, sparse, cross and multi-categorical sandwich kernels. Their partial-sum reduction writes straight into the final p×p output through index maps, with optional mirroring, so the separate reduce, untile and scatter_block launches and temporary buffers are no longer needed. SplitMatrix.sandwich now takes this path by default when there are no row or column subsets, no centering, and the run is not deterministic. The cost is more code paths and a finishing kernel that writes to scattered locations in the output.

```diff
diff --git a/include/tabmat_hip.h b/include/tabmat_hip.h
--- a/include/tabmat_hip.h
+++ b/include/tabmat_hip.h
@@ -539,6 +539,61 @@
                          const int64_t *ci, double *out, int64_t p, int mirror, int diag,
                          void *stream);
 
+int tm_csr_dense_sandwich_ent_into_f32(const float *vals, const uint16_t *meta, const uint32_t *bstart, int64_t n,
+                                       int64_t m, const float *B, int64_t r, const float *d, float *colsum,
+                                       double *out, int64_t ldo, const int64_t *ri, const int64_t *ci, int mirror,
+                                       int transposed, void *stream);
+int tm_csr_dense_sandwich_ent_into_f64(const double *vals, const uint16_t *meta, const uint32_t *bstart, int64_t n,
+                                       int64_t m, const double *B, int64_t r, const double *d, double *colsum,
+                                       double *out, int64_t ldo, const int64_t *ri, const int64_t *ci, int mirror,
+                                       int transposed, void *stream);
+int tm_sparse_sandwich_blocks_into_u8_f32(const float *cm_data, const uint8_t *cm_col8, const int32_t *cptr,
+                                          int64_t n, int64_t m, int64_t nnz, const int32_t *blocks,
+                                          const int32_t *wg_tab, int n_wg, int max_nb, const float *d, double *out,
+                                          int64_t ldo, const int64_t *ri, const int64_t *ci, int mirror,
+                                          int transposed, void *stream);
+int tm_sparse_sandwich_blocks_into_u8_f64(const double *cm_data, const uint8_t *cm_col8, const int32_t *cptr,
+                                          int64_t n, int64_t m, int64_t nnz, const int32_t *blocks,
+                                          const int32_t *wg_tab, int n_wg, int max_nb, const double *d, double *out,
+                                          int64_t ldo, const int64_t *ri, const int64_t *ci, int mirror,
+                                          int transposed, void *stream);
+int tm_sparse_sandwich_blocks_into_p12_f32(const float *cm_data, const uint8_t *cm_col8, const int32_t *cptr,
+                                           int64_t n, int64_t m, int64_t nnz, const int32_t *blocks12,
+                                           const int32_t *wg_tab, int n_wg, int max_nb, const float *d, double *out,
+                                           int64_t ldo, const int64_t *ri, const int64_t *ci, int mirror,
+                                           int transposed, void *stream);
+int tm_sparse_sandwich_blocks_into_p12_f64(const double *cm_data, const uint8_t *cm_col8, const int32_t *cptr,
+                                           int64_t n, int64_t m, int64_t nnz, const int32_t *blocks12,
+                                           const int32_t *wg_tab, int n_wg, int max_nb, const double *d, double *out,
+                                           int64_t ldo, const int64_t *ri, const int64_t *ci, int mirror,
+                                           int transposed, void *stream);
+int tm_multi_cat_dense_sandwich_into_f32(const void *const *h_codes, const int64_t *h_ncols,
+                                         const int32_t *h_drop_first, int n_cats, int64_t n, const float *d,
+                                         const float *M, int64_t M_ncol, int order_f, double *out, int64_t ldo,
+                                         const int64_t *ri, const int64_t *ci, int mirror, int transposed,
+                                         void *stream);
+int tm_multi_cat_dense_sandwich_into_f64(const void *const *h_codes, const int64_t *h_ncols,
+                                         const int32_t *h_drop_first, int n_cats, int64_t n, const double *d,
+                                         const double *M, int64_t M_ncol, int order_f, double *out, int64_t ldo,
+                                         const int64_t *ri, const int64_t *ci, int mirror, int transposed,
+                                         void *stream);
+int tm_dense_sandwich_i8_into_f64(const double *X, int64_t n, int64_t m, const double *d, const double *colmax,
+                                  double *out, int64_t ldo, int32_t *history, void *stream);
+int tm_multi_cat_sparse_ent_staged(int itemsize, int n_cats, int64_t total_levels, int packed, int64_t n, int64_t mk,
+                                   int64_t n_slots, int *staged);
+int tm_multi_cat_sparse_sandwich_ent_into_f32(const void *const *h_codes, const int64_t *h_ncols,
+                                              const int32_t *h_drop_first, int n_cats, int64_t n, const float *d,
+                                              const float *vals, const uint16_t *meta, const uint32_t *bstart,
+                                              int64_t n_slots, int64_t mk, const uint32_t *packed, double *out,
+                                              int64_t ldo, const int64_t *ri, const int64_t *ci, int mirror,
+                                              int transposed, void *stream);
+int tm_multi_cat_sparse_sandwich_ent_into_f64(const void *const *h_codes, const int64_t *h_ncols,
+                                              const int32_t *h_drop_first, int n_cats, int64_t n, const double *d,
+                                              const double *vals, const uint16_t *meta, const uint32_t *bstart,
+                                              int64_t n_slots, int64_t mk, const uint32_t *packed, double *out,
+                                              int64_t ldo, const int64_t *ri, const int64_t *ci, int mirror,
+                                              int transposed, void *stream);
+
 int tm_sparse_sandwich_chunked_rows_f32(const float *cm_data, const int32_t *cm_indices,
                                         const int32_t *row_ranges, int64_t n_sel, int64_t m,
                                         int64_t nnz, const float *d_sel, float *out, void *stream);
diff --git a/tabmat_amd/csrc/cat.hip b/tabmat_amd/csrc/cat.hip
--- a/tabmat_amd/csrc/cat.hip
+++ b/tabmat_amd/csrc/cat.hip
@@ -1305,7 +1305,7 @@
 static int run_multi_cat_dense(const void *const *h_codes, const int64_t *h_ncols,
                                const int32_t *h_drop, int n_cats, int64_t n, const F *d, const F *M,
                                int64_t m, int order_f, F *out, hipStream_t st,
-                               const int32_t *rows = nullptr, int64_t n_rows = 0) {
+                               const int32_t *rows = nullptr, int64_t n_rows = 0, const FinishDst *dst = nullptr) {
     CatSet cs;
     int rc = make_catset(h_codes, h_ncols, h_drop, n_cats, &cs);
     if (rc) return rc;
@@ -1313,6 +1313,9 @@
     if (total == 0) return TM_OK;
     if (rows != nullptr) n = n_rows;
     if (n == 0) {
+        if (dst)
+            return launch_finish_partials<F>(nullptr, (int64_t)cs.total * 32, 0, (int)ceil_div(m, 32),
+                                             TiledRowsLayout{32, m}, *dst, st);
         TM_HIP(hipMemsetAsync(out, 0, sizeof(F) * (size_t)total, st));
         return TM_OK;
     }
@@ -1357,6 +1360,9 @@
             else if (n_cats == 7) rc = gow(&multi_cat_dense_wide_kernel<F, 7>);
             else rc = gow(&multi_cat_dense_wide_kernel<F, 8>);
             if (rc) return rc;
+            if (dst)
+                return launch_finish_partials<F>(ws, stride, (int)nblk, (int)n_parts, TiledRowsLayout{TJW, m}, *dst,
+                                                 st);
             rc = launch_reduce_partials<F>(ws, stride, (int)nblk, (int)n_parts, tmp, n_parts * stride,
                                            false, st);
             if (rc) return rc;
@@ -1365,6 +1371,10 @@
             TM_LAUNCH_CHECK();
             return TM_OK;
         }
+    }
+    if (dst != nullptr) {
+        set_error("multi_cat_dense_into: only the wide-load path finishes in place");
+        return TM_EUNSUPPORTED;
     }
     if (rows != nullptr) {
         set_error("multi_cat_dense: the row-list form needs the wide-load path");
@@ -1531,17 +1541,35 @@
     }
 }
 
+static bool multi_cat_sparse_ent_staged(size_t fsize, int n_cats, int total_levels, bool packed, int64_t n, int64_t mk,
+                                        int64_t n_slots, size_t *lds_staged_out = nullptr) {
+    const size_t lds = ((sizeof(lds_acc_t) * (size_t)total_levels * (32 + 1) + 15) / 16) * 16;
+    const int nw = (int)std::min<int64_t>(16, std::max<int64_t>(4, tune("catsparse_waves", 16)));
+    const int ncw = packed ? 1 : n_cats;
+    const size_t lds_staged = lds + (size_t)nw * 64 * (fsize + 4 * (size_t)ncw);
+    if (lds_staged_out) *lds_staged_out = lds_staged;
+    const int n_groups = (int)(mk / 16);
+    const int64_t n_slabs = ceil_div(n, 64);
+    const double fill = (double)n_slots / ((double)std::max(n_groups, 1) * (double)std::max<int64_t>(n_slabs, 1));
+    return tune("catsparse_staged", 1) != 0 && lds_staged <= 156 * 1024 &&
+           fill >= (double)tune("catsparse_staged_fill", 44);
+}
+
 template <typename F>
 static int run_multi_cat_sparse_ent(const void *const *h_codes, const int64_t *h_ncols, const int32_t *h_drop,
                                     int n_cats, int64_t n, const F *d, const F *vals, const unsigned short *meta,
                                     const unsigned *bstart, int64_t mk, F *out, hipStream_t st,
-                                    const unsigned *packed = nullptr, int64_t n_slots = 0) {
+                                    const unsigned *packed = nullptr, int64_t n_slots = 0,
+                                    const FinishDst *dst = nullptr) {
     CatSet cs;
     int rc = make_catset(h_codes, h_ncols, h_drop, n_cats, &cs);
     if (rc) return rc;
     const int64_t total = (int64_t)cs.total * mk;
     if (total == 0) return TM_OK;
     if (n == 0) {
+        if (dst)
+            return launch_finish_partials<F>(nullptr, (int64_t)cs.total * 32, 0, (int)ceil_div(mk, 32),
+                                             TiledRowsLayout{32, mk}, *dst, st);
         TM_HIP(hipMemsetAsync(out, 0, sizeof(F) * (size_t)total, st));
         return TM_OK;
     }
@@ -1577,11 +1605,8 @@
                 : n_cats == 7 ? &multi_cat_sparse_ent_kernel<F, 7>
                               : &multi_cat_sparse_ent_kernel<F, 8>;
     TM_REQUIRE(packed == nullptr || (n_cats <= 3 && cs.total < 1023), "packed codes: at most 3 categoricals, 1022 levels");
-    const int ncw = packed != nullptr ? 1 : n_cats;
-    const size_t lds_staged = lds + (size_t)nw * 64 * (sizeof(F) + 4 * (size_t)ncw);
-    const double fill = (double)n_slots / ((double)std::max(n_groups, 1) * (double)n_slabs);
-    if (tune("catsparse_staged", 1) != 0 && lds_staged <= 156 * 1024 &&
-        fill >= (double)tune("catsparse_staged_fill", 44)) {
+    size_t lds_staged = 0;
+    if (multi_cat_sparse_ent_staged(sizeof(F), n_cats, cs.total, packed != nullptr, n, mk, n_slots, &lds_staged)) {
         using KS = void (*)(CatSet, const F *, const F *, const unsigned short *, const unsigned *, int, int64_t, int64_t,
                             int64_t, F *, int64_t, const unsigned *, int);
         KS ks = nullptr;
@@ -1617,6 +1642,8 @@
         prof_end(st);
         TM_LAUNCH_CHECK();
     }
+    if (dst)
+        return launch_finish_partials<F>(ws, stride, (int)nblk, n_pairs, TiledRowsLayout{GC, mk}, *dst, st);
     rc = launch_reduce_partials<F>(ws, stride, (int)nblk, n_pairs, tmp, (int64_t)n_pairs * stride, false, st);
     if (rc) return rc;
     hipLaunchKernelGGL((multi_cat_untile_kernel<F>), dim3((unsigned)ceil_div(total, 256)), dim3(256), 0, st, tmp,
@@ -1782,6 +1809,24 @@
                                     double *out, void *stream) {
     return run_multi_cat_dense<double>(h_codes, h_ncols, h_drop_first, n_cats, n, d, M, M_ncol,
                                        order_f, out, as_stream(stream));
+}
+int tm_multi_cat_dense_sandwich_into_f32(const void *const *h_codes, const int64_t *h_ncols,
+                                         const int32_t *h_drop_first, int n_cats, int64_t n, const float *d,
+                                         const float *M, int64_t M_ncol, int order_f, double *out, int64_t ldo,
+                                         const int64_t *ri, const int64_t *ci, int mirror, int transposed,
+                                         void *stream) {
+    const FinishDst dst{out, ldo, ri, ci, mirror, transposed};
+    return run_multi_cat_dense<float>(h_codes, h_ncols, h_drop_first, n_cats, n, d, M, M_ncol, order_f, nullptr,
+                                      as_stream(stream), nullptr, 0, &dst);
+}
+int tm_multi_cat_dense_sandwich_into_f64(const void *const *h_codes, const int64_t *h_ncols,
+                                         const int32_t *h_drop_first, int n_cats, int64_t n, const double *d,
+                                         const double *M, int64_t M_ncol, int order_f, double *out, int64_t ldo,
+                                         const int64_t *ri, const int64_t *ci, int mirror, int transposed,
+                                         void *stream) {
+    const FinishDst dst{out, ldo, ri, ci, mirror, transposed};
+    return run_multi_cat_dense<double>(h_codes, h_ncols, h_drop_first, n_cats, n, d, M, M_ncol, order_f, nullptr,
+                                       as_stream(stream), nullptr, 0, &dst);
 }
 int tm_multi_cat_dense_sandwich_rows_f32(const void *const *h_codes, const int64_t *h_ncols,
                                          const int32_t *h_drop_first, int n_cats, int64_t n,
@@ -1838,6 +1883,32 @@
                                           int64_t n_slots, int64_t mk, const uint32_t *packed, double *out, void *stream) {
     return run_multi_cat_sparse_ent<double>(h_codes, h_ncols, h_drop_first, n_cats, n, d, vals, meta, bstart, mk,
                                             out, as_stream(stream), packed, n_slots);
+}
+int tm_multi_cat_sparse_ent_staged(int itemsize, int n_cats, int64_t total_levels, int packed, int64_t n, int64_t mk,
+                                   int64_t n_slots, int *staged) {
+    TM_REQUIRE(staged != nullptr && (itemsize == 4 || itemsize == 8), "staged is required; itemsize 4 or 8");
+    *staged = multi_cat_sparse_ent_staged((size_t)itemsize, n_cats, (int)total_levels, packed != 0, n, mk, n_slots) ? 1 : 0;
+    return TM_OK;
+}
+int tm_multi_cat_sparse_sandwich_ent_into_f32(const void *const *h_codes, const int64_t *h_ncols,
+                                              const int32_t *h_drop_first, int n_cats, int64_t n, const float *d,
+                                              const float *vals, const uint16_t *meta, const uint32_t *bstart,
+                                              int64_t n_slots, int64_t mk, const uint32_t *packed, double *out,
+                                              int64_t ldo, const int64_t *ri, const int64_t *ci, int mirror,
+                                              int transposed, void *stream) {
+    const FinishDst dst{out, ldo, ri, ci, mirror, transposed};
+    return run_multi_cat_sparse_ent<float>(h_codes, h_ncols, h_drop_first, n_cats, n, d, vals, meta, bstart, mk,
+                                           nullptr, as_stream(stream), packed, n_slots, &dst);
+}
+int tm_multi_cat_sparse_sandwich_ent_into_f64(const void *const *h_codes, const int64_t *h_ncols,
+                                              const int32_t *h_drop_first, int n_cats, int64_t n, const double *d,
+                                              const double *vals, const uint16_t *meta, const uint32_t *bstart,
+                                              int64_t n_slots, int64_t mk, const uint32_t *packed, double *out,
+                                              int64_t ldo, const int64_t *ri, const int64_t *ci, int mirror,
+                                              int transposed, void *stream) {
+    const FinishDst dst{out, ldo, ri, ci, mirror, transposed};
+    return run_multi_cat_sparse_ent<double>(h_codes, h_ncols, h_drop_first, n_cats, n, d, vals, meta, bstart, mk,
+                                            nullptr, as_stream(stream), packed, n_slots, &dst);
 }
 int tm_multi_cat_sparse_sandwich_slab_f32(const void *const *h_codes, const int64_t *h_ncols,
                                           const int32_t *h_drop_first, int n_cats, int64_t n,
diff --git a/tabmat_amd/csrc/reduce.hpp b/tabmat_amd/csrc/reduce.hpp
--- a/tabmat_amd/csrc/reduce.hpp
+++ b/tabmat_amd/csrc/reduce.hpp
@@ -58,6 +58,88 @@
     return TM_OK;
 }
 
+
+struct FinishDst {
+    double *out;
+    int64_t ldo;
+    const int64_t *ri;
+    const int64_t *ci;
+    int mirror;
+    int transposed;
+
+    __device__ __forceinline__ void put(int64_t a, int64_t b, double v) const {
+        const int64_t r = ri[transposed ? b : a], c = ci[transposed ? a : b];
+        if (r < 0 || c < 0) return;
+        out[r * ldo + c] = v;
+        if (mirror) out[c * ldo + r] = v;
+    }
+};
+
+struct TiledRowsLayout {
+    int W;
+    int64_t n_cols;
+
+    __device__ __forceinline__ void place(int part, int64_t e, double v, const FinishDst &dst) const {
+        const int64_t a = e / W, b = (int64_t)part * W + e % W;
+        if (b < n_cols) dst.put(a, b, v);
+    }
+};
+
+struct LowerTilesLayout {
+    int TS;
+    int64_t m;
+
+    __device__ __forceinline__ void place(int part, int64_t e, double v, const FinishDst &dst) const {
+        int I = 0;
+        while ((I + 1) * (I + 2) / 2 <= part) ++I;
+        const int J = part - I * (I + 1) / 2;
+        const int64_t hi = (int64_t)I * TS + e / TS, lo = (int64_t)J * TS + e % TS;
+        if (hi >= m || lo > hi) return;
+        dst.put(hi, lo, v);
+        if (lo != hi) dst.put(lo, hi, v);
+    }
+};
+
+template <typename F, int NW, typename L>
+__global__ __launch_bounds__(NW * 64) void finish_partials_kernel(const F *__restrict__ ws, int64_t stride,
+                                                                  int nb, L lay, FinishDst dst) {
+    __shared__ double red[NW][64];
+    const int lane = threadIdx.x & 63;
+    const int wave = threadIdx.x >> 6;
+    const int64_t e = (int64_t)blockIdx.x * 64 + lane;
+    const int part = blockIdx.y;
+    double acc = 0.0;
+    if (e < stride) {
+        const F *p = ws + ((int64_t)part * nb) * stride + e;
+        for (int b = wave; b < nb; b += NW) acc += (double)p[(int64_t)b * stride];
+    }
+    red[wave][lane] = acc;
+    __syncthreads();
+    if (wave == 0 && e < stride) {
+        double s = 0.0;
+#pragma unroll
+        for (int w = 0; w < NW; w += 4)
+            s += (red[w][lane] + red[w + 1][lane]) + (red[w + 2][lane] + red[w + 3][lane]);
+        lay.place(part, e, (double)(F)s, dst);
+    }
+}
+
+template <typename F, typename L>
+inline int launch_finish_partials(const F *ws, int64_t stride, int nb, int n_parts, L lay, const FinishDst &dst,
+                                  hipStream_t st) {
+    TM_REQUIRE(dst.out != nullptr && dst.ri != nullptr && dst.ci != nullptr && dst.ldo > 0,
+               "finish: out, ri, ci and a positive ldo are required");
+    if (stride == 0 || n_parts == 0) return TM_OK;
+    dim3 grid((unsigned)ceil_div(stride, 64), (unsigned)n_parts);
+    const bool small = (int64_t)grid.x * grid.y < 1024 && nb > 16;
+    if (small)
+        hipLaunchKernelGGL((finish_partials_kernel<F, 16, L>), grid, dim3(1024), 0, st, ws, stride, nb, lay, dst);
+    else
+        hipLaunchKernelGGL((finish_partials_kernel<F, 4, L>), grid, dim3(256), 0, st, ws, stride, nb, lay, dst);
+    TM_LAUNCH_CHECK();
+    return TM_OK;
+}
+
 __global__ void fill_i32_kernel(int32_t *p, int64_t n, int32_t v);
 __global__ void scatter_iota_i32_kernel(int32_t *map, const int32_t *cols, int64_t n_cols);
 
diff --git a/tabmat_amd/csrc/sparse_blocks.hip b/tabmat_amd/csrc/sparse_blocks.hip
--- a/tabmat_amd/csrc/sparse_blocks.hip
+++ b/tabmat_amd/csrc/sparse_blocks.hip
@@ -202,15 +202,17 @@
 template <typename F, bool U8 = false, bool D12 = false>
 static int run_sparse_sandwich_blocks(const F *data, const int32_t *ind, const int32_t *cptr, int64_t n,
                                       int64_t m, int64_t nnz, const int32_t *blocks, const int32_t *wg_tab,
-                                      int n_wg, int max_nb, const F *d, F *out, hipStream_t st) {
+                                      int n_wg, int max_nb, const F *d, F *out, hipStream_t st,
+                                      const FinishDst *dst = nullptr) {
     if (m == 0) return TM_OK;
-    if (n == 0 || nnz == 0 || n_wg == 0) {
-        TM_HIP(hipMemsetAsync(out, 0, sizeof(F) * (size_t)(m * m), st));
-        return TM_OK;
-    }
     constexpr int TS = KB_TS;
     const int nchunk = (int)ceil_div(m, TS);
     const int n_parts = nchunk * (nchunk + 1) / 2;
+    if (n == 0 || nnz == 0 || n_wg == 0) {
+        if (dst) return launch_finish_partials<F>(nullptr, (int64_t)TS * TS, 0, n_parts, LowerTilesLayout{TS, m}, *dst, st);
+        TM_HIP(hipMemsetAsync(out, 0, sizeof(F) * (size_t)(m * m), st));
+        return TM_OK;
+    }
     TM_REQUIRE(nnz < (1ll << 31) && n < (1ll << 29), "sparse block too large for the block-list sandwich");
     TM_REQUIRE(!D12 || n < (1ll << 24), "12-byte block descriptors hold 24 bits of row");
     TM_REQUIRE(max_nb >= 1 && n_wg >= 1, "empty workgroup table");
@@ -233,6 +235,8 @@
                        max_nb, ws, wg_log_ptr());
     prof_end(st);
     TM_LAUNCH_CHECK();
+    if (dst)
+        return launch_finish_partials<F>(ws, (int64_t)TS * TS, max_nb, n_parts, LowerTilesLayout{TS, m}, *dst, st);
     rc = launch_reduce_partials<F>(ws, (int64_t)TS * TS, max_nb, n_parts, tmp, (int64_t)n_parts * TS * TS,
                                    false, st);
     if (rc) return rc;
@@ -295,4 +299,20 @@
                                                                tmh::as_stream(stream));
 }
 
-}
+
+#define TM_K2B_INTO(NAME, F, ...)                                                                                 \
+    int NAME(const F *cm_data, const uint8_t *cm_col8, const int32_t *cptr, int64_t n, int64_t m, int64_t nnz,     \
+             const int32_t *blocks, const int32_t *wg_tab, int n_wg, int max_nb, const F *d, double *out,          \
+             int64_t ldo, const int64_t *ri, const int64_t *ci, int mirror, int transposed, void *stream) {        \
+        const tmh::FinishDst dst{out, ldo, ri, ci, mirror, transposed};                                            \
+        return tmh::run_sparse_sandwich_blocks<__VA_ARGS__>(cm_data, reinterpret_cast<const int32_t *>(cm_col8),   \
+                                                            cptr, n, m, nnz, blocks, wg_tab, n_wg, max_nb, d,      \
+                                                            nullptr, tmh::as_stream(stream), &dst);                \
+    }
+TM_K2B_INTO(tm_sparse_sandwich_blocks_into_u8_f32, float, float, true)
+TM_K2B_INTO(tm_sparse_sandwich_blocks_into_u8_f64, double, double, true)
+TM_K2B_INTO(tm_sparse_sandwich_blocks_into_p12_f32, float, float, true, true)
+TM_K2B_INTO(tm_sparse_sandwich_blocks_into_p12_f64, double, double, true, true)
+#undef TM_K2B_INTO
+
+}
diff --git a/tabmat_amd/csrc/sparse_ent.hip b/tabmat_amd/csrc/sparse_ent.hip
--- a/tabmat_amd/csrc/sparse_ent.hip
+++ b/tabmat_amd/csrc/sparse_ent.hip
@@ -360,7 +360,8 @@
 
 template <typename F>
 static int run_csr_dense_ent(const F *vals, const uint16_t *meta, const uint32_t *bstart, int64_t n, int64_t m,
-                             const F *B, int64_t r, const F *d, F *out, F *colsum, hipStream_t st) {
+                             const F *B, int64_t r, const F *d, F *out, F *colsum, hipStream_t st,
+                             const FinishDst *dst = nullptr) {
     const int64_t nB = r;
     const int64_t total = m * nB;
     if (total == 0) return TM_OK;
@@ -383,8 +384,9 @@
     const int nz = (int)ceil_div(n_groups, EN_NW);
     const bool want_csum = colsum != nullptr;
     if (n_slabs == 0) {
+        if (want_csum) TM_HIP(hipMemsetAsync(colsum, 0, sizeof(F) * (size_t)m, st));
+        if (dst) return launch_finish_partials<F>(nullptr, m * EN_W, 0, n_parts, TiledRowsLayout{EN_W, nB}, *dst, st);
         TM_HIP(hipMemsetAsync(out, 0, sizeof(F) * (size_t)total, st));
-        if (want_csum) TM_HIP(hipMemsetAsync(colsum, 0, sizeof(F) * (size_t)m, st));
         return TM_OK;
     }
     int64_t nblk = std::max<int64_t>(1, tune("ent_rounds", 1) * NUM_CU / ((int64_t)n_parts * nz));
@@ -411,11 +413,16 @@
                        reinterpret_cast<long long *>((uintptr_t)tune("ent_prof", 0)));
     prof_end(st);
     TM_LAUNCH_CHECK();
-    rc = launch_reduce_partials<F>(ws, stride, (int)nblk, n_parts, tmp, n_parts * stride, false, st);
-    if (rc) return rc;
-    hipLaunchKernelGGL((en_untile_kernel<F>), dim3((unsigned)ceil_div(total, 256)), dim3(256), 0, st, tmp, m,
-                       nB, out);
-    TM_LAUNCH_CHECK();
+    if (dst) {
+        rc = launch_finish_partials<F>(ws, stride, (int)nblk, n_parts, TiledRowsLayout{EN_W, nB}, *dst, st);
+        if (rc) return rc;
+    } else {
+        rc = launch_reduce_partials<F>(ws, stride, (int)nblk, n_parts, tmp, n_parts * stride, false, st);
+        if (rc) return rc;
+        hipLaunchKernelGGL((en_untile_kernel<F>), dim3((unsigned)ceil_div(total, 256)), dim3(256), 0, st, tmp, m,
+                           nB, out);
+        TM_LAUNCH_CHECK();
+    }
     if (want_csum) {
         hipLaunchKernelGGL((en_csum_kernel<F>), dim3((unsigned)ceil_div(m, 256)), dim3(256), 0, st, ws_csum,
                            (int)nblk, m, colsum);
@@ -441,4 +448,21 @@
                                   double *colsum, void *stream) {
     return tmh::run_csr_dense_ent<double>(vals, meta, bstart, n, m, B, r, d, out, colsum, tmh::as_stream(stream));
 }
-}
+
+int tm_csr_dense_sandwich_ent_into_f32(const float *vals, const uint16_t *meta, const uint32_t *bstart, int64_t n,
+                                       int64_t m, const float *B, int64_t r, const float *d, float *colsum,
+                                       double *out, int64_t ldo, const int64_t *ri, const int64_t *ci, int mirror,
+                                       int transposed, void *stream) {
+    const tmh::FinishDst dst{out, ldo, ri, ci, mirror, transposed};
+    return tmh::run_csr_dense_ent<float>(vals, meta, bstart, n, m, B, r, d, nullptr, colsum, tmh::as_stream(stream),
+                                         &dst);
+}
+int tm_csr_dense_sandwich_ent_into_f64(const double *vals, const uint16_t *meta, const uint32_t *bstart, int64_t n,
+                                       int64_t m, const double *B, int64_t r, const double *d, double *colsum,
+                                       double *out, int64_t ldo, const int64_t *ri, const int64_t *ci, int mirror,
+                                       int transposed, void *stream) {
+    const tmh::FinishDst dst{out, ldo, ri, ci, mirror, transposed};
+    return tmh::run_csr_dense_ent<double>(vals, meta, bstart, n, m, B, r, d, nullptr, colsum, tmh::as_stream(stream),
+                                          &dst);
+}
+}
diff --git a/tabmat_amd/csrc/syrk_i8.hip b/tabmat_amd/csrc/syrk_i8.hip
--- a/tabmat_amd/csrc/syrk_i8.hip
+++ b/tabmat_amd/csrc/syrk_i8.hip
@@ -753,6 +753,13 @@
     return tmh::run_syrk_i8(X, n, m, d, colmax, out, colsum, history, tmh::as_stream(stream));
 }
 
+int tm_dense_sandwich_i8_into_f64(const double *X, int64_t n, int64_t m, const double *d, const double *colmax,
+                                  double *out, int64_t ldo, int32_t *history, void *stream) {
+    TM_REQUIRE(out != nullptr && ldo >= m, "out (the block's first entry in the result) and its row stride");
+    return tmh::run_syrk_i8_panel(X, m, n, m, d, colmax, out, ldo, nullptr, history, tmh::as_stream(stream), nullptr,
+                                  nullptr, nullptr);
+}
+
 int tm_dense_sandwich_i8_centered_f64(const double *X, int64_t n, int64_t m, const double *d, const double *colmax,
                                       const double *center, double *out, double *colsum, int32_t *history,
                                       void *stream) {
diff --git a/tabmat_amd/dense_matrix.py b/tabmat_amd/dense_matrix.py
--- a/tabmat_amd/dense_matrix.py
+++ b/tabmat_amd/dense_matrix.py
@@ -237,6 +237,15 @@
                 return xd.dense_sandwich_i8(self._dev_c(), d, cmax, history=self._i8_history(key), center=center)
         return xd.dense_sandwich(self._dev_c(), d, rows, cols, center=center)
 
+    def _sandwich_into_dev(self, d, out, off) -> bool:
+        if not (SYRK_I8 and d.dtype == torch.float64 and self.shape[1] <= 128):
+            return False
+        cmax = self._i8_colmax(None)
+        if cmax is None:
+            return False
+        xd.dense_sandwich_i8_into(self._dev_c(), d, cmax, out, off, history=self._i8_history(None))
+        return True
+
     def _sandwich_xtd_dev(self, d, center=None):
         blk = self._dev_c()
         if SYRK_I8 and d.dtype == torch.float64 and blk.m <= 128:
diff --git a/tabmat_amd/ext/dense.py b/tabmat_amd/ext/dense.py
--- a/tabmat_amd/ext/dense.py
+++ b/tabmat_amd/ext/dense.py
@@ -139,6 +139,21 @@
         return out, cs
     call("tm_dense_sandwich_i8_f64", D.p(X.buf), X.n, X.m, D.p(d), D.p(colmax), D.p(out), D.stream_ptr())
     return out
+
+
+def dense_sandwich_i8_into(X: DenseDev, d, colmax, out, off, history=None):
+    import torch
+    from .._lib import lib
+
+    p = int(out.shape[1])
+    assert out.dtype == torch.float64 and out.is_contiguous() and out.shape[0] == p
+    if not (0 <= off and off + X.m <= p):
+        raise ValueError("the block does not fit the result at this offset")
+    D.same_float("dense_sandwich_i8_into", X.buf, d, colmax)
+    if history is not None and history.numel() < int(lib().tm_dense_sandwich_i8_history_words()):
+        raise ValueError("history needs tm_dense_sandwich_i8_history_words() int32 words")
+    call("tm_dense_sandwich_i8_into_f64", D.p(X.buf), X.n, X.m, D.p(d), D.p(colmax),
+         out.data_ptr() + 8 * off * (p + 1), p, D.p(history), D.stream_ptr())
 
 
 def dense_sandwich_i8_wide(X: DenseDev, d, colmax, center=None):
diff --git a/tabmat_amd/ext/sparse.py b/tabmat_amd/ext/sparse.py
--- a/tabmat_amd/ext/sparse.py
+++ b/tabmat_amd/ext/sparse.py
@@ -161,6 +161,26 @@
     return (out[A.inv], cs[A.inv]) if want_colsum else out[A.inv]
 
 
+def ent_kernel_pos(A: SlabEnt, pos):
+    import torch
+
+    kpos = torch.full((A.mk,), -1, dtype=torch.int64, device=pos.device)
+    kpos[A.inv] = pos.to(torch.int64)
+    return kpos
+
+
+def csr_dense_sandwich_ent_into(A: SlabEnt, B: DenseDev, d, out, ri, ci, mirror=False, transposed=False,
+                                want_colsum=False):
+    assert B.n == A.n and ell_supported(B) and A.m > 0 and B.m > 0 and A.n > 0
+    assert out.dtype == D.torch.float64 and out.is_contiguous()
+    cs = D.out_buf((A.mk,), A.dtype) if want_colsum else None
+    D.same_float("csr_dense_sandwich_ent_into", A.vals, B.buf, d)
+    call("tm_csr_dense_sandwich_ent_into_" + D.fsuf(A.vals), D.p(A.vals), D.p(A.meta), D.p(A.bstart), A.n, A.mk,
+         D.p(B.buf), B.m, D.p(d), D.p(cs), D.p(out), out.shape[1], D.p(ri), D.p(ci), int(mirror), int(transposed),
+         D.stream_ptr())
+    return cs[A.inv] if want_colsum else None
+
+
 def _row_table(A: CsrDev, rows, d, as_set: bool):
     import weakref
 
@@ -263,6 +283,18 @@
          int(cm_data.numel()), D.p(blocks), D.p(wg_tab), int(wg_tab.shape[0]), int(max_nb), D.p(d),
          D.p(out), D.stream_ptr())
     return out
+
+
+def sparse_sandwich_blocks_into(A: CsrDev, d, out, ri, ci, mirror=False, transposed=False):
+    assert K2B_U8 and A.m > 0 and A.n > 0
+    assert out.dtype == D.torch.float64 and out.is_contiguous()
+    D.same_float("sparse_sandwich_blocks_into", A.data, d)
+    cm_data, cm_c8, cptr = A.chunk_major()
+    blocks, wg_tab, max_nb = A.pair_blocks(d12=None)
+    form = "p12" if int(blocks.shape[1]) == 3 else "u8"
+    call(f"tm_sparse_sandwich_blocks_into_{form}_{D.fsuf(A.data)}", D.p(cm_data), D.p(cm_c8), D.p(cptr), A.n, A.m,
+         int(cm_data.numel()), D.p(blocks), D.p(wg_tab), int(wg_tab.shape[0]), int(max_nb), D.p(d), D.p(out),
+         out.shape[1], D.p(ri), D.p(ci), int(mirror), int(transposed), D.stream_ptr())
 
 
 def sparse_sandwich_pairs(A: CsrDev, d):
diff --git a/tabmat_amd/ext/split.py b/tabmat_amd/ext/split.py
--- a/tabmat_amd/ext/split.py
+++ b/tabmat_amd/ext/split.py
@@ -368,6 +368,16 @@
     return res
 
 
+def multi_cat_dense_sandwich_into(cats, d, mat_j: DenseDev, out, ri, ci, mirror=False, transposed=False):
+    assert multi_cat_dense_wide_ok(cats, mat_j) and mat_j.n > 0
+    assert out.dtype == D.torch.float64 and out.is_contiguous()
+    codes, ncols, drop, n = _cat_args(cats)
+    D.same_float("multi_cat_dense_sandwich_into", mat_j.buf, d)
+    call(f"tm_multi_cat_dense_sandwich_into_{D.fsuf(mat_j.buf)}", codes, ncols, drop, n, mat_j.n, D.p(d),
+         D.p(mat_j.buf), mat_j.m, mat_j.order_f, D.p(out), out.shape[1], D.p(ri), D.p(ci), int(mirror),
+         int(transposed), D.stream_ptr())
+
+
 def multi_cat_sparse_sandwich(cats, d, S: SlabCsc):
     total = sum(int(c[1]) for c in cats)
     if total == 0 or S.m == 0 or S.n == 0:
@@ -412,6 +422,26 @@
     return res[:, E.inv]
 
 
+def multi_cat_sparse_ent_staged(cats, E, packed=None) -> bool:
+    total = sum(int(c[1]) for c in cats)
+    if total == 0 or E.m == 0 or E.n == 0 or not 1 <= len(cats) <= 8:
+        return False
+    flag = C.c_int(0)
+    call("tm_multi_cat_sparse_ent_staged", E.vals.element_size(), len(cats), total, int(packed is not None), E.n,
+         E.mk, E.n_slots(), C.byref(flag))
+    return bool(flag.value)
+
+
+def multi_cat_sparse_sandwich_ent_into(cats, d, E, out, ri, ci, packed=None, mirror=False, transposed=False):
+    assert E.m > 0 and E.n > 0 and sum(int(c[1]) for c in cats) > 0
+    assert out.dtype == D.torch.float64 and out.is_contiguous()
+    codes, ncols, drop, n = _cat_args(cats)
+    D.same_float("multi_cat_sparse_sandwich_ent_into", E.vals, d)
+    call(f"tm_multi_cat_sparse_sandwich_ent_into_{D.fsuf(E.vals)}", codes, ncols, drop, n, E.n, D.p(d), D.p(E.vals),
+         D.p(E.meta), D.p(E.bstart), E.n_slots(), E.mk, D.p(packed), D.p(out), out.shape[1], D.p(ri), D.p(ci),
+         int(mirror), int(transposed), D.stream_ptr())
+
+
 def multi_cat_sparse_sandwich_rows(cats, d, A, rows):
     from . import sparse as xs
 
diff --git a/tabmat_amd/sparse_matrix.py b/tabmat_amd/sparse_matrix.py
--- a/tabmat_amd/sparse_matrix.py
+++ b/tabmat_amd/sparse_matrix.py
@@ -334,6 +334,55 @@
                 res = res[c64][:, c64].contiguous()
             return res
         return xs.sparse_sandwich(A, d, rows, cols)
+
+    def _sandwich_into_dev(self, d, out, pos) -> bool:
+        from . import categorical_matrix as _cm
+
+        if _cm.DETERMINISTIC or not xs.K2B_U8 or self._row_parts() is not None:
+            return False
+        A = self._dev()
+        if self.shape[0] == 0 or not 0 < A.data.numel() < 2**31 or self.shape[1] > 128 * 32:
+            return False
+        if getattr(self, "_pairs_pay", None) is None:
+            self._pairs_pay = xs.pairs_sandwich_pays(A)
+        if self._pairs_pay:
+            return False
+        if getattr(self, "_direct_pays", None) is None:
+            self._direct_pays = xs.direct_sandwich_pays(A)
+        if self._direct_pays:
+            return False
+        if getattr(self, "_blocks_pay", None) is None:
+            self._blocks_pay = xs.blocks_sandwich_pays(A)
+        if not self._blocks_pay:
+            return False
+        xs.sparse_sandwich_blocks_into(A, d, out, pos, pos)
+        return True
+
+    def _ent_kernel_pos(self, ent, pos):
+        hit = getattr(self, "_ent_kpos", None)
+        if hit is None or hit[0] is not pos or hit[1] is not ent:
+            hit = self._ent_kpos = (pos, ent, xs.ent_kernel_pos(ent, pos))
+        return hit[2]
+
+    def _cross_dense_into_dev(self, other, d, out, pos_self, pos_other, transposed) -> bool:
+        if other.dtype != self.dtype or self._row_parts() is not None:
+            return False
+        Bd = other._dev_c()
+        A = self._dev()
+        if self.shape[0] == 0 or A.data.numel() == 0 or self.shape[1] == 0 or Bd.m == 0:
+            return False
+        if (A.data.numel() <= SORTED_K3_NNZ_PER_ROW * self.shape[0] and self.shape[1] >= 1024
+                and xs.ell_supported(Bd)):
+            return False
+        ent = self._ent() if (Bd.m > 64 and xs.ell_supported(Bd)) else None
+        if ent is None:
+            return False
+        kpos = self._ent_kernel_pos(ent, pos_self)
+        if transposed:
+            xs.csr_dense_sandwich_ent_into(ent, Bd, d, out, pos_other, kpos, mirror=True, transposed=True)
+        else:
+            xs.csr_dense_sandwich_ent_into(ent, Bd, d, out, kpos, pos_other, mirror=True)
+        return True
 
     def _ent_det(self):
         ent = self._ent()
diff --git a/tabmat_amd/split_matrix.py b/tabmat_amd/split_matrix.py
--- a/tabmat_amd/split_matrix.py
+++ b/tabmat_amd/split_matrix.py
@@ -37,6 +37,7 @@
 FULL_UNSELECTED_SHARE = 0.2
 FULL_THEN_SELECT_MV = 0.0
 NARROW_COLS = int(os.environ.get("TABMAT_AMD_NARROW_COLS", "128"))
+SANDWICH_INTO = os.environ.get("TABMAT_AMD_SANDWICH_INTO", "1") != "0"
 from . import categorical_matrix as _cm
 from . import sparse_matrix as _spm
 
@@ -421,19 +422,42 @@
             return xsplit.multi_cat_sparse_sandwich_rows(cats, d_rows, mw._dev(), rows)
         if (isinstance(mw, SparseMatrix) and total * 33 <= budget
                 and mw._dev().data.numel() > 0 and (rows is None or mw._values_finite())):
-            ent = None
-            if len(cats) <= 8 and (getattr(mw, "_entblk", None) or any(
-                    isinstance(mo, DenseMatrix) and mo.shape[1] > 64 and mo.dtype == mw.dtype
-                    for mo in self.matrices)):
-                ent = mw._ent()
+            ent, packed = self._cat_sparse_ent(mw, cats, cat_ids)
             if ent is not None:
-                pk_cache = self.__dict__.setdefault("_packed_codes", {})
-                key = tuple(cat_ids)
-                if key not in pk_cache:
-                    pk_cache[key] = xsplit.pack_codes(cats)
-                return xsplit.multi_cat_sparse_sandwich_ent(cats, d_eff, ent, pk_cache[key])
+                return xsplit.multi_cat_sparse_sandwich_ent(cats, d_eff, ent, packed)
             return xsplit.multi_cat_sparse_sandwich(cats, d_eff, mw._slab())
         return None
+
+    def _cat_sparse_ent(self, mw, cats, cat_ids):
+        ent = None
+        if len(cats) <= 8 and (getattr(mw, "_entblk", None) or any(
+                isinstance(mo, DenseMatrix) and mo.shape[1] > 64 and mo.dtype == mw.dtype
+                for mo in self.matrices)):
+            ent = mw._ent()
+        if ent is None:
+            return None, None
+        pk_cache = self.__dict__.setdefault("_packed_codes", {})
+        key = tuple(cat_ids)
+        if key not in pk_cache:
+            pk_cache[key] = xsplit.pack_codes(cats)
+        return ent, pk_cache[key]
+
+    def _fused_cats_into(self, mw, cats, cat_ids, d, total, budget, out, gpos, pos_w) -> bool:
+        if mw.shape[0] == 0 or mw.shape[1] == 0 or total == 0:
+            return False
+        if isinstance(mw, DenseMatrix):
+            if not xsplit.multi_cat_dense_wide_ok(cats, mw._dev_c()):
+                return False
+            xsplit.multi_cat_dense_sandwich_into(cats, d, mw._dev_c(), out, gpos, pos_w, mirror=True)
+            return True
+        if isinstance(mw, SparseMatrix) and total * 33 <= budget and mw._dev().data.numel() > 0:
+            ent, packed = self._cat_sparse_ent(mw, cats, cat_ids)
+            if ent is None or not xsplit.multi_cat_sparse_ent_staged(cats, ent, packed):
+                return False
+            xsplit.multi_cat_sparse_sandwich_ent_into(cats, d, ent, out, gpos, mw._ent_kernel_pos(ent, pos_w),
+                                                      packed=packed, mirror=True)
+            return True
+        return False
 
     def _parts(self):
         parts = self.__dict__.get("_row_parts", False)
@@ -624,7 +648,7 @@
         sel = nar["sel"]
         return full.index_select(0, sel).index_select(1, sel)
 
-    def _sandwich_dev(self, d, rows, cols_host, plan=None, colsum=None, center=None, xtv=None):
+    def _sandwich_dev(self, d, rows, cols_host, plan=None, colsum=None, center=None, xtv=None, into=False):
         if cols_host is not None and len(cols_host) >= FULL_THEN_SELECT * self.shape[1] \
                 and len(cols_host) > 0 and self._full_product_pays_cols(cols_host):
             pos_d, sub_d, n_cols = plan if plan is not None else self._sandwich_plan(cols_host)
@@ -659,12 +683,31 @@
         empty = [sd is not None and D.nlen(sd) == 0 for sd in sub_d]
         done = set()
         return self._sandwich_terms(d, rows, cols_host, colsum, out, pos_d, sub_d, empty, done, center,
-                                    xtv if cols_host is None else None)
-
-    def _sandwich_terms(self, d, rows, cols_host, colsum, out, pos_d, sub_d, empty, done, center=None, xtv=None):
+                                    xtv if cols_host is None else None, into)
+
+    def _contiguous_offset(self, i):
+        cache = self.__dict__.setdefault("_contig_off", {})
+        if i not in cache:
+            idx = np.asarray(self.indices[i], dtype=np.int64)
+            ok = idx.size > 0 and bool((np.diff(idx) == 1).all())
+            cache[i] = int(idx[0]) if ok else None
+        return cache[i]
+
+    def _group_positions(self, grp, pos_d):
+        cache = self.__dict__.setdefault("_group_pos", {})
+        gpos = cache.get(tuple(grp))
+        if gpos is None:
+            gpos = cache[tuple(grp)] = pos_d[grp[0]] if len(grp) == 1 else torch.cat([pos_d[i] for i in grp])
+        return gpos
+
+    def _sandwich_terms(self, d, rows, cols_host, colsum, out, pos_d, sub_d, empty, done, center=None, xtv=None,
+                        into=False):
         from .ext import dense as xd
 
         mats = self.matrices
+        into = (into and SANDWICH_INTO and cols_host is None and rows is None and colsum is None and center is None
+                and xtv is None and not _cm.DETERMINISTIC and d.dtype == D.torch_dtype(self.dtype)
+                and d.dtype in (torch.float32, torch.float64) and out.is_contiguous())
         cat_ids = [i for i, m in enumerate(mats) if isinstance(m, CategoricalMatrix) and not empty[i]
                    and m.shape[1] > 0]
         budget = (128 * 1024) // 8
@@ -678,16 +721,17 @@
             for w, mw in enumerate(mats):
                 if empty[w] or mw.dtype != self.dtype or d.dtype != D.torch_dtype(self.dtype):
                     continue
+                if into and self._fused_cats_into(mw, cats, grp, d, total, budget, out, self._group_positions(grp, pos_d),
+                                                  pos_d[w]):
+                    done.update((min(i, w), max(i, w)) for i in grp)
+                    continue
                 stacked = self._fused_cats(mw, cats, grp, d_eff, rows, total, budget, d)
                 if stacked is None:
                     continue
                 whole = cols_host is None and len(grp) > 1
                 if whole:
-                    cache = self.__dict__.setdefault("_group_pos", {})
-                    gpos = cache.get(tuple(grp))
-                    if gpos is None:
-                        gpos = cache[tuple(grp)] = torch.cat([pos_d[i] for i in grp])
-                    xsplit.scatter_block(stacked.contiguous(), gpos, pos_d[w], out, mirror=True)
+                    xsplit.scatter_block(stacked.contiguous(), self._group_positions(grp, pos_d), pos_d[w], out,
+                                         mirror=True)
                 for ci, i in enumerate(grp):
                     res = stacked[int(offs[ci]):int(offs[ci + 1])]
                     if (colsum is not None and colsum[w] is None and not mats[i].drop_first
@@ -777,6 +821,12 @@
             elif isinstance(mi, DenseMatrix) and center is not None and center.get(i) is not None:
                 res = mi._sandwich_dev(d, rows, sub_d[i], center=center.get(i))
                 xsplit.scatter_block(res, pos_d[i], pos_d[i], out)
+            elif into and isinstance(mi, SparseMatrix) and mi.dtype == self.dtype \
+                    and mi._sandwich_into_dev(d, out, pos_d[i]):
+                pass
+            elif into and isinstance(mi, DenseMatrix) and mi.dtype == self.dtype \
+                    and (off := self._contiguous_offset(i)) is not None and mi._sandwich_into_dev(d, out, off):
+                pass
             else:
                 res = mi._sandwich_dev(d, rows, sub_d[i])
                 xsplit.scatter_block(res, pos_d[i], pos_d[i], out)
@@ -787,6 +837,9 @@
                 if empty[j] or (i, j) in done:
                     continue
                 si, di = (i, j) if isinstance(mi, SparseMatrix) else (j, i)
+                if (into and isinstance(mats[si], SparseMatrix) and isinstance(mats[di], DenseMatrix)
+                        and mats[si]._cross_dense_into_dev(mats[di], d, out, pos_d[si], pos_d[di], si != i)):
+                    continue
                 if (colsum is not None and colsum[si] is None and isinstance(mats[si], SparseMatrix)
                         and isinstance(mats[di], DenseMatrix)):
                     box = []
@@ -808,7 +861,7 @@
         rows_d = D.idx_dev(normalize_index(rows, self.shape[0]))
         cols_n = collapse_identity(normalize_index(cols, self.shape[1]), self.shape[1])
         plan = self._sandwich_plan(cols_n)
-        return CapturedProduct(lambda dd: self._sandwich_dev(dd, rows_d, cols_n, plan), d)
+        return CapturedProduct(lambda dd: self._sandwich_dev(dd, rows_d, cols_n, plan, into=True), d)
 
     def sandwich(self, d, rows=None, cols=None):
         on_dev = D.is_dev(d)
@@ -817,7 +870,7 @@
         check_sandwich_compatible(self, d)
         rows_n = normalize_index(rows, self.shape[0])
         cols_n = collapse_identity(normalize_index(cols, self.shape[1]), self.shape[1])
-        out = self._sandwich_dev(D.to_dev(d), D.idx_dev(rows_n), cols_n)
+        out = self._sandwich_dev(D.to_dev(d), D.idx_dev(rows_n), cols_n, into=True)
         return out if on_dev else D.to_host(out)
 
     def sandwich_and_transpose_matvec(self, d, v, rows=None, cols=None):
```

After: 1033 GB/s, median of 6. No clear change (+0.4%).
